# lmjakt/kmer_hasheR

Hardware: NVIDIA B200
Metric: kmers_indexed_per_s (higher is better)
Workload: dtype u64

## Files before the change

include/kmergpu.h:

```cpp
#ifndef KMERGPU_H
#define KMERGPU_H

#include <stddef.h>
#include <stdint.h>

#ifdef __cplusplus
extern "C" {
#endif

#define KMG_MAX_K 32

typedef enum {
  KMG_OK = 0,
  KMG_ERR_ARG = -1,
  KMG_ERR_K = -2,
  KMG_ERR_RANGE = -3,
  KMG_ERR_CUDA = -4,
  KMG_ERR_NOMEM = -5,
  KMG_ERR_NODEV = -6,
  KMG_ERR_UNSTABLE = -7
} kmg_status;

typedef struct kmg_index kmg_index;
typedef struct kmg_query kmg_query;
typedef struct kmg_join kmg_join;

const char *kmg_last_error(void);
int kmg_version(void);
int kmg_device_count(int *n);
int kmg_set_device(int device);
int kmg_set_stream(void *cuda_stream);
void *kmg_host_alloc(size_t bytes);
void kmg_host_free(void *p);

int kmg_build(const char *seq, int64_t len, int k, kmg_index **out);

#define KMG_ORDER_GROUPED 0
#define KMG_ORDER_SORTED 1
int kmg_build_ordered(const char *seq, int64_t len, int k, int order, kmg_index **out);
int kmg_index_order(const kmg_index *idx);

int kmg_free(kmg_index *idx);

int kmg_sizes(const kmg_index *idx, uint64_t *U, uint64_t *N, uint64_t *P);
int kmg_index_k(const kmg_index *idx);

int kmg_kmers_u64(const kmg_index *idx, uint64_t *keys );
int kmg_kmers_ascii(const kmg_index *idx, char *buf );
int kmg_counts(const kmg_index *idx, int32_t *counts );
int kmg_positions(const kmg_index *idx, int32_t *out );
int kmg_pairs(const kmg_index *idx, int32_t *out );
int kmg_pairs_chunk(const kmg_index *idx, uint64_t first, uint64_t n, int32_t *out );
int kmg_positions_base(const kmg_index *idx, uint64_t i_base, int32_t *out);
int kmg_pairs_chunk_base(const kmg_index *idx, uint64_t i_base, uint64_t first, uint64_t n, int32_t *out);

int kmg_query_begin(const kmg_index *idx, const char *q, int64_t qlen, int k, kmg_query **st,
                    uint64_t *M);
int kmg_query_begin_rc(const kmg_index *idx, const char *q, int64_t qlen, int k, kmg_query **st,
                       uint64_t *M);
int kmg_query_emit(kmg_query *st, int32_t *out );
int kmg_query_emit_chunk(kmg_query *st, uint64_t first, uint64_t n, int32_t *out );
int kmg_query_free(kmg_query *st);

int kmg_join_begin(const kmg_index *a, const kmg_index *b, kmg_join **st, uint64_t *M);
int kmg_join_emit(kmg_join *st, int32_t *out );
int kmg_join_emit_chunk(kmg_join *st, uint64_t first, uint64_t n, int32_t *out );
int kmg_join_free(kmg_join *st);

int kmg_shard_sample(const void *d_seq, int64_t g0, int64_t g1, int64_t L, int64_t s0, int64_t s1,
                     int k, int n, uint64_t *d_samples);
int kmg_shard_partition(const void *d_seq, int64_t g0, int64_t g1, int64_t L, int64_t s0,
                        int64_t s1, int k, const uint64_t *splitters ,
                        int nparts, uint64_t *d_keys, uint32_t *d_pos, uint64_t *counts);
int kmg_build_records(uint64_t *d_keys, uint32_t *d_pos, int64_t n, int k, kmg_index **out);
int kmg_query_records(const kmg_index *idx, const uint64_t *d_keys, const int32_t *d_i, int64_t n,
                      kmg_query **st, uint64_t *M);

typedef struct kmg_shard kmg_shard;
int kmg_shard_open(const void *d_seq, int64_t g0, int64_t g1, int64_t L, int64_t s0, int64_t s1,
                   int k, kmg_shard **out);
int kmg_shard_pack_bytes(int n_samples);
int kmg_shard_pack(const void *d_own, int64_t n_own, int k, int n_samples, int order, void *d_pack);
int kmg_shard_open_packed(const void *d_own, int64_t n_own, int64_t L, int world, int rank, int k,
                          int n_samples, int order, const void *d_allpack, kmg_shard **out,
                          uint64_t *d_splitters);
int kmg_shard_close(kmg_shard *sh);
int kmg_shard_set_mixed(kmg_shard *sh, int mixed);
int kmg_shard_windows(const kmg_shard *sh, int64_t *nstarts);
int kmg_shard_sample_keys(const kmg_shard *sh, int n, uint64_t *d_samples);
int kmg_shard_count(const kmg_shard *sh, const uint64_t *d_splitters, int nparts, uint64_t *d_counts);
int kmg_shard_scatter(const kmg_shard *sh, const uint64_t *d_splitters, int nparts, int rank,
                      void *const *peer_keys, void *const *peer_pos, uint64_t capacity,
                      const uint64_t *d_matrix, int32_t pos_add, uint64_t *d_info);
int kmg_build_received(uint64_t *d_keys, uint32_t *d_pos, uint64_t capacity, const uint64_t *d_info,
                       int k, int order, kmg_index **out);
int kmg_query_received(const kmg_index *idx, const uint64_t *d_keys, const int32_t *d_i,
                       uint64_t capacity, const uint64_t *d_info, int mixed, kmg_query **st,
                       uint64_t *M);
int kmg_shard_scatter_ranges(const kmg_shard *sh, int nparts, int rank, void *const *peer_keys, void *const *peer_pos,
                             void *const *peer_counts, uint64_t region_cap, int32_t pos_add);
int kmg_build_regions(uint64_t *d_keys, uint32_t *d_pos, uint64_t region_cap, int nparts, const uint64_t *d_counts, int k,
                      kmg_index **out);
int kmg_query_regions(const kmg_index *idx, const uint64_t *d_keys, const int32_t *d_i, uint64_t region_cap, int nparts,
                      const uint64_t *d_counts, kmg_query **st, uint64_t *M);
int kmg_ipc_alloc(size_t bytes, void **dptr, void *handle);
int kmg_ipc_free(void *dptr);
int kmg_ipc_open(const void *handle, void **dptr);
int kmg_ipc_close(void *dptr);

typedef struct kmg_counter kmg_counter;
int kmg_count_new(int k, int source_n, kmg_counter **out);
int kmg_count_add(kmg_counter *c, const char *seq, int64_t len, int source);
int kmg_count_sizes(const kmg_counter *c, uint64_t *U, int *source_n, int *k, uint64_t *new_total);
int kmg_count_kmers_u64(const kmg_counter *c, uint64_t *keys );
int kmg_count_kmers_ascii(const kmg_counter *c, char *buf );
int kmg_count_matrix(const kmg_counter *c, int32_t *out );
int kmg_count_positions(const kmg_counter *c, int32_t *out );
int kmg_count_spectrum(const kmg_counter *c, int source , uint32_t max_count, double *spec );
int kmg_index_spectrum(const kmg_index *idx, uint32_t max_count, double *spec );
int kmg_count_free(kmg_counter *c);

typedef struct kmg_reads kmg_reads;
int kmg_reads_open(const char *path, kmg_reads **out);
int kmg_reads_from_memory(const void *text, int64_t len, kmg_reads **out);
int kmg_reads_count(const kmg_reads *r, uint64_t *n_records, uint64_t *total_bases);
int kmg_reads_record(const kmg_reads *r, uint64_t i, int64_t *seq_len, char *name_buf, int name_cap);
int kmg_reads_sequence(const kmg_reads *r, uint64_t i, char *out );
int kmg_build_record(const kmg_reads *r, uint64_t i, int k, int order, kmg_index **out);
int kmg_count_add_reads(kmg_counter *c, const kmg_reads *r, int source);
int kmg_reads_free(kmg_reads *r);

int kmg_profile_enable(int on);
int kmg_profile_reset(void);
int kmg_profile_count(void);
int kmg_profile_get(int i, const char **name, double *total_ms, uint64_t *launches,
                    double *algo_bytes);
// ... 12 lines not shown
```

kmer_hasher_b200/__init__.py:

```python
from __future__ import annotations

import ctypes as C

import numpy as np

from . import _lib
from ._lib import KmgError, check

__all__ = ["KmerHash", "KmerCounts", "SequenceFile", "make_kmer_hash_file", "count_kmers_file", "make_kmer_hash", "kmer_pos", "seq_kmer_pos", "kmer_pairs", "count_kmers", "kmer_spectrum",
           "pinned_empty", "KmgError",
           "OPT_KMER", "OPT_POS", "OPT_PAIRS", "OPT_COUNT"]

OPT_KMER, OPT_POS, OPT_PAIRS, OPT_COUNT = 1, 2, 4, 8
ORDER_GROUPED, ORDER_SORTED = 0, 1
KMER_HASH_TAG = "kmer_hash_250930"
MAX_K = 32
INT_MAX = 2**31 - 1

_L = _lib.load()


def _seq_buffer(seq):
    if isinstance(seq, str):
        seq = seq.encode("latin-1")
# ... 99 lines not shown
        return nt.value

    def free(self):
        if self._h:
            _L.kmg_count_free(self._h)
            self._h = None


def _extract(ex_ptr) -> KmerHash:
    if not isinstance(ex_ptr, KmerHash):
        raise TypeError("ptr_r should be an external pointer")
    if ex_ptr.tag != KMER_HASH_TAG:
        raise ValueError("External pointer has incorrect tag")
    return ex_ptr


def _extract_index(ex_ptr) -> KmerHash:
    ix = _extract(ex_ptr)
    if isinstance(ix, KmerCounts):
        raise ValueError("this external pointer holds k-mer counts (count.kmers), not a position index")
    return ix


def make_kmer_hash(seq, k, do_sort=False) -> KmerHash:
    if isinstance(seq, (list, tuple)):
        if len(seq) < 1:
            raise ValueError("seq_r should be a character vector of length at least one")
        seq = seq[0]
    k = int(k)
    order = ORDER_SORTED if int(do_sort) else ORDER_GROUPED
    if k < 1 or k > MAX_K:
        raise ValueError("k must be a positive integer less than 1+MAX_K")
    ptr, n, keep = _seq_buffer(seq)
    if n <= k:
        raise ValueError("the length of the sequence must be at least k")
    h = C.c_void_p()
    check(_L.kmg_build_ordered(ptr, n, k, order, C.byref(h)))
    del keep
    return KmerHash(h.value, k)


def _by_key(ix: "KmerHash"):
    U = ix.sizes_un[0]
    keys = np.empty(U, np.uint64)
    check(_L.kmg_kmers_u64(ix._handle(), _out_ptr(keys)))
    order = np.argsort(keys, kind="stable")
    rank = np.empty(U, np.int64)
    rank[order] = np.arange(U)
    return keys, order, rank


def _renumber(rows: np.ndarray, rank: np.ndarray) -> np.ndarray:
    if len(rows) == 0:
        return rows
    new_i = rank[rows[:, 0].astype(np.int64) - 1] + 1
    o = np.argsort(new_i, kind="stable")
    out = rows[o].copy()
    out[:, 0] = new_i[o].astype(np.int32)
    return out


def kmer_pos(ex_ptr, opt_flag, out: dict | None = None, canonical: bool = False) -> dict:
    ix = _extract(ex_ptr)
    opt_flag = int(opt_flag)
    if isinstance(ix, KmerCounts):
        return _count_table_pos(ix, opt_flag)
    out = out or {}
    U, N = ix.sizes_un
    P = ix.sizes[2] if opt_flag & OPT_PAIRS else 0
    h = ix._handle()
    res = {"kmer": None, "pos": None, "pair.pos": None, "count": None}
    if opt_flag & OPT_KMER:
        buf = out.get("kmer_buf")
        if buf is None:
            buf = np.empty(U * (ix.k + 1), np.uint8)
        check(_L.kmg_kmers_ascii(h, _out_ptr(buf)))
        res["kmer"] = np.ascontiguousarray(buf[:U * (ix.k + 1)].reshape(U, ix.k + 1)[:, :ix.k]).view(f"S{ix.k}").ravel()
    if opt_flag & OPT_POS:
        if N > INT_MAX:
            raise OverflowError("pos matrix extent exceeds int")
        a = out.get("pos")
        if a is None:
            a = np.empty((N, 2), np.int32)
        check(_L.kmg_positions(h, _out_ptr(a)))
        res["pos"] = a[:N]
    if opt_flag & OPT_PAIRS:
        if P > INT_MAX:
            raise OverflowError(f"pair.pos would need {P} rows; an R matrix extent is int "
                                "(use kmg_pairs_chunk to stream)")
        a = out.get("pair.pos")
        if a is None:
            a = np.empty((P, 3), np.int32)
        check(_L.kmg_pairs(h, _out_ptr(a)))
        res["pair.pos"] = a[:P]
    if opt_flag & OPT_COUNT:
        a = out.get("count")
        if a is None:
            a = np.empty(U, np.int32)
        check(_L.kmg_counts(h, _out_ptr(a)))
        res["count"] = a[:U]
    if canonical and _L.kmg_index_order(h) != ORDER_SORTED:
        _, order, rank = _by_key(ix)
        if res["kmer"] is not None:
            res["kmer"] = res["kmer"][order]
        if res["count"] is not None:
            res["count"] = np.asarray(res["count"])[order]
        if res["pos"] is not None:
            res["pos"] = _renumber(np.asarray(res["pos"]), rank)
        if res["pair.pos"] is not None:
            res["pair.pos"] = _renumber(np.asarray(res["pair.pos"]), rank)
    return res


def count_kmers(seq, params, hash_ptr: "KmerCounts | None" = None) -> KmerCounts:
    params = [int(p) for p in params]
    if len(params) != 3:
        raise ValueError("k_r must be an integer vector of length 3")
    k, source, source_n = params
    if k < 1 or k > MAX_K:
        raise ValueError("k must be a positive integer less than 1+MAX_K")
    if source_n < 1 or source >= source_n or source < 0:
        raise ValueError("source_n must be larger than 1 and larger than source")
    if isinstance(seq, (str, bytes, bytearray, np.ndarray)) or hasattr(seq, "data_ptr"):
        seq = [seq]
    if len(seq) < 1:
        raise ValueError("seq_r should be a character vector of length at least one")
    if hash_ptr is None:
        h = C.c_void_p()
        check(_L.kmg_count_new(k, source_n, C.byref(h)))
        hash_ptr = KmerCounts(h.value, k, source_n)
    else:
        if not isinstance(hash_ptr, KmerCounts):
            raise ValueError("failed to extract kmer_hash from external pointer")
        if hash_ptr.k != k:
            raise ValueError("mismatch between specified k and that given in the external pointer")
        if hash_ptr.source_n != source_n:
            raise ValueError("mismatch between specified source_n and that of the external pointer")
    for s in seq:
        ptr, n, keep = _seq_buffer(s)
        if n <= k:
            continue
        check(_L.kmg_count_add(hash_ptr._handle(), ptr, n, source))
        del keep
    return hash_ptr


def _count_table_pos(ct: KmerCounts, opt_flag: int) -> dict:
    U = ct.sizes[0]
    sn, h = ct.source_n, ct._handle()
    res = {"kmer": None, "pos": None, "pair.pos": None, "count": None}
    if opt_flag & OPT_KMER:
        buf = np.empty(U * (ct.k + 1), np.uint8)
        check(_L.kmg_count_kmers_ascii(h, _out_ptr(buf)))
        res["kmer"] = np.ascontiguousarray(buf.reshape(U, ct.k + 1)[:, :ct.k]).view(f"S{ct.k}").ravel()
    if opt_flag & OPT_POS:
        if U * sn > INT_MAX:
            raise OverflowError("pos matrix extent exceeds int")
        a = np.empty((U * sn, 2), np.int32)
        check(_L.kmg_count_positions(h, _out_ptr(a)))
        res["pos"] = a
    if opt_flag & OPT_PAIRS:
        m = np.empty((U, sn), np.int32)
        check(_L.kmg_count_matrix(h, _out_ptr(m)))
        ia, ib = np.triu_indices(sn, 1)
        rows = np.empty((U, len(ia), 3), np.int32)
        rows[:, :, 0] = np.arange(1, U + 1, dtype=np.int32)[:, None]
        rows[:, :, 1] = m[:, ia]
        rows[:, :, 2] = m[:, ib]
        res["pair.pos"] = rows.reshape(-1, 3)
    if opt_flag & OPT_COUNT:
        res["count"] = np.full(U, sn, np.int32)
    return res


class SequenceFile:

    def __init__(self, path_or_text):
        h = C.c_void_p()
# ... 163 lines not shown
```

kmer_hasher_b200/_lib.py:

```python
from __future__ import annotations

import ctypes as C
import os

_HERE = os.path.dirname(os.path.abspath(__file__))
LIB_PATH = os.path.join(_HERE, "csrc", "libkmergpu.so")

u64p = C.POINTER(C.c_uint64)
i32p = C.POINTER(C.c_int32)
vp = C.c_void_p

SIGNATURES = {
    "kmg_last_error": (C.c_char_p, []),
    "kmg_version": (C.c_int, []),
    "kmg_device_count": (C.c_int, [C.POINTER(C.c_int)]),
    "kmg_set_device": (C.c_int, [C.c_int]),
    "kmg_set_stream": (C.c_int, [vp]),
    "kmg_host_alloc": (vp, [C.c_size_t]),
    "kmg_host_free": (None, [vp]),
    "kmg_build": (C.c_int, [vp, C.c_int64, C.c_int, C.POINTER(vp)]),
    "kmg_build_ordered": (C.c_int, [vp, C.c_int64, C.c_int, C.c_int, C.POINTER(vp)]),
    "kmg_index_order": (C.c_int, [vp]),
    "kmg_free": (C.c_int, [vp]),
    "kmg_sizes": (C.c_int, [vp, u64p, u64p, u64p]),
    "kmg_index_k": (C.c_int, [vp]),
    "kmg_kmers_u64": (C.c_int, [vp, vp]),
    "kmg_kmers_ascii": (C.c_int, [vp, vp]),
    "kmg_counts": (C.c_int, [vp, vp]),
    "kmg_positions": (C.c_int, [vp, vp]),
    "kmg_pairs": (C.c_int, [vp, vp]),
    "kmg_pairs_chunk": (C.c_int, [vp, C.c_uint64, C.c_uint64, vp]),
    "kmg_query_begin": (C.c_int, [vp, vp, C.c_int64, C.c_int, C.POINTER(vp), u64p]),
    "kmg_query_begin_rc": (C.c_int, [vp, vp, C.c_int64, C.c_int, C.POINTER(vp), u64p]),
    "kmg_query_emit": (C.c_int, [vp, vp]),
    "kmg_query_emit_chunk": (C.c_int, [vp, C.c_uint64, C.c_uint64, vp]),
    "kmg_query_free": (C.c_int, [vp]),
    "kmg_join_begin": (C.c_int, [vp, vp, C.POINTER(vp), u64p]),
    "kmg_join_emit": (C.c_int, [vp, vp]),
    "kmg_join_emit_chunk": (C.c_int, [vp, C.c_uint64, C.c_uint64, vp]),
    "kmg_join_free": (C.c_int, [vp]),
    "kmg_shard_sample": (C.c_int, [vp, C.c_int64, C.c_int64, C.c_int64, C.c_int64, C.c_int64, C.c_int, C.c_int, vp]),
    "kmg_shard_partition": (C.c_int, [vp, C.c_int64, C.c_int64, C.c_int64, C.c_int64, C.c_int64, C.c_int,
                                      u64p, C.c_int, vp, vp, u64p]),
    "kmg_build_records": (C.c_int, [vp, vp, C.c_int64, C.c_int, C.POINTER(vp)]),
    "kmg_query_records": (C.c_int, [vp, vp, vp, C.c_int64, C.POINTER(vp), u64p]),
    "kmg_shard_open": (C.c_int, [vp, C.c_int64, C.c_int64, C.c_int64, C.c_int64, C.c_int64, C.c_int, C.POINTER(vp)]),
    "kmg_shard_close": (C.c_int, [vp]),
    "kmg_shard_pack_bytes": (C.c_int, [C.c_int]),
    "kmg_shard_pack": (C.c_int, [vp, C.c_int64, C.c_int, C.c_int, C.c_int, vp]),
    "kmg_shard_open_packed": (C.c_int, [vp, C.c_int64, C.c_int64, C.c_int, C.c_int, C.c_int, C.c_int, C.c_int, vp, C.POINTER(vp), vp]),
    "kmg_shard_set_mixed": (C.c_int, [vp, C.c_int]),
    "kmg_shard_windows": (C.c_int, [vp, C.POINTER(C.c_int64)]),
    "kmg_shard_sample_keys": (C.c_int, [vp, C.c_int, vp]),
    "kmg_shard_count": (C.c_int, [vp, vp, C.c_int, vp]),
    "kmg_shard_scatter": (C.c_int, [vp, vp, C.c_int, C.c_int, C.POINTER(vp), C.POINTER(vp), C.c_uint64, vp, C.c_int32, vp]),
    "kmg_build_received": (C.c_int, [vp, vp, C.c_uint64, vp, C.c_int, C.c_int, C.POINTER(vp)]),
    "kmg_query_received": (C.c_int, [vp, vp, vp, C.c_uint64, vp, C.c_int, C.POINTER(vp), u64p]),
    "kmg_shard_scatter_ranges": (C.c_int, [vp, C.c_int, C.c_int, C.POINTER(vp), C.POINTER(vp), C.POINTER(vp), C.c_uint64, C.c_int32]),
    "kmg_build_regions": (C.c_int, [vp, vp, C.c_uint64, C.c_int, vp, C.c_int, C.POINTER(vp)]),
    "kmg_query_regions": (C.c_int, [vp, vp, vp, C.c_uint64, C.c_int, vp, C.POINTER(vp), u64p]),
    "kmg_ipc_alloc": (C.c_int, [C.c_size_t, C.POINTER(vp), vp]),
    "kmg_ipc_free": (C.c_int, [vp]),
    "kmg_ipc_open": (C.c_int, [vp, C.POINTER(vp)]),
    "kmg_ipc_close": (C.c_int, [vp]),
    "kmg_profile_enable": (C.c_int, [C.c_int]),
    "kmg_profile_reset": (C.c_int, []),
    "kmg_profile_count": (C.c_int, []),
    "kmg_profile_get": (C.c_int, [C.c_int, C.POINTER(C.c_char_p), C.POINTER(C.c_double), u64p, C.POINTER(C.c_double)]),
    "kmg_launch_count": (C.c_uint64, []),
    "kmg_selftest_lane_order": (C.c_int, [C.POINTER(C.c_uint32)]),
    "kmg_tune": (C.c_int, [C.c_char_p, C.c_int]),
    "kmg_count_new": (C.c_int, [C.c_int, C.c_int, C.POINTER(vp)]),
    "kmg_count_add": (C.c_int, [vp, vp, C.c_int64, C.c_int]),
    "kmg_count_sizes": (C.c_int, [vp, u64p, C.POINTER(C.c_int), C.POINTER(C.c_int), u64p]),
    "kmg_count_kmers_u64": (C.c_int, [vp, vp]),
    "kmg_count_kmers_ascii": (C.c_int, [vp, vp]),
    "kmg_count_matrix": (C.c_int, [vp, vp]),
    "kmg_count_positions": (C.c_int, [vp, vp]),
    "kmg_count_spectrum": (C.c_int, [vp, C.c_int, C.c_uint32, C.POINTER(C.c_double)]),
    "kmg_index_spectrum": (C.c_int, [vp, C.c_uint32, C.POINTER(C.c_double)]),
    "kmg_count_free": (C.c_int, [vp]),
    "kmg_reads_open": (C.c_int, [C.c_char_p, C.POINTER(vp)]),
    "kmg_reads_from_memory": (C.c_int, [vp, C.c_int64, C.POINTER(vp)]),
    "kmg_reads_count": (C.c_int, [vp, u64p, u64p]),
    "kmg_reads_record": (C.c_int, [vp, C.c_uint64, C.POINTER(C.c_int64), C.c_char_p, C.c_int]),
    "kmg_reads_sequence": (C.c_int, [vp, C.c_uint64, vp]),
    "kmg_build_record": (C.c_int, [vp, C.c_uint64, C.c_int, C.c_int, C.POINTER(vp)]),
    "kmg_count_add_reads": (C.c_int, [vp, vp, C.c_int]),
    "kmg_reads_free": (C.c_int, [vp]),
    "kmg_tune_get": (C.c_int64, [C.c_char_p, C.c_int64]),
    "kmg_trim": (C.c_int, []),
    "kmg_cached_bytes": (C.c_uint64, []),
    "kmg_positions_base": (C.c_int, [vp, C.c_uint64, vp]),
    "kmg_pairs_chunk_base": (C.c_int, [vp, C.c_uint64, C.c_uint64, C.c_uint64, vp]),
}

_lib = None


class KmgError(RuntimeError):
    def __init__(self, code: int, msg: str):
        super().__init__(f"libkmergpu error {code}: {msg}")
        self.code = code


def load() -> C.CDLL:
    global _lib
    if _lib is not None:
        return _lib
    if not os.path.exists(LIB_PATH):
        raise ImportError(f"{LIB_PATH} is missing: run `python -c 'import __graft_entry__ as g; g.build()'` "
                          "(libkmergpu is CUDA-only; there is no CPU fallback)")
    lib = C.CDLL(LIB_PATH)
    for name, (res, args) in SIGNATURES.items():
        fn = getattr(lib, name)
        fn.restype = res
        fn.argtypes = args
    _lib = lib
    return lib


def check(rc: int) -> None:
    if rc != 0:
        raise KmgError(rc, load().kmg_last_error().decode("utf-8", "replace"))
```

kmer_hasher_b200/csrc/api.cu:

```cuda
#include <cstdarg>
#include <cstdio>
#include <cstring>
#include <ctime>
#include <algorithm>
#include <atomic>
#include <condition_variable>
#include <deque>
#include <thread>
#include <map>
#include <mutex>
#include <string>
#include <type_traits>
#include <vector>

#include "../../include/kmergpu.h"
#include "common.cuh"
#include "csr.cuh"
#include "lookback.cuh"
#include "probe.cuh"
#include "sort.cuh"
#include "windows.cuh"

using namespace kmg;

// ... 321 lines not shown
  }
  ~CopyPool() {
    { std::lock_guard<std::mutex> l(mu); stop = true; }
    cv_work.notify_all();
    for (auto &t : th) t.join();
  }
};
static CopyPool g_pool;
constexpr size_t STAGE_BYTES = size_t(64) << 20;
constexpr int STAGE_SLOTS = 3;
struct Staging {
  std::mutex mu;
  char *slot[STAGE_SLOTS] = {nullptr, nullptr, nullptr};
  int ensure() {
    for (auto &p : slot)
      if (!p && cudaMallocHost((void **)&p, STAGE_BYTES) != cudaSuccess) { cudaGetLastError(); return fail(KMG_ERR_NOMEM, "pinned staging allocation failed"); }
    return KMG_OK;
  }
  void release() { for (auto &p : slot) { if (p) cudaFreeHost(p); p = nullptr; } }
};
static Staging g_stage;
static void stage_release() { std::lock_guard<std::mutex> gs(g_stage.mu); g_stage.release(); }
static bool staged_transfers() {
  static int on = -1;
  if (on < 0) { const char *e = getenv("KMERGPU_STAGING"); on = !(e && e[0] == '0'); }
  return on == 1;
}

static int staged_upload(void *d_dst, const void *h_src, size_t bytes, cudaStream_t s) {
  std::lock_guard<std::mutex> g(g_stage.mu);
  TRY(g_stage.ensure());
  cudaEvent_t *ev = g_ctx.ev + 4;
  int c = 0;
  for (size_t off = 0; off < bytes; off += STAGE_BYTES, ++c) {
    const int sl = c % STAGE_SLOTS;
    const size_t n = std::min(STAGE_BYTES, bytes - off);
    if (c >= STAGE_SLOTS) CU(cudaEventSynchronize(ev[sl]));
    g_pool.submit(c, g_stage.slot[sl], (const char *)h_src + off, n);
    g_pool.wait(c);
    CU(cudaMemcpyAsync((char *)d_dst + off, g_stage.slot[sl], n, cudaMemcpyHostToDevice, s));
    CU(cudaEventRecord(ev[sl], s));
  }
  CU(cudaStreamSynchronize(s));
  return KMG_OK;
}

enum PtrKind { PK_HOST_PAGEABLE, PK_HOST_PINNED, PK_DEVICE };
static PtrKind ptr_kind(const void *p) {
  cudaPointerAttributes a;
  if (cudaPointerGetAttributes(&a, p) != cudaSuccess) { cudaGetLastError(); return PK_HOST_PAGEABLE; }
  if (a.type == cudaMemoryTypeDevice || a.type == cudaMemoryTypeManaged) return PK_DEVICE;
  if (a.type == cudaMemoryTypeHost) return PK_HOST_PINNED;
  return PK_HOST_PAGEABLE;
}

struct DevSeq {
  uint8_t *buf = nullptr;
  uint8_t *base = nullptr;
  int64_t len = 0;
};
static int upload_seq(const void *src, int64_t len, cudaStream_t s, DevSeq *out) {
  size_t cap = 16 + (size_t)((len + 15) / 16) * 16 + 16;
  TRY(dalloc(&out->buf, cap, s));
  out->base = out->buf + 16;
  out->len = len;
  CU(cudaMemsetAsync(out->buf, 0, 16, s));
  CU(cudaMemsetAsync(out->buf + cap - 32, 0, 32, s));
  if (len > (int64_t)(8 << 20) && staged_transfers() && ptr_kind(src) == PK_HOST_PAGEABLE) return staged_upload(out->base, src, (size_t)len, s);
  if (len > 0) CU(cudaMemcpyAsync(out->base, src, (size_t)len, cudaMemcpyDefault, s));
  return KMG_OK;
}

struct kmg_index {
  int device = 0;
  int k = 0;
  uint64_t U = 0, N = 0;
  uint64_t P = 0, multi = 0;
  uint32_t maxc = 0;
  bool have_stats = false;
  bool grouped = false;
  int hbits = 0;
  bool unstable = false;
  uint64_t *ukeys = nullptr;
  uint32_t *ustart = nullptr;
  uint32_t *pos = nullptr;
  std::mutex mu;
  uint4 *hash = nullptr;
  uint64_t hash_nb = 0;
  int hash_hbits = 0;
  uint32_t *multi_u = nullptr;
  uint64_t *pair_off = nullptr;
};
struct kmg_query {
  const kmg_index *idx = nullptr;
  uint64_t H = 0, M = 0;
  int32_t *hit_i = nullptr;
  uint32_t *hit_start = nullptr;
  uint64_t *row_off = nullptr;
};

constexpr int HIST_THREADS = 512, HIST_ITEMS = 16, HIST_TILE = HIST_THREADS * HIST_ITEMS;
constexpr int RLE_THREADS = 256, RLE_ITEMS = 16, RLE_TILE = RLE_THREADS * RLE_ITEMS;
constexpr int PROBE_THREADS = 256, PROBE_ITEMS = 8, PROBE_TILE = PROBE_THREADS * PROBE_ITEMS;
constexpr int COMPACT_ITEMS = 8, COMPACT_TILE = PROBE_THREADS * COMPACT_ITEMS;
constexpr int EMIT_THREADS = 256, EMIT_TILE = EMIT_THREADS * 8;
constexpr int PIDX_THREADS = 256, PIDX_ITEMS = 8, PIDX_TILE = PIDX_THREADS * PIDX_ITEMS;

static int g_sort_shape = -1;
static int g_rank_override = -1;
static std::atomic<int> g_rank_dev[64];
static std::atomic<uint64_t> g_unstable_rebuilds{0};
static std::atomic<uint64_t> g_region_rebuilds{0};
static uint32_t g_sort_dbg = 0;
static int lane_order_failures(uint32_t *failures);
static bool log_on();

static int rank_variant() {
  if (g_rank_override >= 0) return g_rank_override;
  const int dev = g_ctx.device & 63;
  int v = g_rank_dev[dev].load(std::memory_order_acquire);
  if (v == 0) {
    const char *e = getenv("KMG_SORT_RANK");
    if (e) v = atoi(e) == 3 ? 2 : 1;
    else {
      uint32_t f = 1;
      v = (lane_order_failures(&f) == KMG_OK && f == 0) ? 2 : 1;
      if (log_on()) fprintf(stderr, "[kmergpu] device %d lane-order self-test: %u failures -> rank variant %d\n", dev, f, v == 2 ? 3 : 0);
    }
    int expect = 0;
    g_rank_dev[dev].compare_exchange_strong(expect, v, std::memory_order_acq_rel);
    v = g_rank_dev[dev].load(std::memory_order_acquire);
  }
  return v == 2 ? 3 : 0;
}
static void demote_rank_variant() {
  g_rank_dev[g_ctx.device & 63].store(1, std::memory_order_release);
  g_unstable_rebuilds.fetch_add(1);
  if (g_rank_override >= 3) g_rank_override = -1;
  if (log_on()) fprintf(stderr, "[kmergpu] device %d: position lists not ascending after a one-atomic sort pass; switching to the bitmap variant\n", g_ctx.device);
}

struct SortPlan { int rb, passes; int bits() const { return rb * passes; } };
static int g_hash_bits = 0;
static int g_hash_rb = 0;
static int g_no_regions = 0;
static int g_scatter_shape = 0;
static int g_scatter_bitmap = 0;
static int g_hash_cas = 0;
static int g_fix_cap = 0;
static SortPlan grouped_plan(int64_t n_upper) {
  if (g_hash_bits > 0) {
    const int rb = g_hash_rb > 0 && g_hash_bits % g_hash_rb == 0 ? g_hash_rb : (g_hash_bits % 8 == 0 ? 8 : 9);
    return SortPlan{rb, g_hash_bits / rb};
  }
  if (g_hash_rb > 0) return SortPlan{g_hash_rb, (36 + g_hash_rb - 1) / g_hash_rb};
  return n_upper <= (int64_t)400000000 ? SortPlan{8, 4} : SortPlan{8, 5};
}
static bool grouped_for(int k, int order, int64_t ) {
  return order == KMG_ORDER_GROUPED && 2 * k > 40;
}

static unsigned long long *g_trace = nullptr;
static int g_trace_tiles = 0;
extern "C" int kmg_trace_read(unsigned long long *host, int tiles) {
  if (!g_trace || tiles > g_trace_tiles) return -1;
  return cudaMemcpy(host, g_trace, (size_t)tiles * 64, cudaMemcpyDeviceToHost) == cudaSuccess ? 0 : -4;
}
extern "C" int kmg_tune(const char *key, int value) {
  if (key && !strcmp(key, "sort_cfg")) {
    if (value != -1 && value != 0 && value != 3 && value != 4) return fail(KMG_ERR_ARG, "sort_cfg must be -1 (auto), 0 (bitmap), 3 (one atomic) or 4 (tests: unstable on purpose)");
    g_rank_override = value;
    return KMG_OK;
  }
  if (key && !strcmp(key, "sort_shape")) {
    if (value < -1 || value > 2) return fail(KMG_ERR_ARG, "sort_shape out of range");
    g_sort_shape = value;
    return KMG_OK;
  }
  if (key && !strcmp(key, "sort_dbg")) { g_sort_dbg = (uint32_t)value; return KMG_OK; }
  if (key && !strcmp(key, "fix_cap")) { g_fix_cap = value > 0 ? value : 0; return KMG_OK; }
  if (key && !strcmp(key, "hash_cas")) { g_hash_cas = value != 0; return KMG_OK; }
  if (key && !strcmp(key, "scatter_bitmap")) { g_scatter_bitmap = value != 0; return KMG_OK; }
  if (key && !strcmp(key, "scatter_shape")) { g_scatter_shape = value; return KMG_OK; }
  if (key && !strcmp(key, "no_regions")) { g_no_regions = value; return KMG_OK; }
  if (key && !strcmp(key, "hash_bits")) {
    if (value != 0 && (value < 8 || value > 56 || (value % 8 && value % 9 && value % 10))) return fail(KMG_ERR_ARG, "hash_bits must be 0 (auto) or a multiple of 8, 9 or 10 in [8,56]");
    g_hash_bits = value;
    return KMG_OK;
  }
  if (key && !strcmp(key, "hash_rb")) {
    if (value != 0 && (value < 8 || value > 10)) return fail(KMG_ERR_ARG, "hash_rb must be 0, 8, 9 or 10");
    g_hash_rb = value;
    return KMG_OK;
  }
  if (key && !strcmp(key, "reset_rank")) {
    for (auto &v : g_rank_dev) v.store(0);
    return KMG_OK;
  }
  if (key && !strcmp(key, "sort_trace")) {
    if (g_trace) { cudaFree(g_trace); g_trace = nullptr; }
    g_trace_tiles = value;
    if (value > 0) { if (cudaMalloc(&g_trace, (size_t)value * 64) != cudaSuccess) return fail(KMG_ERR_NOMEM, "trace alloc"); cudaMemset(g_trace, 0, (size_t)value * 64); }
    return KMG_OK;
  }
  return fail(KMG_ERR_ARG, "unknown tuning key");
}
extern "C" int64_t kmg_tune_get(const char *key, int64_t arg) {
  if (key && !strcmp(key, "rank_variant")) return ctx_init() == KMG_OK ? rank_variant() : -1;
  if (key && !strcmp(key, "unstable_rebuilds")) return (int64_t)g_unstable_rebuilds.load();
  if (key && !strcmp(key, "region_rebuilds")) return (int64_t)g_region_rebuilds.load();
  if (key && !strcmp(key, "hash_bits")) return grouped_plan(arg).bits();
  if (key && !strcmp(key, "hash_rb")) return grouped_plan(arg).rb;
  return -1;
}
static int lane_order_failures(uint32_t *failures) {
  TRY(ctx_init());
  cudaStream_t s = g_ctx.stream();
  uint32_t *bad = nullptr;
  TRY(dalloc(&bad, 1, s));
  CU(cudaMemsetAsync(bad, 0, 4, s));
  LAUNCH("lane_order_selftest", s, lane_order_selftest_kernel<<<g_ctx.sms * 4, 256, 0, s>>>(bad));
  CU(cudaMemcpyAsync(failures, bad, 4, cudaMemcpyDeviceToHost, s));
  CU(cudaStreamSynchronize(s));
  dfree(bad, s);
  return KMG_OK;
}
extern "C" int kmg_selftest_lane_order(uint32_t *failures) {
  if (!failures) return fail(KMG_ERR_ARG, "failures is NULL");
  return lane_order_failures(failures);
}
static_assert(2 * (sizeof(PassSmem<PassCfg<256, 28, 2, 3, 4, 8>, false>) + 1024) <= 196 * 1024, "the record pass's tile outgrew the 196 KB carve-out");
constexpr int REGION_SAMPLE_STRIDE = 251;
constexpr int SORT_TILE_MIN = 4096;

template <class Cfg, bool FROM_SEQ, class BinFn, class NextFn, bool HAS_NEXT, bool PEER = false, bool SEGS = false>
static int launch_pass_cfg(const char *name, const PassParams<BinFn, NextFn> &P, int64_t n_upper, cudaStream_t s, int extra_tiles = 0) {
  using S = PassSmem<Cfg, FROM_SEQ>;
  if constexpr (!FROM_SEQ && !PEER && !SEGS) {
    if (P.segs) return launch_pass_cfg<Cfg, FROM_SEQ, BinFn, NextFn, HAS_NEXT, PEER, true>(name, P, n_upper, s, extra_tiles);
  }
  auto kern = scatter_pass_kernel<Cfg, FROM_SEQ, BinFn, NextFn, HAS_NEXT, PEER, SEGS>;
  CU(cudaFuncSetAttribute(kern, cudaFuncAttributeMaxDynamicSharedMemorySize, (int)sizeof(S)));
  const int64_t tiles = ceil_div<int64_t>(n_upper, Cfg::TILE) + extra_tiles;
  if (tiles == 0) return KMG_OK;
  LAUNCH(name, s, kern<<<(unsigned)tiles, Cfg::THREADS, sizeof(S), s>>>(P));
  return KMG_OK;
}
template <bool FROM_SEQ, class BinFn, class NextFn, bool HAS_NEXT>
static int launch_pass(const char *name, const PassParams<BinFn, NextFn> &P, int64_t n_upper, cudaStream_t s, int rb = RADIX_BITS, int extra_tiles = 0) {
  const int rank = rank_variant();
  const int shape = g_sort_shape < 0 ? (rb == 8 ? 1 : 0)
                                     : (rb == 8) ? ((FROM_SEQ && g_sort_shape == 0) ? 1 : g_sort_shape) : (g_sort_shape == 2 ? 0 : g_sort_shape);
#define KMG_GO(T, I, M, RK, RB) return launch_pass_cfg<PassCfg<T, I, M, RK, (RK >= 3 ? 4 : 8), RB>, FROM_SEQ, BinFn, NextFn, HAS_NEXT>(name, P, n_upper, s, extra_tiles)
#define KMG_SHAPES(RK, RB)                         \
  do {                                             \
    if (shape == 1) KMG_GO(256, 28, 2, RK, RB);    \
    KMG_GO(256, 24, 2, RK, RB);                    \
  } while (0)
  if (rb == 8) {
    if (rank == 4) KMG_GO(256, 24, 2, 4, 8);
    if (shape == 2) { if (rank == 3) KMG_GO(256, 20, 3, 3, 8); else KMG_GO(256, 20, 3, 0, 8); }
    if (rank == 3) KMG_SHAPES(3, 8); else KMG_SHAPES(0, 8);
  } else if (rb == 9) {
    if (rank == 4) KMG_GO(256, 24, 2, 4, 9);
    if (rank == 3) KMG_SHAPES(3, 9); else KMG_SHAPES(0, 9);
  } else if (rb == 10) {
    if (rank == 3) KMG_GO(256, 24, 2, 3, 10); else KMG_GO(256, 24, 2, 0, 10);
  }
#undef KMG_SHAPES
#undef KMG_GO
  return fail(KMG_ERR_ARG, "bad sort configuration");
}

static uint32_t record_tile(int rb) {
  const int shape = g_sort_shape < 0 ? (rb == 8 ? 1 : 0) : (rb == 8) ? g_sort_shape : (g_sort_shape == 2 ? 0 : g_sort_shape);
  if (rank_variant() == 4 || rb == 10) return 256 * 24;
  return shape == 1 ? 256 * 28 : shape == 2 ? 256 * 20 : 256 * 24;
}

struct SortScratch {
  uint32_t *small = nullptr;
  uint64_t *status = nullptr;
  size_t small_words = 0, status_words = 0;
  static constexpr size_t H = (size_t)(MAX_PASSES + 1) * MAX_NB;
  uint32_t *hist(int r) const { return small + (size_t)r * MAX_NB; }
  uint32_t *gbase(int r) const { return small + H + (size_t)r * MAX_NB; }
  uint32_t *common() const { return small + 2 * H; }
  uint32_t *ticket(int i) const { return small + 2 * H + RADIX + i; }
  IndexStats *stats() const { return reinterpret_cast<IndexStats *>(small + 2 * H + RADIX + 16); }
};
static int scratch_clear(SortScratch &sc, cudaStream_t s) {
  CU(cudaMemsetAsync(sc.small, 0, sc.small_words * 4, s));
  CU(cudaMemsetAsync(sc.status, 0, sc.status_words * sizeof(uint64_t), s));
  return KMG_OK;
}
static int scratch_alloc(SortScratch &sc, int64_t n_upper, cudaStream_t s, int rb = RADIX_BITS) {
  sc.small_words = 2 * SortScratch::H + RADIX + 16 + sizeof(IndexStats) / 4;
  TRY(dalloc(&sc.small, sc.small_words, s));
  const size_t tiles = (size_t)ceil_div<int64_t>(n_upper > 0 ? n_upper : 1, SORT_TILE_MIN) + MAX_SEGS + 1;
  sc.status_words = tiles << rb;
  TRY(dalloc(&sc.status, sc.status_words, s));
  return scratch_clear(sc, s);
}
static void scratch_free(SortScratch &sc, cudaStream_t s) { dfree(sc.small, s); dfree(sc.status, s); }

template <class... A>
static int launch_scan_hist(int rb, cudaStream_t s, A... args) {
  if (rb == 8) LAUNCH("scan_hist", s, scan_hist_kernel<256><<<1, 256, 0, s>>>(args...));
  else if (rb == 9) LAUNCH("scan_hist", s, scan_hist_kernel<512><<<1, 512, 0, s>>>(args...));
  else if (rb == 10) LAUNCH("scan_hist", s, scan_hist_kernel<1024><<<1, 1024, 0, s>>>(args...));
  else return fail(KMG_ERR_ARG, "bad digit width");
  return KMG_OK;
}

static int finish_index(kmg_index *ix, SortScratch &sc, uint64_t *keys_sorted, uint32_t *pos_sorted,
                        int64_t n_upper, cudaStream_t s, bool hashed = false) {
  IndexStats *st = sc.stats();
  uint64_t *ukeys = nullptr;
  uint32_t *ustart = nullptr;
  Pair64 *status2 = nullptr;
  const int64_t tiles = ceil_div<int64_t>(n_upper > 0 ? n_upper : 1, RLE_TILE);
  TRY(dalloc(&ukeys, (size_t)n_upper, s));
  TRY(dalloc(&ustart, (size_t)n_upper + 1, s));
  TRY(dalloc(&status2, (size_t)tiles, s));
  CU(cudaMemsetAsync(status2, 0, (size_t)tiles * sizeof(Pair64), s));
  LAUNCH("rle", s, rle_kernel<RLE_THREADS, RLE_ITEMS><<<(unsigned)tiles, RLE_THREADS, 0, s>>>(
                       keys_sorted, pos_sorted, st, ukeys, ustart, status2, sc.ticket(MAX_PASSES + 1), hashed));
  IndexStats h;
  CU(cudaMemcpyAsync(&h, st, sizeof h, cudaMemcpyDeviceToHost, s));
  CU(cudaStreamSynchronize(s));
  ix->N = h.n; ix->U = h.U; ix->unstable = h.unstable != 0;
  ix->have_stats = false;
  dfree(status2, s);
  if (h.U * 2 < (uint64_t)n_upper) {
    uint64_t *uk2; uint32_t *us2;
    TRY(dalloc(&uk2, (size_t)h.U, s));
    TRY(dalloc(&us2, (size_t)h.U + 1, s));
    CU(cudaMemcpyAsync(uk2, ukeys, h.U * sizeof(uint64_t), cudaMemcpyDeviceToDevice, s));
    CU(cudaMemcpyAsync(us2, ustart, (h.U + 1) * sizeof(uint32_t), cudaMemcpyDeviceToDevice, s));
    dfree(ukeys, s); dfree(ustart, s);
    ukeys = uk2; ustart = us2;
  }
  ix->ukeys = ukeys; ix->ustart = ustart; ix->pos = pos_sorted;
  const double N = (double)h.n, U = (double)h.U;
  prof_bytes("rle", 12 * N + 12 * U);
  return KMG_OK;
}

static int sort_tail(SortScratch &sc, SortPlan plan, int first_pass, bool has_next, uint64_t *&ka, uint32_t *&pa, uint64_t *&kb,
                     uint32_t *&pb, int64_t n_upper, cudaStream_t s, uint32_t *final_pos = nullptr, const TileSegs *seg0 = nullptr, int nsegs0 = 0,
                     int end_pass = -1) {
  const int R = plan.passes, rb = plan.rb;
  const uint32_t mask = (1u << rb) - 1;
  for (int r = first_pass; r < (end_pass > 0 ? end_pass : R); ++r) {
    PassParams<DigitBin, DigitBin> P{};
    P.keys_in = ka; P.pos_in = pa; P.keys_out = kb; P.pos_out = (final_pos && r == R - 1) ? final_pos : pb;
    P.gbase = sc.gbase(r); P.hist_next = sc.hist(r + 1);
    P.status = sc.status; P.ticket = sc.ticket(r); P.epoch = (uint32_t)(r + 1);
    P.n_records = &sc.stats()->n;
    P.segs = r == first_pass ? seg0 : nullptr;
    const int extra = r == first_pass && seg0 ? nsegs0 : 0;
    P.bin = DigitBin{r * rb, mask}; P.next = DigitBin{(r + 1) * rb, mask};
    P.dbg = g_sort_dbg;
    P.trace = (r == 2 && g_trace && ceil_div<int64_t>(n_upper, SORT_TILE_MIN) <= g_trace_tiles) ? g_trace : nullptr;
    if (has_next && r + 1 < R) {
      TRY((launch_pass<false, DigitBin, DigitBin, true>("sort_pass_hist", P, n_upper, s, rb, extra)));
      TRY(launch_scan_hist(rb, s, sc.hist(r + 1), sc.gbase(r + 1), (uint64_t *)nullptr));
    } else {
      TRY((launch_pass<false, DigitBin, DigitBin, false>("sort_pass", P, n_upper, s, rb, extra)));
    }
    std::swap(ka, kb);
    std::swap(pa, pb);
  }
  return KMG_OK;
}

static int fix_groups(SortScratch &sc, int bits, uint64_t *keys, uint32_t *pos, uint64_t *sk, uint32_t *sp, int64_t n_upper, cudaStream_t s,
                      uint32_t *h_cnt , uint32_t **fixmem_out) {
  FixLists fl{};
  uint32_t *fixmem = nullptr;
  fl.small_cap = g_fix_cap > 0 ? (uint32_t)g_fix_cap : (uint32_t)std::max<int64_t>(1 << 20, n_upper / 8);
  fl.big_cap = 1 << 16;
  const size_t words = 4 + CLAIM_SLOTS + 2 * (size_t)fl.small_cap + 2 * (size_t)fl.big_cap;
  TRY(dalloc(&fixmem, words, s));
  *fixmem_out = fixmem;
  CU(cudaMemsetAsync(fixmem, 0, (4 + CLAIM_SLOTS) * sizeof(uint32_t), s));
  fl.counters = fixmem; fl.claim = fixmem + 4;
  fl.small_tasks = reinterpret_cast<uint2 *>(fixmem + 4 + CLAIM_SLOTS);
  fl.big_tasks = fl.small_tasks + fl.small_cap;
  const unsigned dgrid = (unsigned)std::min<int64_t>(ceil_div<int64_t>(n_upper, 256 * 8), (int64_t)g_ctx.sms * 16);
  if (bits == 32) LAUNCH("group_detect", s, group_detect_kernel<true><<<dgrid, 256, 0, s>>>(keys, sc.stats(), bits, fl));
  else LAUNCH("group_detect", s, group_detect_kernel<false><<<dgrid, 256, 0, s>>>(keys, sc.stats(), bits, fl));
  LAUNCH("small_fix", s, small_fix_kernel<<<g_ctx.sms * 4, 128, 0, s>>>(keys, pos, fl));
  LAUNCH("big_fix", s, big_fix_kernel<1024><<<g_ctx.sms, 1024, 0, s>>>(keys, pos, sk, sp, fl));
  CU(cudaMemcpyAsync(h_cnt, fl.counters, 4 * sizeof(uint32_t), cudaMemcpyDeviceToHost, s));
  return KMG_OK;
}

static int build_grouped(const SeqView &sv, SortPlan plan, kmg_index *ix, SortScratch &sc, uint64_t *&ka, uint32_t *&pa, uint64_t *&kb,
                         uint32_t *&pb, int64_t n_upper, cudaStream_t s, bool *overflow, bool regions, bool *region_overflow) {
  const int R = plan.passes, rb = plan.rb, NB = 1 << rb;
  const uint32_t mask = (1u << rb) - 1;
  uint64_t *kr = nullptr, *d_counts = nullptr;
  uint32_t *pr = nullptr, *d_over = nullptr;
  TileSegs *segs = nullptr;
  uint32_t h_over = 0;
  regions = regions && R > 1 && NB <= MAX_SEGS && n_upper <= (int64_t)1600000000;
  const uint32_t cap = (uint32_t)(((uint64_t)(n_upper / NB) * 5 / 4 + 4096 + 15) & ~uint64_t(15));
  if (regions && g_no_regions == 2) {
  } else if (regions && n_upper >= (int64_t)REGION_SAMPLE_STRIDE * 4096) {
    uint32_t *d_s = nullptr, h_est = 0;
    TRY(dalloc(&d_s, (size_t)MAX_NB + 1, s));
    int rc0 = KMG_OK;
    if (cudaMemsetAsync(d_s, 0, (MAX_NB + 1) * sizeof(uint32_t), s) != cudaSuccess) rc0 = fail(KMG_ERR_CUDA, "memset failed");
    if (rc0 == KMG_OK) {
      const unsigned g = (unsigned)std::min<int64_t>(ceil_div<int64_t>(n_upper / REGION_SAMPLE_STRIDE, 256), (int64_t)g_ctx.sms * 8);
      region_sample_kernel<<<g, 256, 0, s>>>(sv, REGION_SAMPLE_STRIDE, mask, d_s);
      region_estimate_kernel<<<1, 256, 0, s>>>(d_s, NB, REGION_SAMPLE_STRIDE, d_s + MAX_NB);
      if (cudaMemcpyAsync(&h_est, d_s + MAX_NB, 4, cudaMemcpyDeviceToHost, s) != cudaSuccess || cudaStreamSynchronize(s) != cudaSuccess)
        rc0 = fail(KMG_ERR_CUDA, "region estimate failed: %s", cudaGetErrorString(cudaGetLastError()));
    }
    dfree(d_s, s);
    TRY(rc0);
    if ((uint64_t)h_est * 10 > (uint64_t)cap * 9) regions = false;
  } else if (regions) {
    regions = false;
  }
  auto body = [&]() -> int {
    PassParams<DigitBin, DigitBin> P{};
    P.sv = sv; P.keys_out = ka; P.pos_out = pa;
    P.gbase = sc.gbase(0); P.hist_next = sc.hist(1);
    P.status = sc.status; P.ticket = sc.ticket(0); P.epoch = 1;
    P.hashed = 1;
    P.dbg = g_sort_dbg;
    P.bin = DigitBin{0, mask}; P.next = DigitBin{rb, mask};
    if (regions) {
      TRY(dalloc(&kr, (size_t)NB * cap, s));
      TRY(dalloc(&pr, (size_t)NB * cap, s));
      TRY(dalloc(&d_counts, (size_t)MAX_SEGS, s));
      TRY(dalloc(&d_over, 4, s));
      TRY(dalloc(&segs, 1, s));
      CU(cudaMemsetAsync(d_counts, 0, MAX_SEGS * sizeof(uint64_t), s));
      LAUNCH("region_gbase", s, region_gbase_kernel<<<1, 256, 0, s>>>(sc.gbase(0), NB, cap, d_over));
      P.keys_out = kr; P.pos_out = pr;
      P.bin_counts = d_counts; P.bin_cap = cap; P.bin_overflow = d_over;
      TRY((launch_pass<true, DigitBin, DigitBin, true>("sort_pass_seq", P, n_upper, s, rb)));
      TRY(launch_scan_hist(rb, s, sc.hist(1), sc.gbase(1), (uint64_t *)nullptr));
      LAUNCH("tile_segs", s, tile_segs_kernel<<<1, MAX_SEGS, 0, s>>>(d_counts, NB, (uint64_t)cap, record_tile(rb), segs, &sc.stats()->n));
      CU(cudaMemcpyAsync(&h_over, d_over, 4, cudaMemcpyDeviceToHost, s));
      TRY(sort_tail(sc, plan, 1, true, kr, pr, ka, pa, n_upper, s, nullptr, segs, NB, 2));
      std::swap(kr, ka); std::swap(pr, pa);
      TRY(sort_tail(sc, plan, 2, true, ka, pa, kb, pb, n_upper, s));
    } else {
      const int64_t tiles = ceil_div<int64_t>(n_upper, HIST_TILE);
      const unsigned hgrid = (unsigned)std::min<int64_t>(tiles, (int64_t)g_ctx.sms * 2);
      LAUNCH("hist_seq", s, hist_seq_kernel<HIST_THREADS, HIST_ITEMS, HashDigitBin><<<hgrid, HIST_THREADS, 0, s>>>(sv, sc.hist(0), HashDigitBin{0, mask}));
      TRY(launch_scan_hist(rb, s, sc.hist(0), sc.gbase(0), &sc.stats()->n));
      if (R > 1) {
        TRY((launch_pass<true, DigitBin, DigitBin, true>("sort_pass_seq", P, n_upper, s, rb)));
        TRY(launch_scan_hist(rb, s, sc.hist(1), sc.gbase(1), (uint64_t *)nullptr));
      } else {
        TRY((launch_pass<true, DigitBin, DigitBin, false>("sort_pass_seq", P, n_upper, s, rb)));
      }
      TRY(sort_tail(sc, plan, 1, true, ka, pa, kb, pb, n_upper, s));
    }
    return KMG_OK;
  };
  int rc = body();
  uint32_t h_cnt[4] = {0, 0, 0, 0};
  uint32_t *fixmem = nullptr;
  if (rc == KMG_OK) rc = fix_groups(sc, plan.bits(), ka, pa, kb, pb, n_upper, s, h_cnt, &fixmem);
  if (rc == KMG_OK) rc = finish_index(ix, sc, ka, pa, n_upper, s, true);
  dfree(fixmem, s);
  dfree(kr, s); dfree(pr, s); dfree(d_counts, s); dfree(d_over, s); dfree(segs, s);
  *overflow = h_cnt[2] != 0;
  *region_overflow = h_over != 0;
  if (log_on()) fprintf(stderr, "[kmergpu] grouped build on %d bits: %u short and %u long groups fixed\n", plan.bits(), h_cnt[0], h_cnt[1]);
  ix->hbits = plan.bits();
  const double N = (double)ix->N, L = (double)sv.avail;
  if (!regions) prof_bytes("hist_seq", L);
  prof_bytes("sort_pass_seq", L + 12 * N);
  if (R > 2) prof_bytes("sort_pass_hist", 24 * N * (R - 2));
  if (R > 1) prof_bytes("sort_pass", 24 * N);
  prof_bytes("group_detect", 8 * N);
  return rc;
}

static int build_attempt(const SeqView &sv, int k, kmg_index *ix, int order, cudaStream_t s) {
  const int64_t n_upper = sv.nstarts;
  SortScratch sc;
  uint64_t *ka = nullptr, *kb = nullptr;
  uint32_t *pa = nullptr, *pb = nullptr;
  auto body = [&]() -> int {
    const int R = num_passes(k);
    const bool grouped = grouped_for(k, order, n_upper);
    const SortPlan gp = grouped_plan(n_upper);
    TRY(scratch_alloc(sc, n_upper, s, grouped ? gp.rb : RADIX_BITS));
    TRY(dalloc(&ka, (size_t)n_upper, s));
    TRY(dalloc(&pa, (size_t)n_upper, s));
    if (R > 1) { TRY(dalloc(&kb, (size_t)n_upper, s)); TRY(dalloc(&pb, (size_t)n_upper, s)); }
    if (grouped) {
      bool overflow = false, region_overflow = false;
      TRY(build_grouped(sv, gp, ix, sc, ka, pa, kb, pb, n_upper, s, &overflow, g_no_regions != 1, &region_overflow));
      if (region_overflow) {
        g_region_rebuilds.fetch_add(1);
        if (log_on()) fprintf(stderr, "[kmergpu] a first-pass bin outgrew its region: rebuilding with the histogram sweep\n");
        void *old[3] = {ix->ukeys, ix->ustart, nullptr};
        for (void *p : old) g_arena[ix->device & 63].put(p, s, false);
        ix->ukeys = nullptr; ix->ustart = nullptr; ix->pos = nullptr; ix->hbits = 0; ix->unstable = false;
        TRY(scratch_clear(sc, s));
        overflow = false;
        TRY(build_grouped(sv, gp, ix, sc, ka, pa, kb, pb, n_upper, s, &overflow, false, &region_overflow));
      }
      if (!overflow) { pa = nullptr; ix->grouped = true; return KMG_OK; }
      void *old[3] = {ix->ukeys, ix->ustart, nullptr};
      for (void *p : old) g_arena[ix->device & 63].put(p, s, false);
      ix->ukeys = nullptr; ix->ustart = nullptr; ix->pos = nullptr; ix->hbits = 0;
      scratch_free(sc, s);
      TRY(scratch_alloc(sc, n_upper, s, RADIX_BITS));
    }
    const int64_t tiles = ceil_div<int64_t>(n_upper, HIST_TILE);
    const unsigned hgrid = (unsigned)std::min<int64_t>(tiles, (int64_t)g_ctx.sms * 2);
    LAUNCH("hist_all", s, hist_all_kernel<HIST_THREADS, HIST_ITEMS><<<hgrid, HIST_THREADS, 0, s>>>(sv, sc.common(), sc.hist(0), MAX_NB));
    LAUNCH("hist_finish", s, hist_finish_kernel<<<R, RADIX, 0, s>>>(k, sc.common(), sc.hist(0), sc.gbase(0), MAX_NB, &sc.stats()->n));
    {
      PassParams<DigitBin, DigitBin> P{};
      P.sv = sv; P.keys_out = ka; P.pos_out = pa;
      P.gbase = sc.gbase(0);
      P.status = sc.status; P.ticket = sc.ticket(0); P.epoch = 1;
      P.dbg = g_sort_dbg;
      P.bin = DigitBin{0}; P.next = DigitBin{RADIX_BITS};
      TRY((launch_pass<true, DigitBin, DigitBin, false>("sort_pass_seq", P, n_upper, s)));
    }
    TRY(sort_tail(sc, SortPlan{RADIX_BITS, R}, 1, false, ka, pa, kb, pb, n_upper, s));
    TRY(finish_index(ix, sc, ka, pa, n_upper, s));
    pa = nullptr;
    const double N = (double)ix->N, L = (double)sv.avail;
    prof_bytes("hist_all", L);
    prof_bytes("sort_pass_seq", L + 12 * N);
    if (R > 1) prof_bytes("sort_pass", 24 * N * (R - 1));
    return KMG_OK;
  };
  const int rc = body();
  dfree(ka, s); dfree(kb, s); dfree(pa, s); dfree(pb, s);
  scratch_free(sc, s);
  return rc;
}

static void release_index_arrays(kmg_index *ix, cudaStream_t s) {
  void *ptrs[3] = {ix->ukeys, ix->ustart, ix->pos};
  for (void *p : ptrs) g_arena[ix->device & 63].put(p, s, false);
  ix->ukeys = nullptr; ix->ustart = nullptr; ix->pos = nullptr;
  ix->grouped = false; ix->hbits = 0; ix->unstable = false;
}

static int build_from_view(const SeqView &sv, int k, kmg_index **out, int order = KMG_ORDER_SORTED) {
  cudaStream_t s = g_ctx.stream();
  kmg_index *ix = new (std::nothrow) kmg_index();
  if (!ix) return fail(KMG_ERR_NOMEM, "host allocation failed");
  ix->device = g_ctx.device;
  ix->k = k;
  const int64_t n_upper = sv.nstarts;
  if (n_upper <= 0) {
    int rc = dalloc(&ix->ustart, 1, s);
    if (rc == KMG_OK && cudaMemsetAsync(ix->ustart, 0, 4, s) != cudaSuccess) rc = fail(KMG_ERR_CUDA, "memset failed");
    if (rc != KMG_OK) { delete ix; return rc; }
    cudaStreamSynchronize(s);
    *out = ix;
    return KMG_OK;
  }
  if (n_upper > (int64_t)INT32_MAX) { delete ix; return fail(KMG_ERR_RANGE, "%lld windows exceed the 32-bit coordinates of the reference", (long long)n_upper); }
  int rc = build_attempt(sv, k, ix, order, s);
  if (rc == KMG_OK && ix->unstable) {
    const bool was_atomic = rank_variant() >= 3;
    release_index_arrays(ix, s);
    if (!was_atomic) rc = fail(KMG_ERR_CUDA, "internal error: position lists not ascending after a stable sort");
    else {
      demote_rank_variant();
      rc = build_attempt(sv, k, ix, order, s);
      if (rc == KMG_OK && ix->unstable) rc = fail(KMG_ERR_CUDA, "internal error: position lists not ascending after a stable sort");
    }
  }
  if (rc != KMG_OK) { cudaStreamSynchronize(s); kmg_free(ix); return rc; }
  *out = ix;
  return KMG_OK;
}

static double wall_ms() {
  timespec ts;
  clock_gettime(CLOCK_MONOTONIC, &ts);
  return ts.tv_sec * 1e3 + ts.tv_nsec * 1e-6;
}
static bool log_on() {
  static int on = -1;
  if (on < 0) { const char *e = getenv("KMERGPU_LOG"); on = e && e[0] == '1'; }
  return on == 1;
}

extern "C" int kmg_build(const char *seq, int64_t len, int k, kmg_index **out) {
  return kmg_build_ordered(seq, len, k, KMG_ORDER_GROUPED, out);
}
extern "C" int kmg_index_order(const kmg_index *ix) { return !ix ? fail(KMG_ERR_ARG, "index is NULL") : (ix->grouped ? KMG_ORDER_GROUPED : KMG_ORDER_SORTED); }

extern "C" int kmg_build_ordered(const char *seq, int64_t len, int k, int order, kmg_index **out) {
  if (!out) return fail(KMG_ERR_ARG, "out is NULL");
  if (order != KMG_ORDER_SORTED && order != KMG_ORDER_GROUPED) return fail(KMG_ERR_ARG, "order must be KMG_ORDER_SORTED or KMG_ORDER_GROUPED");
  *out = nullptr;
  if (k < 1 || k > KMG_MAX_K) return fail(KMG_ERR_K, "k must be a positive integer less than 1+MAX_K");
  if (len < 0 || (len > 0 && !seq)) return fail(KMG_ERR_ARG, "bad sequence pointer/length");
  const double t0 = wall_ms();
  TRY(ctx_init());
  cudaStream_t s = g_ctx.stream();
  DevSeq ds;
  TRY(upload_seq(seq, len, s, &ds));
  const double t1 = wall_ms();
  SeqView sv;
  sv.base = ds.base; sv.nstarts = len - k + 1 > 0 ? len - k + 1 : 0; sv.avail = len; sv.s0 = 0; sv.L = len; sv.k = k;
  int rc = build_from_view(sv, k, out, order);
  dfree(ds.buf, s);
  if (log_on())
    fprintf(stderr, "[kmergpu] build len=%lld k=%d: upload(enqueue) %.3f ms, build %.3f ms (host wall clock)\n", (long long)len, k, t1 - t0, wall_ms() - t1);
  return rc;
}

extern "C" int kmg_free(kmg_index *ix) {
  if (!ix) return KMG_OK;
  int prev = -1;
  cudaGetDevice(&prev);
  cudaSetDevice(ix->device);
  const bool mine = g_ctx.ready && g_ctx.device == ix->device;
  if (mine) cudaStreamSynchronize(g_ctx.stream()); else cudaDeviceSynchronize();
  void *ptrs[6] = {ix->ukeys, ix->ustart, ix->pos, ix->hash, ix->multi_u, ix->pair_off};
  for (void *p : ptrs) g_arena[ix->device & 63].put(p, nullptr, true);
  cudaGetLastError();
  if (prev >= 0) cudaSetDevice(prev);
  delete ix;
  return KMG_OK;
}

static int use_index(const kmg_index *ix);
static int ensure_stats(const kmg_index *cix) {
  kmg_index *ix = const_cast<kmg_index *>(cix);
  std::lock_guard<std::mutex> g(ix->mu);
  if (ix->have_stats) return KMG_OK;
  if (ix->U == 0) { ix->P = 0; ix->multi = 0; ix->maxc = 0; ix->have_stats = true; return KMG_OK; }
  TRY(use_index(ix));
  cudaStream_t s = g_ctx.stream();
  IndexStats *st = nullptr, h;
  TRY(dalloc(&st, 1, s));
  auto body = [&]() -> int {
    CU(cudaMemsetAsync(st, 0, sizeof(IndexStats), s));
    const unsigned sgrid = (unsigned)std::min<uint64_t>(ceil_div<uint64_t>(ix->U, 256 * 16), (uint64_t)g_ctx.sms * 8);
    LAUNCH("stats", s, stats_kernel<256><<<sgrid, 256, 0, s>>>(ix->ustart, ix->U, st));
    CU(cudaMemcpyAsync(&h, st, sizeof h, cudaMemcpyDeviceToHost, s));
    CU(cudaStreamSynchronize(s));
    return KMG_OK;
  };
  const int rc = body();
  dfree(st, s);
  TRY(rc);
  ix->P = h.P; ix->multi = h.multi; ix->maxc = h.maxc;
  ix->have_stats = true;
  prof_bytes("stats", 4.0 * (double)ix->U);
  return KMG_OK;
}

extern "C" int kmg_sizes(const kmg_index *ix, uint64_t *U, uint64_t *N, uint64_t *P) {
  if (!ix) return fail(KMG_ERR_ARG, "index is NULL");
  if (P) { TRY(ensure_stats(ix)); *P = ix->P; }
  if (U) *U = ix->U;
  if (N) *N = ix->N;
  return KMG_OK;
}
extern "C" int kmg_index_k(const kmg_index *ix) { return ix ? ix->k : fail(KMG_ERR_ARG, "index is NULL"); }
extern "C" int kmg_index_stats(const kmg_index *ix, uint64_t *multi, uint32_t *max_count) {
  if (!ix) return fail(KMG_ERR_ARG, "index is NULL");
  TRY(ensure_stats(ix));
  if (multi) *multi = ix->multi;
  if (max_count) *max_count = ix->maxc;
  return KMG_OK;
}

static int use_index(const kmg_index *ix) {
  if (!ix) return fail(KMG_ERR_ARG, "index is NULL");
  TRY(ctx_init());
  if (ix->device != g_ctx.device)
    return fail(KMG_ERR_ARG, "the index lives on device %d but this thread works on device %d: call kmg_set_device(%d) first", ix->device, g_ctx.device, ix->device);
  return KMG_OK;
}

template <class Emit>
static int stream_rows_staged(uint64_t total, size_t row_bytes, void *out, Emit emit) {
  std::lock_guard<std::mutex> g(g_stage.mu);
  TRY(g_stage.ensure());
  cudaStream_t s = g_ctx.stream(), cs = g_ctx.copy;
  const uint64_t chunk_rows = std::max<uint64_t>(1, STAGE_BYTES / row_bytes);
  const int64_t nchunks = (int64_t)ceil_div<uint64_t>(total, chunk_rows);
  uint64_t *blk = nullptr;
  char *buf[2] = {nullptr, nullptr};
  TRY(dalloc(&blk, (size_t)ceil_div<uint64_t>(chunk_rows, EMIT_TILE), s));
  int rc = dalloc(&buf[0], chunk_rows * row_bytes, s);
  if (rc == KMG_OK && nchunks > 1) rc = dalloc(&buf[1], chunk_rows * row_bytes, s);
  cudaEvent_t *ev = g_ctx.ev;
  int64_t issued = 0, retired = 0;
  while (rc == KMG_OK && retired < nchunks) {
    while (rc == KMG_OK && issued < nchunks && issued - retired < 2) {
      const int64_t c = issued;
      const int b = (int)(c & 1), sl = (int)(c % STAGE_SLOTS);
      const uint64_t first = (uint64_t)c * chunk_rows, rows = std::min<uint64_t>(chunk_rows, total - first);
      if (c >= STAGE_SLOTS) g_pool.wait((int)(c - STAGE_SLOTS));
      if (c >= 2) cudaStreamWaitEvent(s, ev[4 + (int)((c - 2) % STAGE_SLOTS)], 0);
      rc = emit(first, rows, (void *)buf[b], blk, s);
      if (rc != KMG_OK) break;
      cudaEventRecord(ev[b], s);
      cudaStreamWaitEvent(cs, ev[b], 0);
      if (cudaMemcpyAsync(g_stage.slot[sl], buf[b], rows * row_bytes, cudaMemcpyDeviceToHost, cs) != cudaSuccess)
        rc = fail(KMG_ERR_CUDA, "device->host copy failed: %s", cudaGetErrorString(cudaGetLastError()));
      cudaEventRecord(ev[4 + sl], cs);
      ++issued;
    }
    if (rc != KMG_OK) break;
    const int64_t c = retired;
    const int sl = (int)(c % STAGE_SLOTS);
    const uint64_t first = (uint64_t)c * chunk_rows, rows = std::min<uint64_t>(chunk_rows, total - first);
    if (cudaEventSynchronize(ev[4 + sl]) != cudaSuccess) { rc = fail(KMG_ERR_CUDA, "device->host copy failed: %s", cudaGetErrorString(cudaGetLastError())); break; }
    g_pool.submit((int)c, (char *)out + first * row_bytes, g_stage.slot[sl], rows * row_bytes);
    ++retired;
  }
  for (int64_t c = std::max<int64_t>(0, retired - STAGE_SLOTS); c < retired; ++c) g_pool.wait((int)c);
  cudaStreamSynchronize(cs);
  cudaStreamSynchronize(s);
  dfree(buf[0], s); dfree(buf[1], s); dfree(blk, s);
  if (rc == KMG_OK) {
    cudaError_t e = cudaGetLastError();
    if (e != cudaSuccess) rc = fail(KMG_ERR_CUDA, "extraction failed: %s", cudaGetErrorString(e));
  }
  return rc;
}

template <class Emit>
static int stream_rows(uint64_t total, size_t row_bytes, void *out, uint64_t chunk_rows, Emit emit) {
  if (total == 0) return KMG_OK;
  cudaStream_t s = g_ctx.stream();
  const bool to_device = ptr_kind(out) == PK_DEVICE;
  if (!to_device) chunk_rows = std::min<uint64_t>(chunk_rows, total);
  uint64_t *blk = nullptr;
  TRY(dalloc(&blk, (size_t)ceil_div<uint64_t>(to_device ? total : chunk_rows, EMIT_TILE), s));
  if (to_device) {
    int rc = emit((uint64_t)0, total, out, blk, s);
    if (rc == KMG_OK && cudaStreamSynchronize(s) != cudaSuccess) rc = fail(KMG_ERR_CUDA, "extraction failed: %s", cudaGetErrorString(cudaGetLastError()));
    dfree(blk, s);
    return rc;
  }
  if (staged_transfers() && total * row_bytes > (uint64_t)(8 << 20) && ptr_kind(out) == PK_HOST_PAGEABLE) {
    dfree(blk, s);
    return stream_rows_staged(total, row_bytes, out, emit);
  }
  char *buf[2] = {nullptr, nullptr};
  int rc = dalloc(&buf[0], chunk_rows * row_bytes, s);
  if (rc == KMG_OK && total > chunk_rows) rc = dalloc(&buf[1], chunk_rows * row_bytes, s);
  if (rc != KMG_OK) { dfree(buf[0], s); dfree(blk, s); return rc; }
  cudaStream_t cs = g_ctx.copy;
  cudaEvent_t *ev = g_ctx.ev;
  uint64_t done = 0;
  for (int c = 0; done < total && rc == KMG_OK; ++c, done += chunk_rows) {
    const int b = c & 1;
    const uint64_t rows = std::min<uint64_t>(chunk_rows, total - done);
    if (c >= 2) cudaStreamWaitEvent(s, ev[2 + b], 0);
    rc = emit(done, rows, (void *)buf[b], blk, s);
    if (rc != KMG_OK) break;
    cudaEventRecord(ev[b], s);
    cudaStreamWaitEvent(cs, ev[b], 0);
    if (cudaMemcpyAsync((char *)out + done * row_bytes, buf[b], rows * row_bytes, cudaMemcpyDeviceToHost, cs) != cudaSuccess)
      rc = fail(KMG_ERR_CUDA, "device->host copy failed: %s", cudaGetErrorString(cudaGetLastError()));
    cudaEventRecord(ev[2 + b], cs);
  }
  cudaStreamSynchronize(cs);
  cudaStreamSynchronize(s);
  dfree(buf[0], s); dfree(buf[1], s); dfree(blk, s);
  if (rc == KMG_OK) {
    cudaError_t e = cudaGetLastError();
    if (e != cudaSuccess) rc = fail(KMG_ERR_CUDA, "extraction failed: %s", cudaGetErrorString(e));
  }
  return rc;
}
constexpr uint64_t CHUNK_BYTES = uint64_t(256) << 20;

template <typename OffT>
static int block_starts(const OffT *off, uint64_t cnt, uint64_t first, uint64_t rows, cudaStream_t s, uint64_t *blk) {
  const uint64_t nb = ceil_div<uint64_t>(rows, EMIT_TILE);
  LAUNCH("segment_starts", s, segment_starts_kernel<OffT><<<(unsigned)ceil_div<uint64_t>(nb, 128), 128, 0, s>>>(off, cnt, first, EMIT_TILE, nb, blk));
  return KMG_OK;
}

extern "C" int kmg_kmers_u64(const kmg_index *ix, uint64_t *keys) {
  TRY(use_index(ix));
  if (!keys && ix->U) return fail(KMG_ERR_ARG, "keys is NULL");
  if (ix->U == 0) return KMG_OK;
  cudaStream_t s = g_ctx.stream();
  CU(cudaMemcpyAsync(keys, ix->ukeys, ix->U * sizeof(uint64_t), cudaMemcpyDefault, s));
  CU(cudaStreamSynchronize(s));
  return KMG_OK;
}

extern "C" int kmg_kmers_ascii(const kmg_index *ix, char *out) {
  TRY(use_index(ix));
  if (!out && ix->U) return fail(KMG_ERR_ARG, "buf is NULL");
  const size_t stride = (size_t)ix->k + 1;
  const int k = ix->k;
  const uint64_t *ukeys = ix->ukeys;
  const int sms = g_ctx.sms;
  int rc = stream_rows(ix->U, stride, out, CHUNK_BYTES / stride, [=](uint64_t first, uint64_t rows, void *dst, uint64_t *, cudaStream_t s) -> int {
    const unsigned grid = (unsigned)std::min<uint64_t>(ceil_div<uint64_t>(rows * stride, 256), (uint64_t)sms * 16);
    LAUNCH("kmers_ascii", s, kmers_ascii_kernel<<<grid, 256, 0, s>>>(ukeys + first, rows, k, (char *)dst));
    return KMG_OK;
  });
  prof_bytes("kmers_ascii", (double)ix->U * (8 + stride));
  return rc;
}

extern "C" int kmg_counts(const kmg_index *ix, int32_t *out) {
  TRY(use_index(ix));
  if (!out && ix->U) return fail(KMG_ERR_ARG, "counts is NULL");
  const uint32_t *ustart = ix->ustart;
  const int sms = g_ctx.sms;
  int rc = stream_rows(ix->U, 4, out, CHUNK_BYTES / 4, [=](uint64_t first, uint64_t rows, void *dst, uint64_t *, cudaStream_t s) -> int {
    const unsigned grid = (unsigned)std::min<uint64_t>(ceil_div<uint64_t>(rows, 256), (uint64_t)sms * 16);
    LAUNCH("counts", s, counts_kernel<<<grid, 256, 0, s>>>(ustart + first, rows, (int32_t *)dst));
    return KMG_OK;
  });
  prof_bytes("counts", 8.0 * ix->U);
  return rc;
}

extern "C" int kmg_positions(const kmg_index *ix, int32_t *out) { return kmg_positions_base(ix, 0, out); }

extern "C" int kmg_positions_base(const kmg_index *ix, uint64_t i_base, int32_t *out) {
  TRY(use_index(ix));
  if (!out && ix->N) return fail(KMG_ERR_ARG, "out is NULL");
  if (i_base + ix->U > (uint64_t)INT32_MAX) return fail(KMG_ERR_RANGE, "k-mer numbers exceed int");
  const uint32_t *ustart = ix->ustart, *pos = ix->pos;
  const uint64_t U = ix->U, N = ix->N;
  int rc = stream_rows(N, 8, out, CHUNK_BYTES / 8, [=](uint64_t first, uint64_t rows, void *dst, uint64_t *blk, cudaStream_t s) -> int {
    const unsigned grid = (unsigned)ceil_div<uint64_t>(rows, EMIT_TILE);
    TRY(block_starts(ustart, U, first, rows, s, blk));
    LAUNCH("positions", s, positions_kernel<EMIT_THREADS><<<grid, EMIT_THREADS, 0, s>>>(ustart, U, pos, first, rows, blk, (int2 *)dst, (uint32_t)i_base));
    return KMG_OK;
  });
  prof_bytes("positions", 4.0 * U + 12.0 * N);
  return rc;
}

static int ensure_pair_index(kmg_index *ix) {
  TRY(ensure_stats(ix));
  std::lock_guard<std::mutex> g(ix->mu);
  if (ix->pair_off || ix->multi == 0) return KMG_OK;
  cudaStream_t s = g_ctx.stream();
  uint32_t *multi_u = nullptr, *ticket = nullptr;
  uint64_t *pair_off = nullptr;
  Pair64 *status = nullptr;
  const uint64_t tiles = ceil_div<uint64_t>(ix->U, PIDX_TILE);
  TRY(dalloc(&multi_u, ix->multi, s));
  TRY(dalloc(&pair_off, ix->multi, s));
  TRY(dalloc(&status, tiles, s));
  TRY(dalloc(&ticket, 1, s));
  CU(cudaMemsetAsync(status, 0, tiles * sizeof(Pair64), s));
  CU(cudaMemsetAsync(ticket, 0, 4, s));
  LAUNCH("pair_index", s, pair_index_kernel<PIDX_THREADS, PIDX_ITEMS><<<(unsigned)tiles, PIDX_THREADS, 0, s>>>(
                              ix->ustart, ix->U, multi_u, pair_off, status, ticket));
  CU(cudaStreamSynchronize(s));
  dfree(status, s); dfree(ticket, s);
  ix->multi_u = multi_u; ix->pair_off = pair_off;
  prof_bytes("pair_index", 4.0 * ix->U + 12.0 * ix->multi);
  return KMG_OK;
}

extern "C" int kmg_pairs_chunk(const kmg_index *cix, uint64_t first, uint64_t n, int32_t *out) { return kmg_pairs_chunk_base(cix, 0, first, n, out); }

extern "C" int kmg_pairs_chunk_base(const kmg_index *cix, uint64_t i_base, uint64_t first, uint64_t n, int32_t *out) {
  TRY(use_index(cix));
  if (i_base + cix->U > (uint64_t)INT32_MAX) return fail(KMG_ERR_RANGE, "k-mer numbers exceed int");
  kmg_index *ix = const_cast<kmg_index *>(cix);
  TRY(ensure_stats(ix));
  if (first > ix->P || n > ix->P - first) return fail(KMG_ERR_ARG, "pair rows [%llu,+%llu) outside [0,%llu)", (unsigned long long)first, (unsigned long long)n, (unsigned long long)ix->P);
  if (n == 0) return KMG_OK;
  if (!out) return fail(KMG_ERR_ARG, "out is NULL");
  TRY(ensure_pair_index(ix));
  const uint32_t *ustart = ix->ustart, *pos = ix->pos, *multi_u = ix->multi_u;
  const uint64_t *pair_off = ix->pair_off;
  const uint64_t n_multi = ix->multi;
  int rc = stream_rows(n, 12, out, CHUNK_BYTES / 12, [=](uint64_t f, uint64_t rows, void *dst, uint64_t *blk, cudaStream_t s) -> int {
    const unsigned grid = (unsigned)ceil_div<uint64_t>(rows, EMIT_TILE);
    TRY(block_starts(pair_off, n_multi, first + f, rows, s, blk));
    LAUNCH("pairs", s, pairs_kernel<EMIT_THREADS><<<grid, EMIT_THREADS, 0, s>>>(ustart, pos, multi_u, pair_off, n_multi, first + f, rows, blk, (int32_t *)dst, (uint32_t)i_base));
    return KMG_OK;
  });
  prof_bytes("pairs", 12.0 * n);
  return rc;
}
extern "C" int kmg_pairs(const kmg_index *ix, int32_t *out) {
  if (!ix) return fail(KMG_ERR_ARG, "index is NULL");
  TRY(ensure_stats(ix));
  return kmg_pairs_chunk(ix, 0, ix->P, out);
}

static int ensure_hash(kmg_index *ix) {
  std::lock_guard<std::mutex> g(ix->mu);
  if (ix->hash || ix->U == 0) return KMG_OK;
  cudaStream_t s = g_ctx.stream();
  const unsigned grid = (unsigned)std::min<uint64_t>(ceil_div<uint64_t>(ix->U, 256), (uint64_t)g_ctx.sms * 32);
  uint4 *slots = nullptr;
  const bool stream = ix->grouped && ix->hbits >= 8 && ix->hbits <= 56 && !g_hash_cas && (ix->hbits >= 40 || ix->U + ix->U / 4 <= (uint64_t(1) << ix->hbits));
  if (stream) {
    const uint64_t nb = std::max<uint64_t>(ix->U + ix->U / 4, 4);
    uint64_t *d_last = nullptr;
    TRY(dalloc(&slots, nb * BUCKET_SLOTS, s));
    int rc = dalloc(&d_last, 1, s);
    if (rc != KMG_OK) { dfree(slots, s); return rc; }
    auto body = [&]() -> int {
      KeyHash kt{slots, nb, ix->hbits};
      uint64_t h_last = 0;
      LAUNCH("hash_stream", s, hash_stream_kernel<<<grid, 256, 0, s>>>(ix->ukeys, ix->ustart, ix->U, kt, d_last));
      CU(cudaMemcpyAsync(&h_last, d_last, 8, cudaMemcpyDeviceToHost, s));
      CU(cudaStreamSynchronize(s));
      if (h_last + 1 < nb) CU(cudaMemsetAsync(slots + (h_last + 1) * BUCKET_SLOTS, 0, (nb - h_last - 1) * BUCKET_SLOTS * sizeof(uint4), s));
      constexpr int OV_ITEMS = 8;
      const unsigned ogrid = (unsigned)ceil_div<uint64_t>(ix->U, 256 * OV_ITEMS);
      LAUNCH("hash_insert", s, hash_overflow_kernel<OV_ITEMS><<<ogrid, 256, 0, s>>>(ix->ukeys, ix->ustart, ix->U, kt));
      CU(cudaStreamSynchronize(s));
      return KMG_OK;
    };
    rc = body();
    dfree(d_last, s);
    if (rc != KMG_OK) { dfree(slots, s); return rc; }
    ix->hash = slots; ix->hash_nb = nb; ix->hash_hbits = ix->hbits;
    prof_bytes("hash_stream", 12.0 * ix->U + 16.0 * BUCKET_SLOTS * nb);
    prof_bytes("hash_insert", 8.0 * ix->U);
    return KMG_OK;
  }
  uint64_t cap = 4 * BUCKET_SLOTS;
  while (cap < 2 * ix->U) cap <<= 1;
  TRY(dalloc(&slots, cap, s));
  CU(cudaMemsetAsync(slots, 0, cap * sizeof(uint4), s));
  LAUNCH("hash_insert", s, hash_insert_kernel<<<grid, 256, 0, s>>>(ix->ukeys, ix->ustart, ix->U, KeyHash{slots, cap / BUCKET_SLOTS, 0}, false));
  CU(cudaStreamSynchronize(s));
  ix->hash = slots; ix->hash_nb = cap / BUCKET_SLOTS; ix->hash_hbits = 0;
  prof_bytes("hash_insert", 12.0 * ix->U + 16.0 * ix->U);
  return KMG_OK;
}

static int query_common(const kmg_index *cix, bool from_seq, const SeqView &sv, const uint64_t *d_keys,
                        const int32_t *d_i, int64_t n, kmg_query **out, uint64_t *M, const uint64_t *d_n = nullptr, bool mixed = false) {
  kmg_index *ix = const_cast<kmg_index *>(cix);
  cudaStream_t s = g_ctx.stream();
  kmg_query *q = new (std::nothrow) kmg_query();
  if (!q) return fail(KMG_ERR_NOMEM, "host allocation failed");
  q->idx = ix;
  const int64_t total = from_seq ? sv.nstarts : n;
  if (total <= 0 || ix->U == 0) { *out = q; if (M) *M = 0; return KMG_OK; }
  int rc = ensure_hash(ix);
  if (rc != KMG_OK) { delete q; return rc; }
  QueryStats *qs = nullptr;
  Pair64 *status = nullptr;
  uint32_t *ticket = nullptr;
  uint2 *found = nullptr;
  auto body = [&]() -> int {
    const uint64_t tiles = ceil_div<uint64_t>((uint64_t)total, COMPACT_TILE);
    TRY(dalloc(&q->hit_i, (size_t)total, s));
    TRY(dalloc(&q->hit_start, (size_t)total, s));
    TRY(dalloc(&q->row_off, (size_t)total, s));
    TRY(dalloc(&qs, 1, s));
    TRY(dalloc(&status, tiles, s));
    TRY(dalloc(&ticket, 1, s));
    CU(cudaMemsetAsync(qs, 0, sizeof(QueryStats), s));
    CU(cudaMemsetAsync(status, 0, tiles * sizeof(Pair64), s));
    CU(cudaMemsetAsync(ticket, 0, 4, s));
    KeyHash kt{ix->hash, ix->hash_nb, ix->hash_hbits};
    TRY(dalloc(&found, (size_t)total, s));
    const unsigned ltiles = (unsigned)ceil_div<uint64_t>((uint64_t)total, PROBE_TILE);
    if (from_seq) {
      LAUNCH("probe_lookup", s, probe_lookup_kernel<PROBE_THREADS, PROBE_ITEMS, true><<<ltiles, PROBE_THREADS, 0, s>>>(sv, nullptr, 0, nullptr, kt, found));
      LAUNCH("probe_compact", s, probe_compact_kernel<PROBE_THREADS, COMPACT_ITEMS, true><<<(unsigned)tiles, PROBE_THREADS, 0, s>>>(
                                     found, sv.s0 + sv.k, nullptr, total, nullptr, q->hit_i, q->hit_start, q->row_off, qs, status, ticket));
    } else {
      LAUNCH("probe_lookup_rec", s, probe_lookup_kernel<PROBE_THREADS, PROBE_ITEMS, false><<<ltiles, PROBE_THREADS, 0, s>>>(sv, d_keys, n, d_n, kt, found, mixed));
      LAUNCH("probe_compact", s, probe_compact_kernel<PROBE_THREADS, COMPACT_ITEMS, false><<<(unsigned)tiles, PROBE_THREADS, 0, s>>>(
                                     found, 0, d_i, n, d_n, q->hit_i, q->hit_start, q->row_off, qs, status, ticket));
    }
    QueryStats h;
    CU(cudaMemcpyAsync(&h, qs, sizeof h, cudaMemcpyDeviceToHost, s));
    CU(cudaStreamSynchronize(s));
    q->H = h.H; q->M = h.M;
    return KMG_OK;
  };
  rc = body();
  dfree(qs, s); dfree(status, s); dfree(ticket, s); dfree(found, s);
  if (rc != KMG_OK) { cudaStreamSynchronize(s); kmg_query_free(q); return rc; }
  prof_bytes(from_seq ? "probe_lookup" : "probe_lookup_rec", (from_seq ? (double)sv.avail : 8.0 * total) + 128.0 * total + 8.0 * total);
  prof_bytes("probe_compact", 8.0 * total + 16.0 * q->H);
  *out = q;
  if (M) *M = q->M;
  return KMG_OK;
}

extern "C" int kmg_query_begin(const kmg_index *ix, const char *qseq, int64_t qlen, int k, kmg_query **st, uint64_t *M) {
  if (!st) return fail(KMG_ERR_ARG, "st is NULL");
  *st = nullptr;
  if (k < 1 || k > KMG_MAX_K) return fail(KMG_ERR_K, "k must be in [1,32]");
  if (qlen < 0 || (qlen > 0 && !qseq)) return fail(KMG_ERR_ARG, "bad query pointer/length");
  if (qlen + 1 > (int64_t)INT32_MAX) return fail(KMG_ERR_RANGE, "query longer than int coordinates");
  TRY(use_index(ix));
  cudaStream_t s = g_ctx.stream();
  DevSeq ds;
  TRY(upload_seq(qseq, qlen, s, &ds));
  SeqView sv;
  sv.base = ds.base; sv.nstarts = qlen - k + 1 > 0 ? qlen - k + 1 : 0; sv.avail = qlen; sv.s0 = 0; sv.L = qlen; sv.k = k;
  int rc = query_common(ix, true, sv, nullptr, nullptr, 0, st, M);
  dfree(ds.buf, s);
  return rc;
}

extern "C" int kmg_query_begin_rc(const kmg_index *ix, const char *qseq, int64_t qlen, int k, kmg_query **st, uint64_t *M) {
  if (!st) return fail(KMG_ERR_ARG, "st is NULL");
  *st = nullptr;
  if (k < 1 || k > KMG_MAX_K) return fail(KMG_ERR_K, "k must be in [1,32]");
  if (qlen < 0 || (qlen > 0 && !qseq)) return fail(KMG_ERR_ARG, "bad query pointer/length");
  if (qlen + 1 > (int64_t)INT32_MAX) return fail(KMG_ERR_RANGE, "query longer than int coordinates");
// ... 26 lines not shown
  *st = nullptr;
  if (n < 0 || (n > 0 && (!d_keys || !d_i))) return fail(KMG_ERR_ARG, "bad record arrays");
  TRY(use_index(ix));
  SeqView sv{};
  return query_common(ix, false, sv, d_keys, d_i, n, st, M);
}

extern "C" int kmg_query_emit_chunk(kmg_query *q, uint64_t first, uint64_t n, int32_t *out) {
  if (!q) return fail(KMG_ERR_ARG, "query is NULL");
  TRY(use_index(q->idx));
  if (first > q->M || n > q->M - first) return fail(KMG_ERR_ARG, "rows outside the result");
  if (n == 0) return KMG_OK;
  if (!out) return fail(KMG_ERR_ARG, "out is NULL");
  const kmg_index *ix = q->idx;
  const int32_t *hit_i = q->hit_i;
  const uint32_t *hit_start = q->hit_start, *pos = ix->pos;
  const uint64_t *row_off = q->row_off;
  const uint64_t H = q->H;
  int rc = stream_rows(n, 8, out, CHUNK_BYTES / 8, [=](uint64_t f, uint64_t rows, void *dst, uint64_t *blk, cudaStream_t s) -> int {
    const unsigned grid = (unsigned)ceil_div<uint64_t>(rows, EMIT_TILE);
    TRY(block_starts(row_off, H, first + f, rows, s, blk));
    LAUNCH("probe_emit", s, probe_emit_kernel<EMIT_THREADS><<<grid, EMIT_THREADS, 0, s>>>(hit_i, hit_start, row_off, H, pos, first + f, rows, blk, (int2 *)dst));
    return KMG_OK;
  });
  prof_bytes("probe_emit", 12.0 * n);
  return rc;
}
extern "C" int kmg_query_emit(kmg_query *q, int32_t *out) {
  if (!q) return fail(KMG_ERR_ARG, "query is NULL");
  return kmg_query_emit_chunk(q, 0, q->M, out);
}
extern "C" int kmg_query_free(kmg_query *q) {
  if (!q) return KMG_OK;
  const int dev = q->idx ? q->idx->device : g_ctx.device;
  int prev = -1;
  cudaGetDevice(&prev);
  cudaSetDevice(dev);
  const bool mine = g_ctx.ready && g_ctx.device == dev;
  if (mine) cudaStreamSynchronize(g_ctx.stream()); else cudaDeviceSynchronize();
  void *ptrs[3] = {q->hit_i, q->hit_start, q->row_off};
  for (void *p : ptrs) g_arena[dev & 63].put(p, nullptr, true);
  cudaGetLastError();
  if (prev >= 0) cudaSetDevice(prev);
  delete q;
  return KMG_OK;
}

struct kmg_join {
  const kmg_index *a = nullptr, *b = nullptr;
  uint64_t H = 0, M = 0;
  uint32_t *hit_astart = nullptr, *hit_bstart = nullptr, *hit_cb = nullptr;
  uint64_t *row_off = nullptr;
};

extern "C" int kmg_join_free(kmg_join *j) {
  if (!j) return KMG_OK;
  const int dev = j->a ? j->a->device : g_ctx.device;
  int prev = -1;
  cudaGetDevice(&prev);
  cudaSetDevice(dev);
  const bool mine = g_ctx.ready && g_ctx.device == dev;
  if (mine) cudaStreamSynchronize(g_ctx.stream()); else cudaDeviceSynchronize();
  void *ptrs[4] = {j->hit_astart, j->hit_bstart, j->hit_cb, j->row_off};
  for (void *p : ptrs) g_arena[dev & 63].put(p, nullptr, true);
  cudaGetLastError();
  if (prev >= 0) cudaSetDevice(prev);
  delete j;
  return KMG_OK;
}

extern "C" int kmg_join_begin(const kmg_index *a, const kmg_index *cb, kmg_join **out, uint64_t *M) {
  if (!out) return fail(KMG_ERR_ARG, "st is NULL");
  *out = nullptr;
  if (!a || !cb) return fail(KMG_ERR_ARG, "index is NULL");
  if (a->device != cb->device) return fail(KMG_ERR_ARG, "the two indexes live on different devices (%d, %d)", a->device, cb->device);
  TRY(use_index(a));
  kmg_index *b = const_cast<kmg_index *>(cb);
  cudaStream_t s = g_ctx.stream();
  kmg_join *j = new (std::nothrow) kmg_join();
  if (!j) return fail(KMG_ERR_NOMEM, "host allocation failed");
  j->a = a; j->b = b;
  if (a->U == 0 || b->U == 0) { *out = j; if (M) *M = 0; return KMG_OK; }
  int rc = ensure_hash(b);
  if (rc != KMG_OK) { delete j; return rc; }
  QueryStats *qs = nullptr;
  Pair64 *status = nullptr;
  uint32_t *ticket = nullptr;
  uint2 *found = nullptr;
  const uint64_t U = a->U;
  auto body = [&]() -> int {
    const uint64_t tiles = ceil_div<uint64_t>(U, PROBE_TILE);
    TRY(dalloc(&j->hit_astart, (size_t)U, s));
    TRY(dalloc(&j->hit_bstart, (size_t)U, s));
    TRY(dalloc(&j->hit_cb, (size_t)U, s));
    TRY(dalloc(&j->row_off, (size_t)U, s));
    TRY(dalloc(&found, (size_t)U, s));
    TRY(dalloc(&qs, 1, s));
    TRY(dalloc(&status, tiles, s));
    TRY(dalloc(&ticket, 1, s));
    CU(cudaMemsetAsync(qs, 0, sizeof(QueryStats), s));
    CU(cudaMemsetAsync(status, 0, tiles * sizeof(Pair64), s));
    CU(cudaMemsetAsync(ticket, 0, 4, s));
    KeyHash kt{b->hash, b->hash_nb, b->hash_hbits};
    SeqView sv{};
    LAUNCH("probe_lookup_rec", s, probe_lookup_kernel<PROBE_THREADS, PROBE_ITEMS, false><<<(unsigned)tiles, PROBE_THREADS, 0, s>>>(
                                      sv, a->ukeys, (int64_t)U, nullptr, kt, found));
    LAUNCH("join_compact", s, join_compact_kernel<PROBE_THREADS, PROBE_ITEMS><<<(unsigned)tiles, PROBE_THREADS, 0, s>>>(
                                  found, a->ustart, U, j->hit_astart, j->hit_bstart, j->hit_cb, j->row_off, qs, status, ticket));
    QueryStats h;
    CU(cudaMemcpyAsync(&h, qs, sizeof h, cudaMemcpyDeviceToHost, s));
    CU(cudaStreamSynchronize(s));
    j->H = h.H; j->M = h.M;
    return KMG_OK;
  };
  rc = body();
  dfree(qs, s); dfree(status, s); dfree(ticket, s); dfree(found, s);
  if (rc != KMG_OK) { cudaStreamSynchronize(s); kmg_join_free(j); return rc; }
  prof_bytes("probe_lookup_rec", 8.0 * U + 128.0 * U + 8.0 * U);
  prof_bytes("join_compact", 12.0 * U + 20.0 * j->H);
  *out = j;
  if (M) *M = j->M;
  return KMG_OK;
}

extern "C" int kmg_join_emit_chunk(kmg_join *j, uint64_t first, uint64_t n, int32_t *out) {
  if (!j) return fail(KMG_ERR_ARG, "join is NULL");
  TRY(use_index(j->a));
  if (first > j->M || n > j->M - first) return fail(KMG_ERR_ARG, "rows outside the result");
  if (n == 0) return KMG_OK;
  if (!out) return fail(KMG_ERR_ARG, "out is NULL");
  const uint32_t *ha = j->hit_astart, *hb = j->hit_bstart, *hc = j->hit_cb, *pa = j->a->pos, *pb = j->b->pos;
  const uint64_t *row_off = j->row_off;
  const uint64_t H = j->H;
  int rc = stream_rows(n, 8, out, CHUNK_BYTES / 8, [=](uint64_t f, uint64_t rows, void *dst, uint64_t *blk, cudaStream_t s) -> int {
    const unsigned grid = (unsigned)ceil_div<uint64_t>(rows, EMIT_TILE);
    TRY(block_starts(row_off, H, first + f, rows, s, blk));
    LAUNCH("join_emit", s, join_emit_kernel<EMIT_THREADS><<<grid, EMIT_THREADS, 0, s>>>(ha, hb, hc, row_off, H, pa, pb, first + f, rows, blk, (int2 *)dst));
    return KMG_OK;
  });
  prof_bytes("join_emit", 16.0 * n);
  return rc;
}
extern "C" int kmg_join_emit(kmg_join *j, int32_t *out) {
  if (!j) return fail(KMG_ERR_ARG, "join is NULL");
  return kmg_join_emit_chunk(j, 0, j->M, out);
}

static int shard_view(const void *d_seq, int64_t g0, int64_t g1, int64_t L, int64_t s0, int64_t s1, int k,
                      cudaStream_t s, DevSeq *ds, SeqView *sv) {
  if (k < 1 || k > KMG_MAX_K) return fail(KMG_ERR_K, "k must be in [1,32]");
  if (!(0 <= g0 && g0 <= g1 && g1 <= L && 0 <= s0 && s0 <= s1)) return fail(KMG_ERR_ARG, "inconsistent shard bounds");
  const int64_t need_lo = s0 > 0 ? s0 - 1 : 0, need_hi = std::min<int64_t>(L, s1 + k - 1);
  if (s1 > s0 && (g0 > need_lo || g1 < need_hi)) return fail(KMG_ERR_ARG, "shard bytes [%lld,%lld) do not cover [%lld,%lld)", (long long)g0, (long long)g1, (long long)need_lo, (long long)need_hi);
  const int64_t avail = std::max<int64_t>(0, need_hi - s0);
  size_t cap = 16 + (size_t)((avail + 15) / 16) * 16 + 16;
  TRY(dalloc(&ds->buf, cap, s));
  ds->base = ds->buf + 16;
  CU(cudaMemsetAsync(ds->buf, 0, 16, s));
  CU(cudaMemsetAsync(ds->buf + cap - 32, 0, 32, s));
  if (avail > 0) {
    const int64_t lead = s0 > 0 ? 1 : 0;
    CU(cudaMemcpyAsync(ds->base - lead, (const uint8_t *)d_seq + (s0 - lead - g0), (size_t)(avail + lead), cudaMemcpyDefault, s));
  }
  int64_t nstarts = std::min<int64_t>(s1, L - k + 1) - s0;
  sv->base = ds->base; sv->nstarts = nstarts > 0 ? nstarts : 0; sv->avail = avail; sv->s0 = s0; sv->L = L; sv->k = k;
  return KMG_OK;
// ... 21 lines not shown
  LAUNCH("sample", s, sample_kernel<<<ceil_div(n, 256), 256, 0, s>>>(sv, n, d_samples));
  CU(cudaStreamSynchronize(s));
  dfree(ds.buf, s);
  return KMG_OK;
}

extern "C" int kmg_shard_partition(const void *d_seq, int64_t g0, int64_t g1, int64_t L, int64_t s0, int64_t s1, int k,
                                   const uint64_t *splitters, int nparts, uint64_t *d_keys, uint32_t *d_pos, uint64_t *counts) {
  if (nparts < 1 || nparts > RADIX || !counts) return fail(KMG_ERR_ARG, "nparts must be in [1,%d]", RADIX);
  if (nparts > 1 && !splitters) return fail(KMG_ERR_ARG, "splitters is NULL");
  TRY(ctx_init());
  cudaStream_t s = g_ctx.stream();
  DevSeq ds; SeqView sv;
  TRY(shard_view(d_seq, g0, g1, L, s0, s1, k, s, &ds, &sv));
  for (int i = 0; i < nparts; ++i) counts[i] = 0;
  if (sv.nstarts == 0) { dfree(ds.buf, s); return KMG_OK; }
  if (!d_keys || !d_pos) { dfree(ds.buf, s); return fail(KMG_ERR_ARG, "record arrays are NULL"); }
  if (s0 + sv.nstarts > (int64_t)INT32_MAX) { dfree(ds.buf, s); return fail(KMG_ERR_RANGE, "positions exceed int"); }
  SortScratch sc;
  uint64_t *d_spl = nullptr;
  auto body = [&]() -> int {
    TRY(scratch_alloc(sc, sv.nstarts, s));
    TRY(dalloc(&d_spl, (size_t)RADIX, s));
    if (nparts > 1) CU(cudaMemcpyAsync(d_spl, splitters, (size_t)(nparts - 1) * sizeof(uint64_t), cudaMemcpyHostToDevice, s));
    OwnerBin ob{d_spl, nparts};
    const int64_t tiles = ceil_div<int64_t>(sv.nstarts, HIST_TILE);
    const unsigned hgrid = (unsigned)std::min<int64_t>(tiles, (int64_t)g_ctx.sms * 2);
    LAUNCH("hist_seq_owner", s, hist_seq_kernel<HIST_THREADS, HIST_ITEMS, OwnerBin><<<hgrid, HIST_THREADS, 0, s>>>(sv, sc.hist(0), ob));
    TRY(launch_scan_hist(RADIX_BITS, s, sc.hist(0), sc.gbase(0), (uint64_t *)nullptr));
    PassParams<OwnerBin, NoBin> P{};
    P.sv = sv; P.keys_out = d_keys; P.pos_out = d_pos;
    P.gbase = sc.gbase(0); P.hist_next = nullptr;
    P.status = sc.status; P.ticket = sc.ticket(0); P.epoch = 1;
    P.bin = ob;
    TRY((launch_pass<true, OwnerBin, NoBin, false>("partition", P, sv.nstarts, s)));
    std::vector<uint32_t> h(RADIX);
    CU(cudaMemcpyAsync(h.data(), sc.hist(0), RADIX * 4, cudaMemcpyDeviceToHost, s));
    CU(cudaStreamSynchronize(s));
    double tot = 0;
    for (int i = 0; i < nparts; ++i) { counts[i] = h[i]; tot += h[i]; }
    prof_bytes("hist_seq_owner", (double)sv.avail);
    prof_bytes("partition", (double)sv.avail + 12.0 * tot);
    return KMG_OK;
  };
  int rc = body();
  dfree(d_spl, s); dfree(ds.buf, s);
  scratch_free(sc, s);
  if (rc != KMG_OK) cudaStreamSynchronize(s);
  return rc;
}

extern "C" int kmg_build_records(uint64_t *d_keys, uint32_t *d_pos, int64_t n, int k, kmg_index **out) {
  if (!out) return fail(KMG_ERR_ARG, "out is NULL");
  *out = nullptr;
  if (k < 1 || k > KMG_MAX_K) return fail(KMG_ERR_K, "k must be in [1,32]");
  if (n < 0 || (n > 0 && (!d_keys || !d_pos))) return fail(KMG_ERR_ARG, "bad record arrays");
  if (n > (int64_t)INT32_MAX) return fail(KMG_ERR_RANGE, "too many records");
  TRY(ctx_init());
  cudaStream_t s = g_ctx.stream();
  kmg_index *ix = new (std::nothrow) kmg_index();
  if (!ix) return fail(KMG_ERR_NOMEM, "host allocation failed");
  ix->device = g_ctx.device;
  ix->k = k;
  if (n == 0) {
    int rc = dalloc(&ix->ustart, 1, s);
    if (rc == KMG_OK) cudaMemsetAsync(ix->ustart, 0, 4, s);
    cudaStreamSynchronize(s);
    if (rc != KMG_OK) { delete ix; return rc; }
    *out = ix;
    return KMG_OK;
  }
  SortScratch sc;
  uint64_t *ka = d_keys, *kb = nullptr;
  uint32_t *pa = d_pos, *pb = nullptr, *pfinal = nullptr;
  auto body = [&]() -> int {
    TRY(scratch_alloc(sc, n, s));
    TRY(dalloc(&kb, (size_t)n, s));
    TRY(dalloc(&pb, (size_t)n, s));
    const unsigned hgrid = (unsigned)std::min<int64_t>(ceil_div<int64_t>(n, 256 * 16), (int64_t)g_ctx.sms * 8);
    LAUNCH("hist_rec", s, hist_rec_kernel<256, DigitBin><<<hgrid, 256, 0, s>>>(d_keys, n, nullptr, sc.hist(0), DigitBin{0}));
    TRY(launch_scan_hist(RADIX_BITS, s, sc.hist(0), sc.gbase(0), &sc.stats()->n));
    TRY(dalloc(&pfinal, (size_t)n, s));
    TRY(sort_tail(sc, SortPlan{RADIX_BITS, num_passes(k)}, 0, true, ka, pa, kb, pb, n, s, pfinal));
    TRY(finish_index(ix, sc, ka, pfinal, n, s));
    pfinal = nullptr;
    if (ix->unstable) { demote_rank_variant(); return fail(KMG_ERR_UNSTABLE, "position lists not ascending after the one-atomic sort pass; rebuild (the bitmap variant is now selected)"); }
    const int R = num_passes(k);
    prof_bytes("hist_rec", 8.0 * n);
    if (R > 1) prof_bytes("sort_pass_hist", 24.0 * n * (R - 1));
    prof_bytes("sort_pass", 24.0 * n);
    return KMG_OK;
  };
  int rc = body();
  if (ka != d_keys) dfree(ka, s);
  if (kb != d_keys) dfree(kb, s);
  if (pa != d_pos) dfree(pa, s);
  if (pb != d_pos) dfree(pb, s);
  dfree(pfinal, s);
  scratch_free(sc, s);
  if (rc != KMG_OK) { cudaStreamSynchronize(s); kmg_free(ix); return rc; }
  *out = ix;
  return KMG_OK;
}


struct kmg_shard {
  int device = 0;
  bool hashed = false;
  DevSeq ds;
  SeqView sv;
};

extern "C" int kmg_shard_open(const void *d_seq, int64_t g0, int64_t g1, int64_t L, int64_t s0, int64_t s1, int k, kmg_shard **out) {
  if (!out) return fail(KMG_ERR_ARG, "out is NULL");
  *out = nullptr;
  TRY(ctx_init());
  kmg_shard *sh = new (std::nothrow) kmg_shard();
  if (!sh) return fail(KMG_ERR_NOMEM, "host allocation failed");
  sh->device = g_ctx.device;
  int rc = shard_view(d_seq, g0, g1, L, s0, s1, k, g_ctx.stream(), &sh->ds, &sh->sv);
  if (rc != KMG_OK) { delete sh; return rc; }
  if (s0 + sh->sv.nstarts > (int64_t)INT32_MAX) { kmg_shard_close(sh); return fail(KMG_ERR_RANGE, "positions exceed int"); }
  *out = sh;
  return KMG_OK;
}
extern "C" int kmg_shard_close(kmg_shard *sh) {
  if (!sh) return KMG_OK;
  if (g_ctx.ready && g_ctx.device == sh->device) dfree(sh->ds.buf, g_ctx.stream());
  else { cudaSetDevice(sh->device); g_arena[sh->device & 63].put(sh->ds.buf, nullptr, false); }
  delete sh;
  return KMG_OK;
}
extern "C" int kmg_shard_set_mixed(kmg_shard *sh, int mixed) {
  if (!sh) return fail(KMG_ERR_ARG, "shard is NULL");
  sh->hashed = mixed != 0;
  return KMG_OK;
}
extern "C" int kmg_shard_windows(const kmg_shard *sh, int64_t *nstarts) {
  if (!sh || !nstarts) return fail(KMG_ERR_ARG, "NULL argument");
  *nstarts = sh->sv.nstarts;
  return KMG_OK;
}

extern "C" int kmg_shard_sample_keys(const kmg_shard *sh, int n, uint64_t *d_samples) {
  if (!sh || n <= 0 || !d_samples) return fail(KMG_ERR_ARG, "bad sample request");
  TRY(ctx_init());
  cudaStream_t s = g_ctx.stream();
  LAUNCH("sample", s, sample_kernel<<<ceil_div(n, 256), 256, 0, s>>>(sh->sv, n, d_samples));
  return KMG_OK;
}

__global__ void widen_counts_kernel(const uint32_t *hist, int n, uint64_t *out) {
  if ((int)threadIdx.x < n) out[threadIdx.x] = hist[threadIdx.x];
}

extern "C" int kmg_shard_count(const kmg_shard *sh, const uint64_t *d_splitters, int nparts, uint64_t *d_counts) {
  if (!sh || !d_counts) return fail(KMG_ERR_ARG, "NULL argument");
  if (nparts < 1 || nparts > MAX_PEERS) return fail(KMG_ERR_ARG, "nparts must be in [1,%d]", MAX_PEERS);
  if (nparts > 1 && !d_splitters) return fail(KMG_ERR_ARG, "splitters is NULL");
  TRY(ctx_init());
  cudaStream_t s = g_ctx.stream();
  uint32_t *hist = nullptr;
  TRY(dalloc(&hist, (size_t)RADIX, s));
  CU(cudaMemsetAsync(hist, 0, RADIX * 4, s));
  if (sh->sv.nstarts > 0) {
    OwnerBin ob{d_splitters, nparts};
    const int64_t tiles = ceil_div<int64_t>(sh->sv.nstarts, HIST_TILE);
    const unsigned hgrid = (unsigned)std::min<int64_t>(tiles, (int64_t)g_ctx.sms * 2);
    if (sh->hashed)
      LAUNCH("hist_seq_owner", s, hist_seq_kernel<HIST_THREADS, HIST_ITEMS, HashOwnerBin><<<hgrid, HIST_THREADS, 0, s>>>(sh->sv, hist, HashOwnerBin{ob}));
    else
      LAUNCH("hist_seq_owner", s, hist_seq_kernel<HIST_THREADS, HIST_ITEMS, OwnerBin><<<hgrid, HIST_THREADS, 0, s>>>(sh->sv, hist, ob));
    prof_bytes("hist_seq_owner", (double)sh->sv.avail);
  }
  LAUNCH("widen_counts", s, widen_counts_kernel<<<1, MAX_PEERS, 0, s>>>(hist, nparts, d_counts));
  dfree(hist, s);
// ... 7 lines not shown
  if (nparts < 1 || nparts > MAX_PEERS || rank < 0 || rank >= nparts) return fail(KMG_ERR_ARG, "bad nparts/rank");
  if (nparts > 1 && !d_splitters) return fail(KMG_ERR_ARG, "splitters is NULL");
  if (capacity > (uint64_t)INT32_MAX) return fail(KMG_ERR_RANGE, "capacity exceeds int coordinates");
  TRY(ctx_init());
  cudaStream_t s = g_ctx.stream();
  SortScratch sc;
  PeerTable *tab = nullptr;
  auto body = [&]() -> int {
    TRY(scratch_alloc(sc, sh->sv.nstarts, s));
    TRY(dalloc(&tab, 1, s));
    PeerPtrs pp{};
    for (int i = 0; i < nparts; ++i) { pp.keys[i] = (uint64_t *)peer_keys[i]; pp.pos[i] = (uint32_t *)peer_pos[i]; }
    LAUNCH("owner_offsets", s, owner_offsets_kernel<<<1, RADIX, 0, s>>>(d_matrix, nparts, rank, capacity, pp, sc.gbase(0), tab, d_info));
    if (sh->sv.nstarts == 0) return KMG_OK;
    OwnerBin ob{d_splitters, nparts};
    PassParams<OwnerBin, NoBin> P{};
    P.sv = sh->sv;
    P.gbase = sc.gbase(0); P.hist_next = nullptr;
    P.status = sc.status; P.ticket = sc.ticket(0); P.epoch = 1;
    P.pos_add = (uint32_t)pos_add;
    P.hashed = sh->hashed ? 1u : 0u;
    P.peer = tab;
    P.bin = ob;
    TRY((launch_pass_cfg<PassCfg<256, 24, 2, 0, 8, 8>, true, OwnerBin, NoBin, false, true>("scatter_peer", P, sh->sv.nstarts, s)));
    prof_bytes("scatter_peer", (double)sh->sv.avail + 12.0 * (double)sh->sv.nstarts);
    return KMG_OK;
  };
  int rc = body();
  dfree(tab, s);
  scratch_free(sc, s);
  return rc;
}

__global__ void set_n_kernel(const uint64_t *info, uint64_t cap, uint64_t *n) { *n = info[0] < cap ? info[0] : cap; }

static int owner_build(uint64_t *d_keys, uint32_t *d_pos, uint64_t capacity, const uint64_t *d_info, int nsegs, uint64_t region_cap,
                       const uint64_t *d_counts, int k, int order, kmg_index **out) {
  TRY(ctx_init());
  cudaStream_t s = g_ctx.stream();
  kmg_index *ix = new (std::nothrow) kmg_index();
  if (!ix) return fail(KMG_ERR_NOMEM, "host allocation failed");
  ix->device = g_ctx.device;
  ix->k = k;
  const int64_t n = (int64_t)capacity;
  SortScratch sc;
  uint64_t *ka = d_keys, *kb = nullptr;
  uint32_t *pa = d_pos, *pb = nullptr, *pfinal = nullptr;
  TileSegs *seg = nullptr;
  uint64_t h_info[2] = {0, 0};
  uint32_t h_seg_overflow = 0;
  const bool grouped = grouped_for(k, order, n);
  const SortPlan gp = grouped_plan(d_counts ? n * 10 / 13 : n * 4 / 5);
  auto body = [&]() -> int {
    TRY(scratch_alloc(sc, n, s, grouped ? gp.rb : RADIX_BITS));
    TRY(dalloc(&kb, (size_t)n, s));
    TRY(dalloc(&pb, (size_t)n, s));
    const unsigned hgrid = (unsigned)std::min<int64_t>(ceil_div<int64_t>(n, 256 * 16), (int64_t)g_ctx.sms * 8);
    const int rb0 = grouped ? gp.rb : RADIX_BITS;
    if (d_counts) {
      TRY(dalloc(&seg, 1, s));
      LAUNCH("tile_segs", s, tile_segs_kernel<<<1, MAX_SEGS, 0, s>>>(d_counts, nsegs, region_cap, record_tile(rb0), seg, &sc.stats()->n));
      LAUNCH("hist_rec", s, hist_seg_kernel<256, DigitBin><<<hgrid, 256, 0, s>>>(d_keys, seg, sc.hist(0), DigitBin{0, (1u << rb0) - 1}));
      CU(cudaMemcpyAsync(&h_seg_overflow, &seg->overflow, 4, cudaMemcpyDeviceToHost, s));
    } else {
      LAUNCH("set_n", s, set_n_kernel<<<1, 1, 0, s>>>(d_info, capacity, &sc.stats()->n));
      LAUNCH("hist_rec", s, hist_rec_kernel<256, DigitBin><<<hgrid, 256, 0, s>>>(d_keys, n, &sc.stats()->n, sc.hist(0), DigitBin{0, (1u << rb0) - 1}));
      CU(cudaMemcpyAsync(h_info, d_info, sizeof h_info, cudaMemcpyDeviceToHost, s));
    }
    TRY(launch_scan_hist(rb0, s, sc.hist(0), sc.gbase(0), (uint64_t *)nullptr));
    TRY(dalloc(&pfinal, (size_t)n, s));
    if (grouped) {
      TRY(sort_tail(sc, gp, 0, true, ka, pa, kb, pb, n, s, nullptr, seg, nsegs));
      uint32_t h_cnt[4] = {0, 0, 0, 0};
      uint32_t *fixmem = nullptr;
      int rc = fix_groups(sc, gp.bits(), ka, pa, kb, pb, n, s, h_cnt, &fixmem);
      if (rc == KMG_OK && pa != d_pos) {
        dfree(pfinal, s);
        pfinal = pa;
        pa = nullptr;
      } else if (rc == KMG_OK && cudaMemcpyAsync(pfinal, pa, (size_t)n * 4, cudaMemcpyDeviceToDevice, s) != cudaSuccess) {
        rc = fail(KMG_ERR_CUDA, "copy failed");
      }
      if (rc == KMG_OK) {
        rc = finish_index(ix, sc, ka, pfinal, n, s, true);
        if (rc == KMG_OK) pfinal = nullptr;
      }
      dfree(fixmem, s);
      TRY(rc);
      if (h_cnt[2]) return fail(KMG_ERR_RANGE, "more colliding groups than the task lists hold");
      ix->grouped = true;
      ix->hbits = gp.bits();
    } else {
      TRY(sort_tail(sc, SortPlan{RADIX_BITS, num_passes(k)}, 0, true, ka, pa, kb, pb, n, s, pfinal, seg, nsegs));
      TRY(finish_index(ix, sc, ka, pfinal, n, s));
    }
    pfinal = nullptr;
    if (ix->unstable) { demote_rank_variant(); return fail(KMG_ERR_UNSTABLE, "position lists not ascending after the one-atomic sort pass; rebuild (the bitmap variant is now selected)"); }
    const int R = grouped ? gp.passes : num_passes(k);
    prof_bytes("hist_rec", 8.0 * (double)ix->N);
    if (R > 1) prof_bytes("sort_pass_hist", 24.0 * (double)ix->N * (R - 1));
    prof_bytes("sort_pass", 24.0 * (double)ix->N);
    if (grouped) prof_bytes("group_detect", 8.0 * (double)ix->N);
    return KMG_OK;
  };
  int rc = body();
  if (ka != d_keys) dfree(ka, s);
  if (kb != d_keys) dfree(kb, s);
  if (pa && pa != d_pos) dfree(pa, s);
  if (pb != d_pos) dfree(pb, s);
  dfree(pfinal, s);
  dfree(seg, s);
  scratch_free(sc, s);
  if (rc == KMG_OK && (h_info[1] || h_seg_overflow))
    rc = fail(KMG_ERR_RANGE, "an owner received more than the exchange capacity of %llu records", (unsigned long long)(d_counts ? region_cap : capacity));
  if (rc != KMG_OK) { cudaStreamSynchronize(s); kmg_free(ix); return rc; }
  *out = ix;
  return KMG_OK;
}

extern "C" int kmg_build_received(uint64_t *d_keys, uint32_t *d_pos, uint64_t capacity, const uint64_t *d_info, int k, int order,
                                  kmg_index **out) {
  if (!out) return fail(KMG_ERR_ARG, "out is NULL");
  *out = nullptr;
  if (k < 1 || k > KMG_MAX_K) return fail(KMG_ERR_K, "k must be in [1,32]");
  if (capacity == 0 || capacity > (uint64_t)INT32_MAX || !d_keys || !d_pos || !d_info) return fail(KMG_ERR_ARG, "bad record arrays");
  return owner_build(d_keys, d_pos, capacity, d_info, 0, 0, nullptr, k, order, out);
}
extern "C" int kmg_build_regions(uint64_t *d_keys, uint32_t *d_pos, uint64_t region_cap, int nparts, const uint64_t *d_counts, int k,
                                 kmg_index **out) {
  if (!out) return fail(KMG_ERR_ARG, "out is NULL");
  *out = nullptr;
  if (k < 1 || k > KMG_MAX_K) return fail(KMG_ERR_K, "k must be in [1,32]");
  if (nparts < 1 || nparts > MAX_PEERS || region_cap == 0 || region_cap * (uint64_t)nparts > (uint64_t)INT32_MAX || !d_keys || !d_pos || !d_counts)
    return fail(KMG_ERR_ARG, "bad record arrays");
  if (!grouped_for(k, KMG_ORDER_GROUPED, (int64_t)(region_cap * nparts))) return fail(KMG_ERR_ARG, "region exchange carries mixed keys: k must be large enough for the grouped build");
  return owner_build(d_keys, d_pos, region_cap * (uint64_t)nparts, nullptr, nparts, region_cap, d_counts, k, KMG_ORDER_GROUPED, out);
}

__global__ void region_table_kernel(PeerPtrs pp, PeerPtrs counts , int nparts, int rank, uint64_t region_cap,
                                    PeerTable *tab, uint32_t *gbase, bool announce_zero) {
  const int b = threadIdx.x;
  for (int o = b; o < MAX_NB; o += blockDim.x) gbase[o] = 0;
  if (b < MAX_PEERS) {
    tab->keys[b] = b < nparts ? pp.keys[b] : nullptr;
    tab->pos[b] = b < nparts ? pp.pos[b] : nullptr;
    tab->delta[b] = (int64_t)rank * (int64_t)region_cap;
    tab->counts[b] = b < nparts ? counts.keys[b] : nullptr;
    if (announce_zero && b < nparts) counts.keys[b][rank] = 0;
  }
  if (b == 0) { tab->cap = region_cap; tab->rank = (uint32_t)rank; tab->region = 1; }
}

extern "C" int kmg_shard_scatter_ranges(const kmg_shard *sh, int nparts, int rank, void *const *peer_keys, void *const *peer_pos,
                                        void *const *peer_counts, uint64_t region_cap, int32_t pos_add) {
  if (!sh || !peer_keys || !peer_pos || !peer_counts) return fail(KMG_ERR_ARG, "NULL argument");
  if (nparts < 1 || nparts > MAX_PEERS || rank < 0 || rank >= nparts) return fail(KMG_ERR_ARG, "bad nparts/rank");
  if (region_cap == 0 || region_cap * (uint64_t)nparts > (uint64_t)INT32_MAX) return fail(KMG_ERR_RANGE, "capacity exceeds int coordinates");
  if (!sh->hashed) return fail(KMG_ERR_ARG, "region exchange needs a shard of mixed keys (grouped order, k large enough)");
  TRY(ctx_init());
  cudaStream_t s = g_ctx.stream();
  SortScratch sc;
  PeerTable *tab = nullptr;
  auto body = [&]() -> int {
    TRY(scratch_alloc(sc, sh->sv.nstarts, s, 4));
    TRY(dalloc(&tab, 1, s));
    PeerPtrs pp{}, pc{};
    for (int i = 0; i < nparts; ++i) { pp.keys[i] = (uint64_t *)peer_keys[i]; pp.pos[i] = (uint32_t *)peer_pos[i]; pc.keys[i] = (uint64_t *)peer_counts[i]; }
    LAUNCH("region_table", s, region_table_kernel<<<1, 256, 0, s>>>(pp, pc, nparts, rank, region_cap, tab, sc.gbase(0), sh->sv.nstarts == 0));
    if (sh->sv.nstarts == 0) return KMG_OK;
    PassParams<RangeBin, NoBin> P{};
    P.sv = sh->sv;
    P.gbase = sc.gbase(0); P.hist_next = nullptr;
    P.status = sc.status; P.ticket = sc.ticket(0); P.epoch = 1;
    P.pos_add = (uint32_t)pos_add;
    P.hashed = 1;
    P.peer = tab;
    P.dbg = g_sort_dbg;
    P.bin = RangeBin{(uint32_t)nparts};
    if (rank_variant() >= 3 && !g_scatter_bitmap) {
      if (g_scatter_shape == 1) TRY((launch_pass_cfg<PassCfg<256, 24, 3, 3, 4, 4>, true, RangeBin, NoBin, false, true>("scatter_peer", P, sh->sv.nstarts, s)));
      else if (g_scatter_shape == 2) TRY((launch_pass_cfg<PassCfg<256, 16, 4, 3, 4, 4>, true, RangeBin, NoBin, false, true>("scatter_peer", P, sh->sv.nstarts, s)));
      else TRY((launch_pass_cfg<PassCfg<256, 24, 2, 3, 4, 4>, true, RangeBin, NoBin, false, true>("scatter_peer", P, sh->sv.nstarts, s)));
    } else
      TRY((launch_pass_cfg<PassCfg<256, 24, 2, 0, 8, 4>, true, RangeBin, NoBin, false, true>("scatter_peer", P, sh->sv.nstarts, s)));
    prof_bytes("scatter_peer", (double)sh->sv.avail + 12.0 * (double)sh->sv.nstarts);
    return KMG_OK;
  };
  int rc = body();
// ... 229 lines not shown
};

__global__ void count_first_kernel(const uint32_t *__restrict__ ustart, uint64_t U, int source_n, int source, int32_t *__restrict__ counts) {
  for (uint64_t u = (uint64_t)blockIdx.x * blockDim.x + threadIdx.x; u < U; u += (uint64_t)gridDim.x * blockDim.x)
    counts[u * source_n + source] = (int32_t)(ustart[u + 1] - ustart[u]);
}
__global__ void iota_kernel(uint32_t *p, uint64_t n) {
  for (uint64_t i = (uint64_t)blockIdx.x * blockDim.x + threadIdx.x; i < n; i += (uint64_t)gridDim.x * blockDim.x) p[i] = (uint32_t)i;
}
__global__ void count_merge_kernel(const uint32_t *__restrict__ mstart, const uint32_t *__restrict__ mpay, uint64_t Um, uint64_t Ut,
                                   const int32_t *__restrict__ old_counts, const uint32_t *__restrict__ bstart, int source_n, int source,
                                   int32_t *__restrict__ counts) {
  for (uint64_t u = (uint64_t)blockIdx.x * blockDim.x + threadIdx.x; u < Um; u += (uint64_t)gridDim.x * blockDim.x) {
    int32_t add = 0;
    const int32_t *row = nullptr;
    for (uint32_t j = mstart[u]; j < mstart[u + 1]; ++j) {
      const uint32_t p = mpay[j];
      if (p < Ut) row = old_counts + (uint64_t)p * source_n;
      else add += (int32_t)(bstart[p - Ut + 1] - bstart[p - Ut]);
    }
    for (int s = 0; s < source_n; ++s) counts[u * source_n + s] = (row ? row[s] : 0) + (s == source ? add : 0);
  }
}
__global__ void count_rows_kernel(const int32_t *__restrict__ counts, uint64_t cells, int source_n, int2 *__restrict__ out) {
  for (uint64_t c = (uint64_t)blockIdx.x * blockDim.x + threadIdx.x; c < cells; c += (uint64_t)gridDim.x * blockDim.x)
    out[c] = make_int2((int)(c / source_n + 1), counts[c]);
}
__global__ void spectrum_counts_kernel(const int32_t *__restrict__ counts, uint64_t U, int source_n, int source, uint32_t max_count,
                                       unsigned long long *__restrict__ spec) {
  for (uint64_t u = (uint64_t)blockIdx.x * blockDim.x + threadIdx.x; u < U; u += (uint64_t)gridDim.x * blockDim.x) {
    uint64_t c = 0;
    if (source >= 0) c = (uint64_t)counts[u * source_n + source];
    else for (int s = 0; s < source_n; ++s) c += (uint64_t)counts[u * source_n + s];
    atomicAdd(spec + (c >= max_count ? max_count : c), 1ull);
  }
}
__global__ void spectrum_index_kernel(const uint32_t *__restrict__ ustart, uint64_t U, uint32_t max_count, unsigned long long *__restrict__ spec) {
  for (uint64_t u = (uint64_t)blockIdx.x * blockDim.x + threadIdx.x; u < U; u += (uint64_t)gridDim.x * blockDim.x) {
    const uint32_t c = ustart[u + 1] - ustart[u];
    atomicAdd(spec + (c >= max_count ? max_count : c), 1ull);
  }
}

extern "C" int kmg_count_new(int k, int source_n, kmg_counter **out) {
  if (!out) return fail(KMG_ERR_ARG, "out is NULL");
  *out = nullptr;
  if (k < 1 || k > KMG_MAX_K) return fail(KMG_ERR_K, "k must be a positive integer less than 1+MAX_K");
  if (source_n < 1) return fail(KMG_ERR_ARG, "source_n must be larger than 1 and larger than source");
  TRY(ctx_init());
  kmg_counter *c = new (std::nothrow) kmg_counter();
  if (!c) return fail(KMG_ERR_NOMEM, "host allocation failed");
  c->device = g_ctx.device; c->k = k; c->source_n = source_n;
  *out = c;
  return KMG_OK;
}
extern "C" int kmg_count_free(kmg_counter *c) {
  if (!c) return KMG_OK;
  int prev = -1;
  cudaGetDevice(&prev);
  cudaSetDevice(c->device);
  const bool mine = g_ctx.ready && g_ctx.device == c->device;
  if (mine) cudaStreamSynchronize(g_ctx.stream()); else cudaDeviceSynchronize();
  g_arena[c->device & 63].put(c->keys, nullptr, true);
  g_arena[c->device & 63].put(c->counts, nullptr, true);
  cudaGetLastError();
  if (prev >= 0) cudaSetDevice(prev);
  delete c;
  return KMG_OK;
}
static int use_counter(const kmg_counter *c) {
  if (!c) return fail(KMG_ERR_ARG, "counter is NULL");
  TRY(ctx_init());
  if (c->device != g_ctx.device) return fail(KMG_ERR_ARG, "the count table lives on device %d but this thread works on device %d", c->device, g_ctx.device);
  return KMG_OK;
}

extern "C" int kmg_count_add(kmg_counter *c, const char *seq, int64_t len, int source) {
  TRY(use_counter(c));
  if (source < 0 || source >= c->source_n) return fail(KMG_ERR_ARG, "source_n must be larger than 1 and larger than source");
  if (len < 0 || (len > 0 && !seq)) return fail(KMG_ERR_ARG, "bad sequence pointer/length");
  kmg_index *b = nullptr;
  TRY(kmg_build_ordered(seq, len, c->k, KMG_ORDER_SORTED, &b));
  if (b->U == 0) { kmg_free(b); return KMG_OK; }
  cudaStream_t s = g_ctx.stream();
  const int sn = c->source_n;
  const unsigned grid_of_b = (unsigned)std::min<uint64_t>(ceil_div<uint64_t>(b->U, 256), (uint64_t)g_ctx.sms * 16);
  uint64_t *cat_keys = nullptr;
  uint32_t *cat_pay = nullptr;
  int32_t *ncounts = nullptr;
  kmg_index *m = nullptr;
  auto body = [&]() -> int {
    if (c->U == 0) {
      TRY(dalloc(&ncounts, (size_t)b->U * sn, s));
      CU(cudaMemsetAsync(ncounts, 0, (size_t)b->U * sn * sizeof(int32_t), s));
      LAUNCH("count_first", s, count_first_kernel<<<grid_of_b, 256, 0, s>>>(b->ustart, b->U, sn, source, ncounts));
      CU(cudaStreamSynchronize(s));
      c->keys = b->ukeys; b->ukeys = nullptr;
      c->counts = ncounts; ncounts = nullptr;
      c->U = b->U; c->new_total += b->U;
      return KMG_OK;
    }
    const uint64_t Ut = c->U, n = Ut + b->U;
    if (n > (uint64_t)INT32_MAX) return fail(KMG_ERR_RANGE, "count table would exceed 2^31-1 k-mers");
    TRY(dalloc(&cat_keys, (size_t)n, s));
    TRY(dalloc(&cat_pay, (size_t)n, s));
    CU(cudaMemcpyAsync(cat_keys, c->keys, Ut * 8, cudaMemcpyDeviceToDevice, s));
    CU(cudaMemcpyAsync(cat_keys + Ut, b->ukeys, b->U * 8, cudaMemcpyDeviceToDevice, s));
    LAUNCH("iota", s, iota_kernel<<<(unsigned)std::min<uint64_t>(ceil_div<uint64_t>(n, 256), (uint64_t)g_ctx.sms * 16), 256, 0, s>>>(cat_pay, n));
    TRY(kmg_build_records(cat_keys, cat_pay, (int64_t)n, c->k, &m));
    TRY(dalloc(&ncounts, (size_t)m->U * sn, s));
    LAUNCH("count_merge", s, count_merge_kernel<<<(unsigned)std::min<uint64_t>(ceil_div<uint64_t>(m->U, 256), (uint64_t)g_ctx.sms * 16), 256, 0, s>>>(
                                 m->ustart, m->pos, m->U, Ut, c->counts, b->ustart, sn, source, ncounts));
    CU(cudaStreamSynchronize(s));
    dfree(c->keys, s); dfree(c->counts, s);
    c->keys = m->ukeys; m->ukeys = nullptr;
    c->counts = ncounts; ncounts = nullptr;
    c->new_total += m->U - Ut;
    c->U = m->U;
    return KMG_OK;
  };
  const int rc = body();
  dfree(cat_keys, s); dfree(cat_pay, s); dfree(ncounts, s);
  if (m) kmg_free(m);
  kmg_free(b);
  return rc;
}

extern "C" int kmg_count_sizes(const kmg_counter *c, uint64_t *U, int *source_n, int *k, uint64_t *new_total) {
  if (!c) return fail(KMG_ERR_ARG, "counter is NULL");
  if (U) *U = c->U;
  if (source_n) *source_n = c->source_n;
  if (k) *k = c->k;
  if (new_total) *new_total = c->new_total;
  return KMG_OK;
}
extern "C" int kmg_count_kmers_u64(const kmg_counter *c, uint64_t *keys) {
  TRY(use_counter(c));
  if (c->U == 0) return KMG_OK;
  if (!keys) return fail(KMG_ERR_ARG, "keys is NULL");
  CU(cudaMemcpyAsync(keys, c->keys, c->U * 8, cudaMemcpyDefault, g_ctx.stream()));
  CU(cudaStreamSynchronize(g_ctx.stream()));
  return KMG_OK;
}
extern "C" int kmg_count_kmers_ascii(const kmg_counter *c, char *out) {
  TRY(use_counter(c));
  if (!out && c->U) return fail(KMG_ERR_ARG, "buf is NULL");
  const size_t stride = (size_t)c->k + 1;
  const int k = c->k;
  const uint64_t *keys = c->keys;
  const int sms = g_ctx.sms;
  return stream_rows(c->U, stride, out, CHUNK_BYTES / stride, [=](uint64_t first, uint64_t rows, void *dst, uint64_t *, cudaStream_t s) -> int {
    const unsigned grid = (unsigned)std::min<uint64_t>(ceil_div<uint64_t>(rows * stride, 256), (uint64_t)sms * 16);
    LAUNCH("kmers_ascii", s, kmers_ascii_kernel<<<grid, 256, 0, s>>>(keys + first, rows, k, (char *)dst));
    return KMG_OK;
  });
}
extern "C" int kmg_count_matrix(const kmg_counter *c, int32_t *out) {
  TRY(use_counter(c));
  if (c->U == 0) return KMG_OK;
  if (!out) return fail(KMG_ERR_ARG, "out is NULL");
  CU(cudaMemcpyAsync(out, c->counts, c->U * c->source_n * sizeof(int32_t), cudaMemcpyDefault, g_ctx.stream()));
  CU(cudaStreamSynchronize(g_ctx.stream()));
  return KMG_OK;
}
extern "C" int kmg_count_positions(const kmg_counter *c, int32_t *out) {
  TRY(use_counter(c));
  const uint64_t cells = c->U * (uint64_t)c->source_n;
  if (cells == 0) return KMG_OK;
  if (!out) return fail(KMG_ERR_ARG, "out is NULL");
  const int32_t *counts = c->counts;
  const int sn = c->source_n, sms = g_ctx.sms;
  return stream_rows(cells, 8, out, CHUNK_BYTES / 8, [=](uint64_t first, uint64_t rows, void *dst, uint64_t *, cudaStream_t s) -> int {
    const unsigned grid = (unsigned)std::min<uint64_t>(ceil_div<uint64_t>(rows, 256), (uint64_t)sms * 16);
    LAUNCH("count_rows", s, count_rows_kernel<<<grid, 256, 0, s>>>(counts, first + rows, sn, (int2 *)dst - first));
    return KMG_OK;
  });
}

static int spectrum_out(unsigned long long *d_spec, uint32_t max_count, double *spec, cudaStream_t s) {
  std::vector<unsigned long long> h((size_t)max_count + 1);
  CU(cudaMemcpyAsync(h.data(), d_spec, h.size() * 8, cudaMemcpyDeviceToHost, s));
  CU(cudaStreamSynchronize(s));
  for (size_t i = 0; i < h.size(); ++i) spec[i] = (double)h[i];
  return KMG_OK;
}
extern "C" int kmg_count_spectrum(const kmg_counter *c, int source, uint32_t max_count, double *spec) {
  TRY(use_counter(c));
  if (!spec) return fail(KMG_ERR_ARG, "spec is NULL");
  if (max_count < 1 || max_count > (1u << 30)) return fail(KMG_ERR_ARG, "Unsuitable value of max_count");
  if (source >= c->source_n) return fail(KMG_ERR_ARG, "source out of range");
  cudaStream_t s = g_ctx.stream();
  unsigned long long *d = nullptr;
// ... 242 lines not shown
```

kmer_hasher_b200/csrc/csr.cuh:

```cuda
#pragma once
#include "common.cuh"
#include "lookback.cuh"

namespace kmg {

struct IndexStats {
  uint64_t n;
  uint64_t U;
  uint64_t P;
  uint64_t multi;
  uint32_t maxc;
  uint32_t unstable;
};

template <int THREADS, int ITEMS>
__global__ void __launch_bounds__(THREADS)
rle_kernel(const uint64_t *__restrict__ keys, const uint32_t *__restrict__ pos, IndexStats *st, uint64_t *__restrict__ ukeys,
           uint32_t *__restrict__ ustart, Pair64 *status, uint32_t *ticket, const bool hashed) {
  constexpr int TILE = THREADS * ITEMS, WARPS = THREADS / 32;
  __shared__ uint32_t s_tile, s_wsum[WARPS];
  __shared__ uint64_t s_base;
  const unsigned tid = threadIdx.x, lane = tid & 31u, warp = tid >> 5;
  if (tid == 0) s_tile = atomicAdd(ticket, 1u);
  __syncthreads();
  const uint32_t tile = s_tile;
  const uint64_t n = st->n;
  const uint64_t q0 = (uint64_t)tile * TILE;
  if (q0 >= n) {
    if (n == 0 && tile == 0 && tid == 0) { ustart[0] = 0; st->U = 0; }
    return;
  }
  const uint64_t w0 = q0 + (uint64_t)warp * (32 * ITEMS);
  uint64_t key[ITEMS];
  uint32_t p[ITEMS];
  uint32_t heads = 0, running = 0;
  uint64_t carry = 0;
  uint32_t pcarry = 0;
  bool bad = false;
  if (lane == 0 && w0 > 0 && w0 < n) { carry = ld_stream_u64(keys + w0 - 1); pcarry = ld_stream_u32(pos + w0 - 1); }
  if (q0 + TILE <= n) {
#pragma unroll
    for (int i = 0; i < ITEMS; ++i) key[i] = ld_stream_u64(keys + w0 + i * 32 + lane);
#pragma unroll
    for (int i = 0; i < ITEMS; ++i) p[i] = ld_stream_u32(pos + w0 + i * 32 + lane);
  } else {
#pragma unroll
    for (int i = 0; i < ITEMS; ++i) {
      const uint64_t idx = w0 + i * 32 + lane;
      key[i] = idx < n ? ld_stream_u64(keys + idx) : 0;
      p[i] = idx < n ? ld_stream_u32(pos + idx) : 0;
    }
  }
#pragma unroll
  for (int i = 0; i < ITEMS; ++i) {
    const uint64_t idx = w0 + i * 32 + lane;
    const bool ok = idx < n;
    uint64_t prev = __shfl_up_sync(FULL, key[i], 1);
    uint32_t pprev = __shfl_up_sync(FULL, p[i], 1);
    if (lane == 0) { prev = carry; pprev = pcarry; }
    const bool head = ok && (idx == 0 || key[i] != prev);
    bad |= ok && !head && p[i] <= pprev;
    running += __popc(__ballot_sync(FULL, head));
    if (head) heads |= 1u << i;
    carry = __shfl_sync(FULL, key[i], 31);
    pcarry = __shfl_sync(FULL, p[i], 31);
  }
  if (__any_sync(FULL, bad) && lane == 0) st->unstable = 1;
  if (lane == 0) s_wsum[warp] = running;
  __syncthreads();
  uint32_t wbase = 0, total = 0;
#pragma unroll
  for (int w = 0; w < WARPS; ++w) {
    uint32_t c = s_wsum[w];
    if (w < (int)warp) wbase += c;
    total += c;
  }
  if (warp == 0) {
    uint64_t ea, eb;
    pair_lookback(status, tile, total, 0, ea, eb);
    if (lane == 0) s_base = ea;
  }
  __syncthreads();
  uint64_t base = s_base + wbase;
#pragma unroll
  for (int i = 0; i < ITEMS; ++i) {
    const bool head = (heads >> i) & 1u;
    const unsigned bal = __ballot_sync(FULL, head);
    if (head) {
      const uint64_t u = base + __popc(bal & lanemask_lt());
      ukeys[u] = hashed ? unmix64(key[i]) : key[i];
      ustart[u] = (uint32_t)(w0 + i * 32 + lane);
    }
    base += __popc(bal);
  }
  if (q0 + TILE >= n && tid == 0) {
    const uint64_t U = s_base + total;
    ustart[U] = (uint32_t)n;
    st->U = U;
  }
}

constexpr int SMALL_GROUP = 64;
constexpr uint32_t CLAIM_SLOTS = 1u << 16;

struct FixLists {
  uint2 *small_tasks;
  uint2 *big_tasks;
  uint32_t *counters;
  uint32_t *claim;
  uint32_t small_cap, big_cap;
};

__device__ __forceinline__ uint64_t first_at_least(const uint64_t *h, uint64_t n, uint64_t lowmask, uint64_t v) {
  uint64_t lo = 0, hi = n;
  while (lo < hi) {
    const uint64_t mid = (lo + hi) >> 1;
    if ((h[mid] & lowmask) < v) lo = mid + 1; else hi = mid;
  }
  return lo;
}

__device__ __forceinline__ void file_group(const uint64_t *__restrict__ h, uint64_t n, uint64_t lowmask, uint64_t i, const FixLists &fl) {
  const uint64_t low = h[i] & lowmask;
  constexpr int WALK = 24;
  uint64_t s = i, e = i + 1;
  int w = 0;
  while (s > 0 && w < WALK && (h[s - 1] & lowmask) == low) { --s; ++w; }
  if (s > 0 && (h[s - 1] & lowmask) == low) s = first_at_least(h, n, lowmask, low);
  w = 0;
  while (e < n && w < WALK && (h[e] & lowmask) == low) { ++e; ++w; }
  if (e < n && (h[e] & lowmask) == low) e = low == lowmask ? n : first_at_least(h, n, lowmask, low + 1);
  if (e - s <= SMALL_GROUP) {
    bool first = true;
    const uint64_t h0 = h[s];
    for (uint64_t j = s + 1; j < i; ++j) first &= h[j] == h0;
    if (first) {
      bool dirty = false;
      for (uint64_t j = s + 1; j < e && !dirty; ++j) {
        const uint64_t x = h[j];
        if (x != h[j - 1])
          for (uint64_t m = s; m + 1 < j; ++m)
            if (h[m] == x) { dirty = true; break; }
      }
      if (dirty) {
        const uint32_t t = atomicAdd(fl.counters + 0, 1u);
        if (t < fl.small_cap) fl.small_tasks[t] = make_uint2((uint32_t)s, (uint32_t)e); else fl.counters[2] = 1;
      }
    }
  } else {
    uint32_t slot = (uint32_t)(mix64(s) & (CLAIM_SLOTS - 1));
    bool mine = false, seen = false;
    for (uint32_t probe = 0; probe < CLAIM_SLOTS && !mine && !seen; ++probe) {
      const uint32_t old = atomicCAS(fl.claim + slot, 0u, (uint32_t)s + 1u);
      mine = old == 0u;
      seen = old == (uint32_t)s + 1u;
      slot = (slot + 1) & (CLAIM_SLOTS - 1);
    }
    if (!mine && !seen) fl.counters[2] = 1;
    if (mine) {
      const uint32_t t = atomicAdd(fl.counters + 1, 1u);
      if (t < fl.big_cap) fl.big_tasks[t] = make_uint2((uint32_t)s, (uint32_t)e); else fl.counters[2] = 1;
    }
  }
}

__device__ __forceinline__ void file_group_warp(const uint64_t *__restrict__ h, uint64_t n, uint64_t lowmask, uint64_t i, const FixLists &fl) {
  const unsigned lane = lane_id();
  const uint64_t w0 = i >= 16 ? i - 16 : 0;
  const unsigned p = (unsigned)(i - w0);
  const bool valid = w0 + lane < n;
  const uint64_t x = valid ? h[w0 + lane] : 0;
  const uint64_t low = __shfl_sync(FULL, x, p) & lowmask;
  const unsigned m = __ballot_sync(FULL, valid && (x & lowmask) == low);
  const unsigned below = ~m & ((1u << p) - 1u);
  const unsigned s = below ? 32u - __clz(below) : 0u;
  const unsigned above = ~m >> p;
  const unsigned e = above ? p + (unsigned)__ffs(above) - 1u : 32u;
  if ((s == 0 && w0 > 0) || (e == 32 && w0 + 32 < n)) {
    if (lane == 0) file_group(h, n, lowmask, i, fl);
    return;
  }
  const unsigned run = (e >= 32 ? ~0u : ((1u << e) - 1u)) & ~((1u << s) - 1u);
// ... 126 lines not shown
        s_cur = mm;
        s_placed = placed;
      }
      __syncthreads();
      const uint64_t cur = s_cur;
      if (have_last && cur <= last) break;
      for (uint32_t base = s; base < e; base += THREADS) {
        const uint32_t j = base + tid;
        const bool hit = j < e && h[j] == cur;
        const unsigned bal = __ballot_sync(FULL, hit);
        if (lane == 0) s_cnt[warp] = __popc(bal);
        __syncthreads();
        uint32_t before = 0, total = 0;
#pragma unroll
        for (int w = 0; w < THREADS / 32; ++w) { if (w < (int)warp) before += s_cnt[w]; total += s_cnt[w]; }
        const uint32_t at = s + s_placed + before + __popc(bal & lanemask_lt());
        if (hit) { sh[at] = cur; sp[at] = pos[j]; }
        __syncthreads();
        if (tid == 0) s_placed += total;
        __syncthreads();
      }
      placed = s_placed;
      last = cur;
      have_last = true;
      __syncthreads();
    }
    for (uint32_t j = s + tid; j < e; j += THREADS) { h[j] = sh[j]; pos[j] = sp[j]; }
    __syncthreads();
  }
}

template <int THREADS>
__global__ void __launch_bounds__(THREADS)
stats_kernel(const uint32_t *__restrict__ ustart, const uint64_t U, IndexStats *st) {
  uint64_t P = 0, multi = 0;
  uint32_t maxc = 0;
  const uint64_t groups = U / 4;
  for (uint64_t g = (uint64_t)blockIdx.x * THREADS + threadIdx.x; g < groups; g += (uint64_t)gridDim.x * THREADS) {
    const uint4 v = ld_stream_u4(reinterpret_cast<const uint4 *>(ustart) + g);
    const uint32_t nx = __ldg(ustart + 4 * g + 4);
    const uint32_t c[4] = {v.y - v.x, v.z - v.y, v.w - v.z, nx - v.w};
#pragma unroll
    for (int j = 0; j < 4; ++j) {
      P += (uint64_t)c[j] * (c[j] - 1) / 2;
      multi += c[j] > 1;
      maxc = max(maxc, c[j]);
    }
  }
  if (blockIdx.x == 0 && threadIdx.x < U - 4 * groups) {
    const uint64_t u = 4 * groups + threadIdx.x;
    const uint64_t c = ustart[u + 1] - ustart[u];
    P += c * (c - 1) / 2;
    multi += c > 1;
    maxc = max(maxc, (uint32_t)c);
  }
  P = warp_sum64(P);
  multi = warp_sum64(multi);
#pragma unroll
  for (int d = 16; d > 0; d >>= 1) maxc = max(maxc, __shfl_xor_sync(FULL, maxc, d));
  if (lane_id() == 0) {
    if (P) atomicAdd((unsigned long long *)&st->P, (unsigned long long)P);
    if (multi) atomicAdd((unsigned long long *)&st->multi, (unsigned long long)multi);
    if (maxc) atomicMax(&st->maxc, maxc);
  }
}

template <typename OffT>
__global__ void segment_starts_kernel(const OffT *__restrict__ off, uint64_t cnt, uint64_t first, uint64_t T, uint64_t nblocks,
                                      uint64_t *__restrict__ out) {
  const uint64_t b = (uint64_t)blockIdx.x * blockDim.x + threadIdx.x;
  if (b >= nblocks) return;
  const uint64_t r0 = first + b * T;
  uint64_t lo = 0, hi = cnt;
  while (hi - lo > 1) {
    const uint64_t mid = (lo + hi) >> 1;
    if ((uint64_t)off[mid] <= r0) lo = mid; else hi = mid;
  }
  out[b] = lo;
}

template <int THREADS, int PER, typename OffT>
__device__ __forceinline__ uint64_t block_segments(const OffT *__restrict__ off, uint64_t cnt, uint64_t r0, uint64_t m_first_in,
                                                   uint8_t *s_flag , uint32_t *s_seg ,
                                                   uint32_t *s_warp , uint64_t *s_first) {
  static_assert(PER == 8, "flags are read as one 64-bit word per thread");
  constexpr int T = THREADS * PER, WARPS = THREADS / 32;
  const unsigned tid = threadIdx.x;
  if (tid == 0) *s_first = m_first_in;
  reinterpret_cast<uint64_t *>(s_flag)[tid] = 0;
  __syncthreads();
  const uint64_t m_first = *s_first;
  for (uint64_t m = m_first + 1 + tid; m < cnt; m += THREADS) {
    const uint64_t o = (uint64_t)off[m];
    if (o >= r0 + T) break;
    s_flag[o - r0] = 1;
  }
  __syncthreads();
  const uint64_t f = reinterpret_cast<const uint64_t *>(s_flag)[tid];
  uint32_t mine = __popcll(f);
  uint32_t incl = warp_incl_scan(mine);
  if (lane_id() == 31) s_warp[tid >> 5] = incl;
  __syncthreads();
  uint32_t run = incl - mine;
#pragma unroll
  for (int w = 0; w < WARPS; ++w) if (w < (int)(tid >> 5)) run += s_warp[w];
  uint32_t out[PER];
#pragma unroll
  for (int j = 0; j < PER; ++j) { run += (uint32_t)((f >> (8 * j)) & 1u); out[j] = run; }
  uint4 *dst = reinterpret_cast<uint4 *>(s_seg + tid * PER);
  dst[0] = make_uint4(out[0], out[1], out[2], out[3]);
  dst[1] = make_uint4(out[4], out[5], out[6], out[7]);
  __syncthreads();
  return m_first;
}

__global__ void counts_kernel(const uint32_t *__restrict__ ustart, uint64_t U, int32_t *__restrict__ out) {
  const bool vec = ((reinterpret_cast<uintptr_t>(ustart) | reinterpret_cast<uintptr_t>(out)) & 15u) == 0;
  const uint64_t groups = vec ? U / 4 : 0;
  for (uint64_t g = (uint64_t)blockIdx.x * blockDim.x + threadIdx.x; g < groups; g += (uint64_t)gridDim.x * blockDim.x) {
    const uint4 v = ld_stream_u4(reinterpret_cast<const uint4 *>(ustart) + g);
    const uint32_t nx = __ldg(ustart + 4 * g + 4);
    reinterpret_cast<int4 *>(out)[g] = make_int4((int)(v.y - v.x), (int)(v.z - v.y), (int)(v.w - v.z), (int)(nx - v.w));
  }
  for (uint64_t u = 4 * groups + (uint64_t)blockIdx.x * blockDim.x + threadIdx.x; u < U; u += (uint64_t)gridDim.x * blockDim.x)
    out[u] = (int32_t)(ustart[u + 1] - ustart[u]);
}

template <int THREADS>
__global__ void __launch_bounds__(THREADS)
positions_kernel(const uint32_t *__restrict__ ustart, uint64_t U, const uint32_t *__restrict__ pos, uint64_t first,
                 uint64_t nrows, const uint64_t *__restrict__ blk_first, int2 *__restrict__ out, const uint32_t i_base) {
  constexpr int PER = 8, T = THREADS * PER;
  __shared__ __align__(16) uint8_t s_flag[T];
  __shared__ __align__(16) uint32_t s_seg[T];
  __shared__ uint32_t s_warp[THREADS / 32];
  __shared__ uint64_t s_first;
  const uint64_t b0 = (uint64_t)blockIdx.x * T;
  if (b0 >= nrows) return;
  const uint64_t r0 = first + b0;
  const uint64_t u0 = block_segments<THREADS, PER, uint32_t>(ustart, U, r0, blk_first[blockIdx.x], s_flag, s_seg, s_warp, &s_first);
#pragma unroll
  for (int j = 0; j < PER; ++j) {
    const uint32_t s = j * THREADS + threadIdx.x;
    if (b0 + s < nrows) out[b0 + s] = make_int2((int)(i_base + u0 + s_seg[s] + 1), (int)ld_stream_u32(pos + r0 + s));
  }
}

template <int THREADS, int ITEMS>
__global__ void __launch_bounds__(THREADS)
pair_index_kernel(const uint32_t *__restrict__ ustart, uint64_t U, uint32_t *__restrict__ multi_u,
                  uint64_t *__restrict__ pair_off, Pair64 *status, uint32_t *ticket) {
  constexpr int TILE = THREADS * ITEMS, WARPS = THREADS / 32;
  __shared__ uint32_t s_tile, s_wcnt[WARPS];
  __shared__ uint64_t s_wsum[WARPS], s_base_cnt, s_base_sum;
  const unsigned tid = threadIdx.x, lane = tid & 31u, warp = tid >> 5;
  if (tid == 0) s_tile = atomicAdd(ticket, 1u);
  __syncthreads();
  const uint32_t tile = s_tile;
  const uint64_t q0 = (uint64_t)tile * TILE;
  if (q0 >= U) return;
  const uint64_t u0 = q0 + (uint64_t)tid * ITEMS;
  uint32_t c[ITEMS], cnt = 0;
  uint64_t sum = 0;
#pragma unroll
  for (int i = 0; i < ITEMS; ++i) {
    const uint64_t u = u0 + i;
    c[i] = u < U ? ustart[u + 1] - ustart[u] : 0;
    if (c[i] > 1) { cnt++; sum += (uint64_t)c[i] * (c[i] - 1) / 2; }
  }
  const uint32_t icnt = warp_incl_scan(cnt);
  const uint64_t isum = warp_incl_scan64(sum);
  if (lane == 31) { s_wcnt[warp] = icnt; s_wsum[warp] = isum; }
  __syncthreads();
  uint64_t bcnt = 0, bsum = 0, tcnt = 0, tsum = 0;
#pragma unroll
  for (int w = 0; w < WARPS; ++w) {
    if (w < (int)warp) { bcnt += s_wcnt[w]; bsum += s_wsum[w]; }
    tcnt += s_wcnt[w]; tsum += s_wsum[w];
  }
  if (warp == 0) {
    uint64_t ea, eb;
    pair_lookback(status, tile, tcnt, tsum, ea, eb);
    if (lane == 0) { s_base_cnt = ea; s_base_sum = eb; }
  }
  __syncthreads();
  uint64_t m = s_base_cnt + bcnt + (icnt - cnt);
  uint64_t o = s_base_sum + bsum + (isum - sum);
#pragma unroll
  for (int i = 0; i < ITEMS; ++i) {
    if (c[i] > 1) {
      multi_u[m] = (uint32_t)(u0 + i);
      pair_off[m] = o;
      ++m;
      o += (uint64_t)c[i] * (c[i] - 1) / 2;
    }
  }
}

__device__ __forceinline__ void unrank_pair(uint64_t t, uint64_t n, uint32_t &a, uint32_t &b) {
  const uint64_t m = 2 * n - 1;
  const uint64_t D = m * m - 8 * t;
  uint64_t r = (uint64_t)sqrt((double)D);
  while (r * r > D) --r;
  while ((r + 1) * (r + 1) <= D) ++r;
  uint64_t j = (m - r) / 2;
  if (j > n - 2) j = n - 2;
  while (j > 0 && j * (2 * n - j - 1) / 2 > t) --j;
  while (j + 1 <= n - 2 && (j + 1) * (2 * n - j - 2) / 2 <= t) ++j;
  a = (uint32_t)j;
  b = (uint32_t)(j + 1 + (t - j * (2 * n - j - 1) / 2));
}

template <int THREADS>
__global__ void __launch_bounds__(THREADS)
pairs_kernel(const uint32_t *__restrict__ ustart, const uint32_t *__restrict__ pos,
             const uint32_t *__restrict__ multi_u, const uint64_t *__restrict__ pair_off, uint64_t n_multi,
             uint64_t first, uint64_t nrows, const uint64_t *__restrict__ blk_first, int32_t *__restrict__ out, const uint32_t i_base) {
  constexpr int PER = 8, T = THREADS * PER;
  __shared__ __align__(16) uint8_t s_flag[T];
  __shared__ __align__(16) uint32_t s_seg[T];
  __shared__ uint32_t s_warp[THREADS / 32];
  __shared__ uint64_t s_first;
  const uint64_t b0 = (uint64_t)blockIdx.x * T;
// ... 32 lines not shown
```

kmer_hasher_b200/csrc/probe.cuh:

```cuda
#pragma once
#include "common.cuh"
#include "lookback.cuh"
#include "windows.cuh"
#include "csr.cuh"

namespace kmg {

struct QueryStats {
  uint64_t H;
  uint64_t M;
};

constexpr int BUCKET_SLOTS = 2;

__device__ __forceinline__ uint64_t hash64(uint64_t x) {
  x ^= x >> 33; x *= 0xff51afd7ed558ccdULL;
  x ^= x >> 33; x *= 0xc4ceb9fe1a85ec53ULL;
  x ^= x >> 33;
  return x;
}

struct KeyHash {
  uint4 *slots;
  uint64_t nb;
  int hbits;
  __device__ __forceinline__ uint64_t bucket(uint64_t key) const {
    const uint64_t h = hash64(key);
    return hbits ? __umul64hi(h << (64 - hbits), nb) : (h & (nb - 1));
  }
  __device__ __forceinline__ uint64_t next(uint64_t b) const { return b + 1 == nb ? 0 : b + 1; }
};

__device__ __forceinline__ bool claim_slot(uint4 *slot, uint4 desired) {
  uint64_t olo, ohi;
  const uint64_t dlo = (uint64_t)desired.x | ((uint64_t)desired.y << 32), dhi = (uint64_t)desired.z | ((uint64_t)desired.w << 32);
  asm volatile(
      "{\n\t.reg .b128 cmp, val, old;\n\t"
      "mov.b128 cmp, {%3, %3};\n\t"
      "mov.b128 val, {%4, %5};\n\t"
      "atom.relaxed.gpu.global.cas.b128 old, [%2], cmp, val;\n\t"
      "mov.b128 {%0, %1}, old;\n\t}"
      : "=l"(olo), "=l"(ohi) : "l"(slot), "l"((uint64_t)0), "l"(dlo), "l"(dhi) : "memory");
  return olo == 0 && ohi == 0;
}

__device__ __forceinline__ void cas_insert(const KeyHash &kh, uint64_t key, uint32_t start, uint32_t count, uint64_t b, bool skip_home) {
  const uint4 rec = make_uint4((uint32_t)key, (uint32_t)(key >> 32), start, count);
  if (skip_home) b = kh.next(b);
  bool placed = false;
  while (!placed) {
#pragma unroll
    for (int j = 0; j < BUCKET_SLOTS; ++j)
      if (!placed) placed = claim_slot(kh.slots + b * BUCKET_SLOTS + j, rec);
    b = kh.next(b);
  }
}

__global__ void hash_insert_kernel(const uint64_t *__restrict__ ukeys, const uint32_t *__restrict__ ustart, uint64_t U, KeyHash kh,
                                   const bool overflow_only) {
  for (uint64_t u = (uint64_t)blockIdx.x * blockDim.x + threadIdx.x; u < U; u += (uint64_t)gridDim.x * blockDim.x) {
    const uint64_t key = ukeys[u];
    const uint64_t b = kh.bucket(key);
    if (overflow_only) {
      if (u < 2) continue;
      if (kh.bucket(ukeys[u - 1]) != b || kh.bucket(ukeys[u - 2]) != b) continue;
    }
    const uint32_t start = ustart[u];
    cas_insert(kh, key, start, ustart[u + 1] - start, b, overflow_only);
  }
}

template <int ITEMS>
__global__ void __launch_bounds__(256)
hash_overflow_kernel(const uint64_t *__restrict__ ukeys, const uint32_t *__restrict__ ustart, uint64_t U, KeyHash kh) {
  const uint64_t u0 = ((uint64_t)blockIdx.x * blockDim.x + threadIdx.x) * ITEMS;
  if (u0 >= U) return;
  uint64_t key[ITEMS], cur[ITEMS];
  uint32_t st[ITEMS], cn[ITEMS], slot = 0;
  uint32_t pend = 0;
  uint64_t bm2 = u0 >= 2 ? kh.bucket(ukeys[u0 - 2]) : ~uint64_t(0), bm1 = u0 >= 1 ? kh.bucket(ukeys[u0 - 1]) : ~uint64_t(0);
#pragma unroll
  for (int i = 0; i < ITEMS; ++i) {
    const uint64_t u = u0 + i;
    key[i] = u < U ? ukeys[u] : 0;
    const uint64_t b = kh.bucket(key[i]);
    if (u < U && u >= 2 && bm1 == b && bm2 == b) {
      pend |= 1u << i;
      cur[i] = kh.next(b);
      st[i] = ustart[u];
      cn[i] = ustart[u + 1] - st[i];
    }
    bm2 = bm1; bm1 = b;
  }
  while (pend) {
    uint64_t olo[ITEMS], ohi[ITEMS];
#pragma unroll
    for (int i = 0; i < ITEMS; ++i) {
      if ((pend >> i) & 1u) {
        uint4 *sl = kh.slots + cur[i] * BUCKET_SLOTS + ((slot >> i) & 1u);
        const uint64_t dlo = key[i], dhi = (uint64_t)st[i] | ((uint64_t)cn[i] << 32);
        asm volatile(
            "{\n\t.reg .b128 cmp, val, old;\n\t"
            "mov.b128 cmp, {%3, %3};\n\t"
            "mov.b128 val, {%4, %5};\n\t"
            "atom.relaxed.gpu.global.cas.b128 old, [%2], cmp, val;\n\t"
            "mov.b128 {%0, %1}, old;\n\t}"
            : "=l"(olo[i]), "=l"(ohi[i]) : "l"(sl), "l"((uint64_t)0), "l"(dlo), "l"(dhi) : "memory");
      }
    }
#pragma unroll
    for (int i = 0; i < ITEMS; ++i) {
      if ((pend >> i) & 1u) {
        if (olo[i] == 0 && ohi[i] == 0) pend &= ~(1u << i);
        else if ((slot >> i) & 1u) { slot &= ~(1u << i); cur[i] = kh.next(cur[i]); }
        else slot |= 1u << i;
      }
    }
  }
}

__global__ void hash_stream_kernel(const uint64_t *__restrict__ ukeys, const uint32_t *__restrict__ ustart, uint64_t U, KeyHash kh,
                                   uint64_t *last_bucket) {
  const uint4 zero = make_uint4(0, 0, 0, 0);
  for (uint64_t u = (uint64_t)blockIdx.x * blockDim.x + threadIdx.x; u < U; u += (uint64_t)gridDim.x * blockDim.x) {
    const uint64_t key = ukeys[u];
    const uint64_t b = kh.bucket(key);
    const int64_t bp1 = u > 0 ? (int64_t)kh.bucket(ukeys[u - 1]) : -1;
    if (bp1 != (int64_t)b) {
      const uint32_t s0 = ustart[u], s1 = ustart[u + 1];
      uint4 second = zero;
      if (u + 1 < U) {
        const uint64_t kn = ukeys[u + 1];
        if (kh.bucket(kn) == b) second = make_uint4((uint32_t)kn, (uint32_t)(kn >> 32), s1, ustart[u + 2] - s1);
      }
      kh.slots[b * BUCKET_SLOTS] = make_uint4((uint32_t)key, (uint32_t)(key >> 32), s0, s1 - s0);
      kh.slots[b * BUCKET_SLOTS + 1] = second;
      for (int64_t g = bp1 + 1; g < (int64_t)b; ++g) { kh.slots[g * BUCKET_SLOTS] = zero; kh.slots[g * BUCKET_SLOTS + 1] = zero; }
    }
    if (u + 1 == U) *last_bucket = b;
  }
}

__device__ __forceinline__ uint2 resolve_key(const KeyHash &kh, uint64_t key, uint64_t b, uint4 s0, uint4 s1) {
  const uint32_t klo = (uint32_t)key, khi = (uint32_t)(key >> 32);
  while (true) {
    if (s0.w != 0 && s0.x == klo && s0.y == khi) return make_uint2(s0.z, s0.w);
    if (s1.w != 0 && s1.x == klo && s1.y == khi) return make_uint2(s1.z, s1.w);
    if (s0.w == 0 || s1.w == 0) return make_uint2(0u, 0u);
    b = kh.next(b);
    ld_stream_sector(kh.slots + b * BUCKET_SLOTS, s0, s1);
  }
}

template <int THREADS, int ITEMS, bool FROM_SEQ>
__global__ void __launch_bounds__(THREADS, 4)
probe_lookup_kernel(const SeqView sv, const uint64_t *__restrict__ keys_in, int64_t n_in, const uint64_t *__restrict__ n_dev,
                    const KeyHash kh, uint2 *__restrict__ found, const bool mixed = false) {
  constexpr int TILE = THREADS * ITEMS;
  __shared__ TileCodes<FROM_SEQ ? TILE : 16> tc;
  const unsigned tid = threadIdx.x;
  const int64_t q0 = (int64_t)blockIdx.x * TILE;
  const int64_t total = FROM_SEQ ? sv.nstarts : (n_dev ? min((int64_t)*n_dev, n_in) : n_in);
  if (q0 >= total) return;
  const int t0 = tid * ITEMS;
  bool special = false;
  if constexpr (FROM_SEQ) special = tile_pack<TILE, THREADS>(sv, q0, tc);
  constexpr int BATCH = 4;
  static_assert(ITEMS % BATCH == 0, "items in batches");
  uint64_t key = 0;
  const uint64_t kmask = key_mask(FROM_SEQ ? sv.k : 32);
#pragma unroll
  for (int i0 = 0; i0 < ITEMS; i0 += BATCH) {
    uint4 s0[BATCH], s1[BATCH];
    uint64_t kk[BATCH], home[BATCH];
    bool ok[BATCH];
#pragma unroll
    for (int j = 0; j < BATCH; ++j) {
      const int i = i0 + j;
      if constexpr (FROM_SEQ) {
        if (i == 0) key = tile_key<TILE>(tc, t0, sv.k);
        else {
          const int p = t0 + i + sv.k - 1;
          const uint32_t code = (tc.codes[p >> 4] >> (30 - 2 * (p & 15))) & 3u;
          key = ((key << 2) | code) & kmask;
        }
        ok[j] = tile_valid<TILE>(sv, tc, q0, t0 + i, special);
      } else {
        ok[j] = q0 + t0 + i < total;
        key = ok[j] ? ld_stream_u64(keys_in + q0 + t0 + i) : 0;
        if (mixed) key = unmix64(key);
      }
      kk[j] = key;
      home[j] = kh.bucket(key);
      if (ok[j]) ld_stream_sector(kh.slots + home[j] * BUCKET_SLOTS, s0[j], s1[j]);
    }
    uint2 r[BATCH];
#pragma unroll
    for (int j = 0; j < BATCH; ++j) r[j] = ok[j] ? resolve_key(kh, kk[j], home[j], s0[j], s1[j]) : make_uint2(0u, 0u);
    if (q0 + t0 + i0 + BATCH <= total) {
      uint4 *dst = reinterpret_cast<uint4 *>(found + q0 + t0 + i0);
      dst[0] = make_uint4(r[0].x, r[0].y, r[1].x, r[1].y);
      dst[1] = make_uint4(r[2].x, r[2].y, r[3].x, r[3].y);
    } else {
#pragma unroll
      for (int j = 0; j < BATCH; ++j)
        if (q0 + t0 + i0 + j < total) found[q0 + t0 + i0 + j] = r[j];
    }
  }
}

template <int THREADS, int ITEMS, bool FROM_SEQ>
__global__ void __launch_bounds__(THREADS)
probe_compact_kernel(const uint2 *__restrict__ found, int64_t coord0, const int32_t *__restrict__ i_in, int64_t n_in,
                     const uint64_t *__restrict__ n_dev, int32_t *__restrict__ hit_i, uint32_t *__restrict__ hit_start,
                     uint64_t *__restrict__ row_off, QueryStats *qs, Pair64 *status, uint32_t *ticket) {
  constexpr int TILE = THREADS * ITEMS, WARPS = THREADS / 32;
// ... 201 lines not shown
```

kmer_hasher_b200/rglue/kmer_hash.c:

```c
#include <R.h>
#include <Rinternals.h>
#include <limits.h>
#include <stdint.h>
#include <stdlib.h>
#include <string.h>

#include "kmergpu.h"

#define KMER_HASH_TAG "kmer_hash_250930"
enum { F_KMER = 1, F_POS = 2, F_PAIRS = 4, F_COUNT = 8 };
static const char *const field_names[4] = {"kmer", "pos", "pair.pos", "count"};

typedef struct {
  kmg_index *index;
  kmg_counter *counter;
  int k;
} kmer_handle;

static kmer_handle *handle_or_null(SEXP ptr) {
  if (TYPEOF(ptr) != EXTPTRSXP) return NULL;
  SEXP tag = R_ExternalPtrTag(ptr);
  if (TYPEOF(tag) != STRSXP || length(tag) != 1 || strcmp(CHAR(STRING_ELT(tag, 0)), KMER_HASH_TAG) != 0) return NULL;
  return (kmer_handle *)R_ExternalPtrAddr(ptr);
}
// ... 106 lines not shown
  }
  UNPROTECT(1);
  if (failed) error("kmer.pos failed while extracting %s: %s", failed, kmg_last_error());
  return ret;
}

SEXP count_kmers(SEXP hash_ptr_r, SEXP params_r, SEXP seq_r) {
  if (TYPEOF(seq_r) != STRSXP || length(seq_r) < 1) error("seq_r should be a character vector of length at least one");
  if (TYPEOF(params_r) != INTSXP || length(params_r) != 3) error("k_r must be an integer vector of length 3");
  const int *params = INTEGER(params_r);
  const int k = params[0], source = params[1], source_n = params[2];
  if (k < 1 || k > KMG_MAX_K) error("k must be a positive integer less than 1+MAX_K");
  if (source_n < 1 || source >= source_n || source < 0) error("source_n must be larger than 1 and larger than source");
  SEXP ptr_r = hash_ptr_r;
  kmer_handle *h = NULL;
  int protect_n = 0;
  if (ptr_r == R_NilValue) {
    h = (kmer_handle *)calloc(1, sizeof *h);
    if (!h) error("out of memory");
    h->k = k;
    if (kmg_count_new(k, source_n, &h->counter) != KMG_OK) {
      free(h);
      error("count.kmers failed: %s", kmg_last_error());
    }
    SEXP tag = PROTECT(allocVector(STRSXP, 1));
    SET_STRING_ELT(tag, 0, mkChar(KMER_HASH_TAG));
    ptr_r = PROTECT(R_MakeExternalPtr(h, tag, R_NilValue));
    R_RegisterCFinalizerEx(ptr_r, finalise_handle, TRUE);
    protect_n = 2;
  } else {
    h = handle_or_null(hash_ptr_r);
  }
  if (!h) error("failed to extract kmer_hash from external pointer");
  if (!h->counter) { UNPROTECT(protect_n); error("the external pointer holds a position index, not k-mer counts"); }
  if (h->k != k) { UNPROTECT(protect_n); error("mismatch between specified k and that given in the external pointer"); }
  int sn = 0;
  kmg_count_sizes(h->counter, NULL, &sn, NULL, NULL);
  if (sn != source_n) { UNPROTECT(protect_n); error("mismatch between specified source_n and that of the external pointer"); }
  for (int i = 0; i < length(seq_r); ++i) {
    SEXP s = STRING_ELT(seq_r, i);
    if (length(s) <= k) continue;
    if (kmg_count_add(h->counter, CHAR(s), (int64_t)length(s), source) != KMG_OK) {
      UNPROTECT(protect_n);
      error("count.kmers failed: %s", kmg_last_error());
    }
  }
  UNPROTECT(protect_n);
  return ptr_r;
}

SEXP kmer_positions(SEXP ptr_r, SEXP opt_flag_r) {
  kmer_handle *h = handle_or_error(ptr_r);
  if (TYPEOF(opt_flag_r) != INTSXP || length(opt_flag_r) != 1) error("opt_flag_r should be an integer vector of length 1");
  const unsigned flag = (unsigned)asInteger(opt_flag_r);
  if (h->counter) return count_table_positions(h, flag);

  uint64_t U = 0, N = 0, P = 0;
  if (kmg_sizes(h->index, &U, &N, (flag & F_PAIRS) ? &P : NULL) != KMG_OK) error("kmer.pos failed: %s", kmg_last_error());
  if ((flag & (F_KMER | F_COUNT)) && U > (uint64_t)INT_MAX) error("%llu distinct k-mers do not fit an R vector", (unsigned long long)U);
  if ((flag & F_POS) && N > (uint64_t)INT_MAX) error("%llu positions do not fit an R matrix", (unsigned long long)N);
  if ((flag & F_PAIRS) && P > (uint64_t)INT_MAX)
    error("pair.pos would have %llu rows, more than an R matrix can hold (2^31-1); index a shorter region", (unsigned long long)P);

  SEXP ret = PROTECT(allocVector(VECSXP, 4));
  SEXP names = PROTECT(allocVector(STRSXP, 4));
  for (int i = 0; i < 4; ++i) SET_STRING_ELT(names, i, mkChar(field_names[i]));
  setAttrib(ret, R_NamesSymbol, names);
  UNPROTECT(1);

  const char *failed = NULL;
  if (flag & F_KMER) {
    const size_t stride = (size_t)h->k + 1;
    char *buf = R_alloc(U ? U : 1, (int)stride);
    if (kmg_kmers_ascii(h->index, buf) != KMG_OK) failed = "kmer";
    else {
      SEXP kmers = allocVector(STRSXP, (R_xlen_t)U);
      SET_VECTOR_ELT(ret, 0, kmers);
      for (uint64_t u = 0; u < U; ++u) SET_STRING_ELT(kmers, (R_xlen_t)u, mkCharLen(buf + u * stride, h->k));
    }
  }
  if (!failed && (flag & F_POS)) {
    SEXP m = allocMatrix(INTSXP, 2, (int)N);
    SET_VECTOR_ELT(ret, 1, m);
    if (kmg_positions(h->index, INTEGER(m)) != KMG_OK) failed = "pos";
  }
  if (!failed && (flag & F_PAIRS)) {
    SEXP m = allocMatrix(INTSXP, 3, (int)P);
    SET_VECTOR_ELT(ret, 2, m);
    if (kmg_pairs(h->index, INTEGER(m)) != KMG_OK) failed = "pair.pos";
  }
  if (!failed && (flag & F_COUNT)) {
    SEXP v = allocVector(INTSXP, (R_xlen_t)U);
    SET_VECTOR_ELT(ret, 3, v);
    if (kmg_counts(h->index, INTEGER(v)) != KMG_OK) failed = "count";
  }
  UNPROTECT(1);
  if (failed) error("kmer.pos failed while extracting %s: %s", failed, kmg_last_error());
  return ret;
}

static void finalise_query_guard(SEXP g) {
  kmg_query *q = (kmg_query *)R_ExternalPtrAddr(g);
  if (q) kmg_query_free(q);
  R_ClearExternalPtr(g);
}
static void finalise_join_guard(SEXP g) {
  kmg_join *j = (kmg_join *)R_ExternalPtrAddr(g);
  if (j) kmg_join_free(j);
  R_ClearExternalPtr(g);
}

SEXP sequence_kmer_positions(SEXP ptr_r, SEXP seq_r, SEXP k_r) {
  kmer_handle *h = index_handle_or_error(ptr_r);
  if (TYPEOF(seq_r) != STRSXP || length(seq_r) != 1) error("seq_r should be a single sequence");
  if (TYPEOF(k_r) != INTSXP || length(k_r) != 1) error("k should be an integer of length 1");
  const int k = INTEGER(k_r)[0];
  SEXP s = STRING_ELT(seq_r, 0);
  const char *allow = getenv("KMERGPU_ALLOW_K32");
  const int kmax = (allow && allow[0] == '1') ? 32 : 31;
  if (length(s) <= k || k > kmax || k < 1) error("the sequence should be longer than k and k should not be longer than 31");

  kmg_query *q = NULL;
  uint64_t M = 0;
  if (kmg_query_begin(h->index, CHAR(s), (int64_t)length(s), k, &q, &M) != KMG_OK) error("seq.kmer.pos failed: %s", kmg_last_error());
  if (M > (uint64_t)INT_MAX) {
    kmg_query_free(q);
    error("seq.kmer.pos would return %llu rows, more than an R matrix can hold (2^31-1)", (unsigned long long)M);
  }
  SEXP guard = PROTECT(R_MakeExternalPtr(q, R_NilValue, R_NilValue));
  R_RegisterCFinalizerEx(guard, finalise_query_guard, TRUE);
  SEXP m = PROTECT(allocMatrix(INTSXP, 2, (int)M));
  const int rc = kmg_query_emit(q, INTEGER(m));
  kmg_query_free(q);
  R_ClearExternalPtr(guard);
  UNPROTECT(2);
  if (rc != KMG_OK) error("seq.kmer.pos failed: %s", kmg_last_error());
  return m;
}

SEXP kmer_pair_pos(SEXP ptr_a, SEXP ptr_b) {
  kmer_handle *a = index_handle_or_error(ptr_a);
  kmer_handle *b = index_handle_or_error(ptr_b);
  kmg_join *j = NULL;
  uint64_t M = 0;
  if (kmg_join_begin(a->index, b->index, &j, &M) != KMG_OK) error("kmer.pairs failed: %s", kmg_last_error());
  if (M > (uint64_t)INT_MAX) {
    kmg_join_free(j);
    error("kmer.pairs would return %llu rows, more than an R matrix can hold (2^31-1)", (unsigned long long)M);
  }
  SEXP guard = PROTECT(R_MakeExternalPtr(j, R_NilValue, R_NilValue));
  R_RegisterCFinalizerEx(guard, finalise_join_guard, TRUE);
  SEXP m = PROTECT(allocMatrix(INTSXP, 2, (int)M));
  const int rc = kmg_join_emit(j, INTEGER(m));
  kmg_join_free(j);
  R_ClearExternalPtr(guard);
  UNPROTECT(2);
  if (rc != KMG_OK) error("kmer.pairs failed: %s", kmg_last_error());
  return m;
}

static SEXP new_tagged_pointer(kmer_handle *h) {
  SEXP tag = PROTECT(allocVector(STRSXP, 1));
  SET_STRING_ELT(tag, 0, mkChar(KMER_HASH_TAG));
  SEXP ptr = PROTECT(R_MakeExternalPtr(h, tag, R_NilValue));
  R_RegisterCFinalizerEx(ptr, finalise_handle, TRUE);
  UNPROTECT(2);
  return ptr;
}

SEXP make_kmer_h_index_file(SEXP file_r, SEXP record_r, SEXP k_r, SEXP sort_pos_r) {
  if (TYPEOF(file_r) != STRSXP || length(file_r) != 1) error("file_r should be a single file name");
  if (TYPEOF(record_r) != INTSXP || length(record_r) != 1) error("record_r should be a single integer");
  if (TYPEOF(k_r) != INTSXP || length(k_r) < 1) error("k_r must be an integer vector of length at least one");
  if (TYPEOF(sort_pos_r) != INTSXP || length(sort_pos_r) < 1) error("sort_pos_r must be an integer vector of length at least one");
// ... 66 lines not shown
```

Before: 25.63 billion.

## Defer unique-key materialisation, compact hash overflow list, fuse positions and counts

```diff
diff --git a/include/kmergpu.h b/include/kmergpu.h
--- a/include/kmergpu.h
+++ b/include/kmergpu.h
@@ -52,6 +52,7 @@
 int kmg_pairs(const kmg_index *idx, int32_t *out );
 int kmg_pairs_chunk(const kmg_index *idx, uint64_t first, uint64_t n, int32_t *out );
 int kmg_positions_base(const kmg_index *idx, uint64_t i_base, int32_t *out);
+int kmg_positions_counts(const kmg_index *idx, uint64_t i_base, int32_t *pos , int32_t *counts );
 int kmg_pairs_chunk_base(const kmg_index *idx, uint64_t i_base, uint64_t first, uint64_t n, int32_t *out);
 
 int kmg_query_begin(const kmg_index *idx, const char *q, int64_t qlen, int k, kmg_query **st,
diff --git a/kmer_hasher_b200/__init__.py b/kmer_hasher_b200/__init__.py
--- a/kmer_hasher_b200/__init__.py
+++ b/kmer_hasher_b200/__init__.py
@@ -205,7 +205,14 @@
         a = out.get("pos")
         if a is None:
             a = np.empty((N, 2), np.int32)
-        check(_L.kmg_positions(h, _out_ptr(a)))
+        if opt_flag & OPT_COUNT:
+            c = out.get("count")
+            if c is None:
+                c = np.empty(U, np.int32)
+            check(_L.kmg_positions_counts(h, 0, _out_ptr(a), _out_ptr(c)))
+            res["count"] = c[:U]
+        else:
+            check(_L.kmg_positions(h, _out_ptr(a)))
         res["pos"] = a[:N]
     if opt_flag & OPT_PAIRS:
         if P > INT_MAX:
@@ -216,7 +223,7 @@
             a = np.empty((P, 3), np.int32)
         check(_L.kmg_pairs(h, _out_ptr(a)))
         res["pair.pos"] = a[:P]
-    if opt_flag & OPT_COUNT:
+    if opt_flag & OPT_COUNT and res["count"] is None:
         a = out.get("count")
         if a is None:
             a = np.empty(U, np.int32)
diff --git a/kmer_hasher_b200/_lib.py b/kmer_hasher_b200/_lib.py
--- a/kmer_hasher_b200/_lib.py
+++ b/kmer_hasher_b200/_lib.py
@@ -92,6 +92,7 @@
     "kmg_trim": (C.c_int, []),
     "kmg_cached_bytes": (C.c_uint64, []),
     "kmg_positions_base": (C.c_int, [vp, C.c_uint64, vp]),
+    "kmg_positions_counts": (C.c_int, [vp, C.c_uint64, vp, vp]),
     "kmg_pairs_chunk_base": (C.c_int, [vp, C.c_uint64, C.c_uint64, C.c_uint64, vp]),
 }
 
diff --git a/kmer_hasher_b200/csrc/api.cu b/kmer_hasher_b200/csrc/api.cu
--- a/kmer_hasher_b200/csrc/api.cu
+++ b/kmer_hasher_b200/csrc/api.cu
@@ -427,6 +427,8 @@
   int hbits = 0;
   bool unstable = false;
   uint64_t *ukeys = nullptr;
+  uint64_t *hkeys = nullptr;
+  bool hmixed = false;
   uint32_t *ustart = nullptr;
   uint32_t *pos = nullptr;
   std::mutex mu;
@@ -493,6 +495,7 @@
 static int g_scatter_bitmap = 0;
 static int g_hash_cas = 0;
 static int g_fix_cap = 0;
+static int g_overflow_cap = 0;
 static SortPlan grouped_plan(int64_t n_upper) {
   if (g_hash_bits > 0) {
     const int rb = g_hash_rb > 0 && g_hash_bits % g_hash_rb == 0 ? g_hash_rb : (g_hash_bits % 8 == 0 ? 8 : 9);
@@ -524,6 +527,7 @@
   }
   if (key && !strcmp(key, "sort_dbg")) { g_sort_dbg = (uint32_t)value; return KMG_OK; }
   if (key && !strcmp(key, "fix_cap")) { g_fix_cap = value > 0 ? value : 0; return KMG_OK; }
+  if (key && !strcmp(key, "overflow_cap")) { g_overflow_cap = value > 0 ? value : 0; return KMG_OK; }
   if (key && !strcmp(key, "hash_cas")) { g_hash_cas = value != 0; return KMG_OK; }
   if (key && !strcmp(key, "scatter_bitmap")) { g_scatter_bitmap = value != 0; return KMG_OK; }
   if (key && !strcmp(key, "scatter_shape")) { g_scatter_shape = value; return KMG_OK; }
@@ -658,37 +662,68 @@
   return KMG_OK;
 }
 
+static int gather_ukeys(const uint64_t *keys, const uint32_t *ustart, uint64_t U, bool mixed, uint64_t **out, cudaStream_t s) {
+  uint64_t *ukeys = nullptr;
+  *out = nullptr;
+  if (U == 0) return KMG_OK;
+  TRY(dalloc(&ukeys, (size_t)U, s));
+  const unsigned grid = (unsigned)std::min<uint64_t>(ceil_div<uint64_t>(U, 256), (uint64_t)g_ctx.sms * 16);
+  LAUNCH("ukeys_gather", s, ukeys_gather_kernel<<<grid, 256, 0, s>>>(keys, ustart, U, mixed, ukeys));
+  prof_bytes("ukeys_gather", 12.0 * (double)U + 8.0 * (double)U);
+  *out = ukeys;
+  return KMG_OK;
+}
+
 static int finish_index(kmg_index *ix, SortScratch &sc, uint64_t *keys_sorted, uint32_t *pos_sorted,
-                        int64_t n_upper, cudaStream_t s, bool hashed = false) {
+                        int64_t n_upper, cudaStream_t s, bool hashed = false, bool may_keep = true) {
   IndexStats *st = sc.stats();
+  uint32_t *ustart = nullptr;
   uint64_t *ukeys = nullptr;
-  uint32_t *ustart = nullptr;
   Pair64 *status2 = nullptr;
   const int64_t tiles = ceil_div<int64_t>(n_upper > 0 ? n_upper : 1, RLE_TILE);
-  TRY(dalloc(&ukeys, (size_t)n_upper, s));
   TRY(dalloc(&ustart, (size_t)n_upper + 1, s));
+  if (!may_keep) TRY(dalloc(&ukeys, (size_t)n_upper, s));
   TRY(dalloc(&status2, (size_t)tiles, s));
   CU(cudaMemsetAsync(status2, 0, (size_t)tiles * sizeof(Pair64), s));
-  LAUNCH("rle", s, rle_kernel<RLE_THREADS, RLE_ITEMS><<<(unsigned)tiles, RLE_THREADS, 0, s>>>(
-                       keys_sorted, pos_sorted, st, ukeys, ustart, status2, sc.ticket(MAX_PASSES + 1), hashed));
+  if (may_keep)
+    LAUNCH("rle", s, rle_kernel<RLE_THREADS, RLE_ITEMS, false><<<(unsigned)tiles, RLE_THREADS, 0, s>>>(
+                         keys_sorted, pos_sorted, st, nullptr, ustart, status2, sc.ticket(MAX_PASSES + 1), false));
+  else
+    LAUNCH("rle", s, rle_kernel<RLE_THREADS, RLE_ITEMS, true><<<(unsigned)tiles, RLE_THREADS, 0, s>>>(
+                         keys_sorted, pos_sorted, st, ukeys, ustart, status2, sc.ticket(MAX_PASSES + 1), hashed));
   IndexStats h;
   CU(cudaMemcpyAsync(&h, st, sizeof h, cudaMemcpyDeviceToHost, s));
   CU(cudaStreamSynchronize(s));
   ix->N = h.n; ix->U = h.U; ix->unstable = h.unstable != 0;
   ix->have_stats = false;
   dfree(status2, s);
-  if (h.U * 2 < (uint64_t)n_upper) {
-    uint64_t *uk2; uint32_t *us2;
-    TRY(dalloc(&uk2, (size_t)h.U, s));
+  ix->hmixed = hashed;
+  const bool shrink = h.U * 2 < (uint64_t)n_upper;
+  if (shrink) {
+    uint32_t *us2;
     TRY(dalloc(&us2, (size_t)h.U + 1, s));
-    CU(cudaMemcpyAsync(uk2, ukeys, h.U * sizeof(uint64_t), cudaMemcpyDeviceToDevice, s));
     CU(cudaMemcpyAsync(us2, ustart, (h.U + 1) * sizeof(uint32_t), cudaMemcpyDeviceToDevice, s));
-    dfree(ukeys, s); dfree(ustart, s);
-    ukeys = uk2; ustart = us2;
-  }
-  ix->ukeys = ukeys; ix->ustart = ustart; ix->pos = pos_sorted;
+    dfree(ustart, s);
+    ustart = us2;
+    if (ukeys) {
+      uint64_t *uk2;
+      TRY(dalloc(&uk2, (size_t)h.U, s));
+      CU(cudaMemcpyAsync(uk2, ukeys, h.U * sizeof(uint64_t), cudaMemcpyDeviceToDevice, s));
+      dfree(ukeys, s);
+      ukeys = uk2;
+    }
+  }
+  ix->ustart = ustart; ix->pos = pos_sorted;
+  if (ukeys) {
+    ix->ukeys = ukeys;
+  } else if (shrink) {
+    TRY(gather_ukeys(keys_sorted, ustart, h.U, hashed, &ix->ukeys, s));
+    CU(cudaStreamSynchronize(s));
+  } else {
+    ix->hkeys = keys_sorted;
+  }
   const double N = (double)h.n, U = (double)h.U;
-  prof_bytes("rle", 12 * N + 12 * U);
+  prof_bytes("rle", 12 * N + (may_keep ? 4 : 12) * U);
   return KMG_OK;
 }
 
@@ -852,7 +887,7 @@
         if (log_on()) fprintf(stderr, "[kmergpu] a first-pass bin outgrew its region: rebuilding with the histogram sweep\n");
         void *old[3] = {ix->ukeys, ix->ustart, nullptr};
         for (void *p : old) g_arena[ix->device & 63].put(p, s, false);
-        ix->ukeys = nullptr; ix->ustart = nullptr; ix->pos = nullptr; ix->hbits = 0; ix->unstable = false;
+        ix->ukeys = nullptr; ix->hkeys = nullptr; ix->ustart = nullptr; ix->pos = nullptr; ix->hbits = 0; ix->unstable = false;
         TRY(scratch_clear(sc, s));
         overflow = false;
         TRY(build_grouped(sv, gp, ix, sc, ka, pa, kb, pb, n_upper, s, &overflow, false, &region_overflow));
@@ -860,7 +895,7 @@
       if (!overflow) { pa = nullptr; ix->grouped = true; return KMG_OK; }
       void *old[3] = {ix->ukeys, ix->ustart, nullptr};
       for (void *p : old) g_arena[ix->device & 63].put(p, s, false);
-      ix->ukeys = nullptr; ix->ustart = nullptr; ix->pos = nullptr; ix->hbits = 0;
+      ix->ukeys = nullptr; ix->hkeys = nullptr; ix->ustart = nullptr; ix->pos = nullptr; ix->hbits = 0;
       scratch_free(sc, s);
       TRY(scratch_alloc(sc, n_upper, s, RADIX_BITS));
     }
@@ -887,15 +922,16 @@
     return KMG_OK;
   };
   const int rc = body();
+  if (ix->hkeys == ka) ka = nullptr;
   dfree(ka, s); dfree(kb, s); dfree(pa, s); dfree(pb, s);
   scratch_free(sc, s);
   return rc;
 }
 
 static void release_index_arrays(kmg_index *ix, cudaStream_t s) {
-  void *ptrs[3] = {ix->ukeys, ix->ustart, ix->pos};
+  void *ptrs[4] = {ix->ukeys, ix->hkeys, ix->ustart, ix->pos};
   for (void *p : ptrs) g_arena[ix->device & 63].put(p, s, false);
-  ix->ukeys = nullptr; ix->ustart = nullptr; ix->pos = nullptr;
+  ix->ukeys = nullptr; ix->hkeys = nullptr; ix->ustart = nullptr; ix->pos = nullptr;
   ix->grouped = false; ix->hbits = 0; ix->unstable = false;
 }
 
@@ -975,7 +1011,7 @@
   cudaSetDevice(ix->device);
   const bool mine = g_ctx.ready && g_ctx.device == ix->device;
   if (mine) cudaStreamSynchronize(g_ctx.stream()); else cudaDeviceSynchronize();
-  void *ptrs[6] = {ix->ukeys, ix->ustart, ix->pos, ix->hash, ix->multi_u, ix->pair_off};
+  void *ptrs[7] = {ix->ukeys, ix->hkeys, ix->ustart, ix->pos, ix->hash, ix->multi_u, ix->pair_off};
   for (void *p : ptrs) g_arena[ix->device & 63].put(p, nullptr, true);
   cudaGetLastError();
   if (prev >= 0) cudaSetDevice(prev);
@@ -1007,6 +1043,24 @@
   ix->P = h.P; ix->multi = h.multi; ix->maxc = h.maxc;
   ix->have_stats = true;
   prof_bytes("stats", 4.0 * (double)ix->U);
+  return KMG_OK;
+}
+
+static int ensure_ukeys(const kmg_index *cix) {
+  kmg_index *ix = const_cast<kmg_index *>(cix);
+  std::lock_guard<std::mutex> g(ix->mu);
+  if (ix->ukeys || ix->U == 0) return KMG_OK;
+  TRY(use_index(ix));
+  if (!ix->hkeys) return fail(KMG_ERR_CUDA, "internal error: the index holds neither its keys nor its sorted records");
+  cudaStream_t s = g_ctx.stream();
+  uint64_t *ukeys = nullptr;
+  TRY(gather_ukeys(ix->hkeys, ix->ustart, ix->U, ix->hmixed, &ukeys, s));
+  if (cudaStreamSynchronize(s) != cudaSuccess) {
+    dfree(ukeys, s);
+    return fail(KMG_ERR_CUDA, "key gather failed: %s", cudaGetErrorString(cudaGetLastError()));
+  }
+  dfree(ix->hkeys, s);
+  ix->ukeys = ukeys;
   return KMG_OK;
 }
 
@@ -1142,6 +1196,7 @@
   TRY(use_index(ix));
   if (!keys && ix->U) return fail(KMG_ERR_ARG, "keys is NULL");
   if (ix->U == 0) return KMG_OK;
+  TRY(ensure_ukeys(ix));
   cudaStream_t s = g_ctx.stream();
   CU(cudaMemcpyAsync(keys, ix->ukeys, ix->U * sizeof(uint64_t), cudaMemcpyDefault, s));
   CU(cudaStreamSynchronize(s));
@@ -1151,6 +1206,7 @@
 extern "C" int kmg_kmers_ascii(const kmg_index *ix, char *out) {
   TRY(use_index(ix));
   if (!out && ix->U) return fail(KMG_ERR_ARG, "buf is NULL");
+  TRY(ensure_ukeys(ix));
   const size_t stride = (size_t)ix->k + 1;
   const int k = ix->k;
   const uint64_t *ukeys = ix->ukeys;
@@ -1193,6 +1249,28 @@
     return KMG_OK;
   });
   prof_bytes("positions", 4.0 * U + 12.0 * N);
+  return rc;
+}
+
+extern "C" int kmg_positions_counts(const kmg_index *ix, uint64_t i_base, int32_t *pos_out, int32_t *counts) {
+  TRY(use_index(ix));
+  if ((!pos_out && ix->N) || (!counts && ix->U)) return fail(KMG_ERR_ARG, "out is NULL");
+  if (ix->N == 0) return KMG_OK;
+  if (ptr_kind(pos_out) != PK_DEVICE || ptr_kind(counts) != PK_DEVICE) {
+    TRY(kmg_positions_base(ix, i_base, pos_out));
+    return kmg_counts(ix, counts);
+  }
+  if (i_base + ix->U > (uint64_t)INT32_MAX) return fail(KMG_ERR_RANGE, "k-mer numbers exceed int");
+  const uint32_t *ustart = ix->ustart, *pos = ix->pos;
+  const uint64_t U = ix->U, N = ix->N;
+  int rc = stream_rows(N, 8, pos_out, N, [=](uint64_t first, uint64_t rows, void *dst, uint64_t *blk, cudaStream_t s) -> int {
+    const unsigned grid = (unsigned)ceil_div<uint64_t>(rows, EMIT_TILE);
+    TRY(block_starts(ustart, U, first, rows, s, blk));
+    LAUNCH("positions_counts", s, positions_kernel<EMIT_THREADS, true><<<grid, EMIT_THREADS, 0, s>>>(
+                                      ustart, U, pos, first, rows, blk, (int2 *)dst, (uint32_t)i_base, counts));
+    return KMG_OK;
+  });
+  prof_bytes("positions_counts", 8.0 * U + 12.0 * N);
   return rc;
 }
 
@@ -1254,40 +1332,53 @@
   if (ix->hash || ix->U == 0) return KMG_OK;
   cudaStream_t s = g_ctx.stream();
   const unsigned grid = (unsigned)std::min<uint64_t>(ceil_div<uint64_t>(ix->U, 256), (uint64_t)g_ctx.sms * 32);
+  const bool lazy = !ix->ukeys;
+  const KeySource keys{lazy ? ix->hkeys : ix->ukeys, lazy, lazy && ix->hmixed};
   uint4 *slots = nullptr;
   const bool stream = ix->grouped && ix->hbits >= 8 && ix->hbits <= 56 && !g_hash_cas && (ix->hbits >= 40 || ix->U + ix->U / 4 <= (uint64_t(1) << ix->hbits));
   if (stream) {
     const uint64_t nb = std::max<uint64_t>(ix->U + ix->U / 4, 4);
+    const uint32_t list_cap = g_overflow_cap > 0 ? (uint32_t)g_overflow_cap : (uint32_t)std::min<uint64_t>(ix->U / 4 + 1024, INT32_MAX);
     uint64_t *d_last = nullptr;
+    uint4 *list = nullptr;
     TRY(dalloc(&slots, nb * BUCKET_SLOTS, s));
-    int rc = dalloc(&d_last, 1, s);
-    if (rc != KMG_OK) { dfree(slots, s); return rc; }
+    int rc = dalloc(&d_last, 2, s);
+    if (rc == KMG_OK) rc = dalloc(&list, list_cap, s);
+    if (rc != KMG_OK) { dfree(slots, s); dfree(d_last, s); return rc; }
+    uint64_t h_last[2] = {0, 0};
     auto body = [&]() -> int {
       KeyHash kt{slots, nb, ix->hbits};
-      uint64_t h_last = 0;
-      LAUNCH("hash_stream", s, hash_stream_kernel<<<grid, 256, 0, s>>>(ix->ukeys, ix->ustart, ix->U, kt, d_last));
-      CU(cudaMemcpyAsync(&h_last, d_last, 8, cudaMemcpyDeviceToHost, s));
+      CU(cudaMemsetAsync(d_last, 0, 2 * sizeof(uint64_t), s));
+      LAUNCH("hash_stream", s, hash_stream_kernel<<<grid, 256, 0, s>>>(keys, ix->ustart, ix->U, kt, d_last, list, list_cap,
+                                                                         reinterpret_cast<uint32_t *>(d_last + 1)));
+      CU(cudaMemcpyAsync(h_last, d_last, sizeof h_last, cudaMemcpyDeviceToHost, s));
       CU(cudaStreamSynchronize(s));
-      if (h_last + 1 < nb) CU(cudaMemsetAsync(slots + (h_last + 1) * BUCKET_SLOTS, 0, (nb - h_last - 1) * BUCKET_SLOTS * sizeof(uint4), s));
+      if (h_last[0] + 1 < nb) CU(cudaMemsetAsync(slots + (h_last[0] + 1) * BUCKET_SLOTS, 0, (nb - h_last[0] - 1) * BUCKET_SLOTS * sizeof(uint4), s));
       constexpr int OV_ITEMS = 8;
-      const unsigned ogrid = (unsigned)ceil_div<uint64_t>(ix->U, 256 * OV_ITEMS);
-      LAUNCH("hash_insert", s, hash_overflow_kernel<OV_ITEMS><<<ogrid, 256, 0, s>>>(ix->ukeys, ix->ustart, ix->U, kt));
+      const uint64_t n_over = (uint32_t)h_last[1];
+      if (n_over <= list_cap) {
+        if (n_over) LAUNCH("hash_insert", s, hash_overflow_list_kernel<OV_ITEMS><<<(unsigned)ceil_div<uint64_t>(n_over, 256 * OV_ITEMS), 256, 0, s>>>(list, n_over, kt));
+      } else {
+        const unsigned ogrid = (unsigned)ceil_div<uint64_t>(ix->U, 256 * OV_ITEMS);
+        LAUNCH("hash_insert", s, hash_overflow_kernel<OV_ITEMS><<<ogrid, 256, 0, s>>>(keys, ix->ustart, ix->U, kt));
+      }
       CU(cudaStreamSynchronize(s));
       return KMG_OK;
     };
     rc = body();
-    dfree(d_last, s);
+    dfree(d_last, s); dfree(list, s);
     if (rc != KMG_OK) { dfree(slots, s); return rc; }
     ix->hash = slots; ix->hash_nb = nb; ix->hash_hbits = ix->hbits;
-    prof_bytes("hash_stream", 12.0 * ix->U + 16.0 * BUCKET_SLOTS * nb);
-    prof_bytes("hash_insert", 8.0 * ix->U);
+    const uint64_t n_over = (uint32_t)h_last[1];
+    prof_bytes("hash_stream", 12.0 * ix->U + 16.0 * BUCKET_SLOTS * nb + 16.0 * (double)std::min<uint64_t>(n_over, list_cap));
+    prof_bytes("hash_insert", n_over <= list_cap ? 16.0 * n_over : 12.0 * ix->U);
     return KMG_OK;
   }
   uint64_t cap = 4 * BUCKET_SLOTS;
   while (cap < 2 * ix->U) cap <<= 1;
   TRY(dalloc(&slots, cap, s));
   CU(cudaMemsetAsync(slots, 0, cap * sizeof(uint4), s));
-  LAUNCH("hash_insert", s, hash_insert_kernel<<<grid, 256, 0, s>>>(ix->ukeys, ix->ustart, ix->U, KeyHash{slots, cap / BUCKET_SLOTS, 0}, false));
+  LAUNCH("hash_insert", s, hash_insert_kernel<<<grid, 256, 0, s>>>(keys, ix->ustart, ix->U, KeyHash{slots, cap / BUCKET_SLOTS, 0}, false));
   CU(cudaStreamSynchronize(s));
   ix->hash = slots; ix->hash_nb = cap / BUCKET_SLOTS; ix->hash_hbits = 0;
   prof_bytes("hash_insert", 12.0 * ix->U + 16.0 * ix->U);
@@ -1480,6 +1571,7 @@
   j->a = a; j->b = b;
   if (a->U == 0 || b->U == 0) { *out = j; if (M) *M = 0; return KMG_OK; }
   int rc = ensure_hash(b);
+  if (rc == KMG_OK) rc = ensure_ukeys(a);
   if (rc != KMG_OK) { delete j; return rc; }
   QueryStats *qs = nullptr;
   Pair64 *status = nullptr;
@@ -1667,7 +1759,7 @@
     TRY(launch_scan_hist(RADIX_BITS, s, sc.hist(0), sc.gbase(0), &sc.stats()->n));
     TRY(dalloc(&pfinal, (size_t)n, s));
     TRY(sort_tail(sc, SortPlan{RADIX_BITS, num_passes(k)}, 0, true, ka, pa, kb, pb, n, s, pfinal));
-    TRY(finish_index(ix, sc, ka, pfinal, n, s));
+    TRY(finish_index(ix, sc, ka, pfinal, n, s, false, ka != d_keys));
     pfinal = nullptr;
     if (ix->unstable) { demote_rank_variant(); return fail(KMG_ERR_UNSTABLE, "position lists not ascending after the one-atomic sort pass; rebuild (the bitmap variant is now selected)"); }
     const int R = num_passes(k);
@@ -1677,6 +1769,7 @@
     return KMG_OK;
   };
   int rc = body();
+  if (ix->hkeys == ka) ka = nullptr;
   if (ka != d_keys) dfree(ka, s);
   if (kb != d_keys) dfree(kb, s);
   if (pa != d_pos) dfree(pa, s);
@@ -1850,7 +1943,7 @@
         rc = fail(KMG_ERR_CUDA, "copy failed");
       }
       if (rc == KMG_OK) {
-        rc = finish_index(ix, sc, ka, pfinal, n, s, true);
+        rc = finish_index(ix, sc, ka, pfinal, n, s, true, ka != d_keys);
         if (rc == KMG_OK) pfinal = nullptr;
       }
       dfree(fixmem, s);
@@ -1860,7 +1953,7 @@
       ix->hbits = gp.bits();
     } else {
       TRY(sort_tail(sc, SortPlan{RADIX_BITS, num_passes(k)}, 0, true, ka, pa, kb, pb, n, s, pfinal, seg, nsegs));
-      TRY(finish_index(ix, sc, ka, pfinal, n, s));
+      TRY(finish_index(ix, sc, ka, pfinal, n, s, false, ka != d_keys));
     }
     pfinal = nullptr;
     if (ix->unstable) { demote_rank_variant(); return fail(KMG_ERR_UNSTABLE, "position lists not ascending after the one-atomic sort pass; rebuild (the bitmap variant is now selected)"); }
@@ -1872,6 +1965,7 @@
     return KMG_OK;
   };
   int rc = body();
+  if (ix->hkeys == ka) ka = nullptr;
   if (ka != d_keys) dfree(ka, s);
   if (kb != d_keys) dfree(kb, s);
   if (pa && pa != d_pos) dfree(pa, s);
@@ -2267,6 +2361,7 @@
   kmg_index *b = nullptr;
   TRY(kmg_build_ordered(seq, len, c->k, KMG_ORDER_SORTED, &b));
   if (b->U == 0) { kmg_free(b); return KMG_OK; }
+  if (const int rc0 = ensure_ukeys(b)) { kmg_free(b); return rc0; }
   cudaStream_t s = g_ctx.stream();
   const int sn = c->source_n;
   const unsigned grid_of_b = (unsigned)std::min<uint64_t>(ceil_div<uint64_t>(b->U, 256), (uint64_t)g_ctx.sms * 16);
@@ -2293,6 +2388,7 @@
     CU(cudaMemcpyAsync(cat_keys + Ut, b->ukeys, b->U * 8, cudaMemcpyDeviceToDevice, s));
     LAUNCH("iota", s, iota_kernel<<<(unsigned)std::min<uint64_t>(ceil_div<uint64_t>(n, 256), (uint64_t)g_ctx.sms * 16), 256, 0, s>>>(cat_pay, n));
     TRY(kmg_build_records(cat_keys, cat_pay, (int64_t)n, c->k, &m));
+    TRY(ensure_ukeys(m));
     TRY(dalloc(&ncounts, (size_t)m->U * sn, s));
     LAUNCH("count_merge", s, count_merge_kernel<<<(unsigned)std::min<uint64_t>(ceil_div<uint64_t>(m->U, 256), (uint64_t)g_ctx.sms * 16), 256, 0, s>>>(
                                  m->ustart, m->pos, m->U, Ut, c->counts, b->ustart, sn, source, ncounts));
diff --git a/kmer_hasher_b200/csrc/csr.cuh b/kmer_hasher_b200/csrc/csr.cuh
--- a/kmer_hasher_b200/csrc/csr.cuh
+++ b/kmer_hasher_b200/csrc/csr.cuh
@@ -13,7 +13,7 @@
   uint32_t unstable;
 };
 
-template <int THREADS, int ITEMS>
+template <int THREADS, int ITEMS, bool KEYS>
 __global__ void __launch_bounds__(THREADS)
 rle_kernel(const uint64_t *__restrict__ keys, const uint32_t *__restrict__ pos, IndexStats *st, uint64_t *__restrict__ ukeys,
            uint32_t *__restrict__ ustart, Pair64 *status, uint32_t *ticket, const bool hashed) {
@@ -88,7 +88,7 @@
     const unsigned bal = __ballot_sync(FULL, head);
     if (head) {
       const uint64_t u = base + __popc(bal & lanemask_lt());
-      ukeys[u] = hashed ? unmix64(key[i]) : key[i];
+      if (KEYS) ukeys[u] = hashed ? unmix64(key[i]) : key[i];
       ustart[u] = (uint32_t)(w0 + i * 32 + lane);
     }
     base += __popc(bal);
@@ -98,6 +98,17 @@
     ustart[U] = (uint32_t)n;
     st->U = U;
   }
+}
+
+__device__ __forceinline__ uint64_t distinct_key(const uint64_t *__restrict__ keys, const uint32_t *__restrict__ ustart, uint64_t u,
+                                                 bool mixed) {
+  const uint64_t h = keys[ustart[u]];
+  return mixed ? unmix64(h) : h;
+}
+__global__ void ukeys_gather_kernel(const uint64_t *__restrict__ keys, const uint32_t *__restrict__ ustart, uint64_t U, bool mixed,
+                                    uint64_t *__restrict__ ukeys) {
+  for (uint64_t u = (uint64_t)blockIdx.x * blockDim.x + threadIdx.x; u < U; u += (uint64_t)gridDim.x * blockDim.x)
+    ukeys[u] = distinct_key(keys, ustart, u, mixed);
 }
 
 constexpr int SMALL_GROUP = 64;
@@ -390,7 +401,8 @@
 template <int THREADS, int PER, typename OffT>
 __device__ __forceinline__ uint64_t block_segments(const OffT *__restrict__ off, uint64_t cnt, uint64_t r0, uint64_t m_first_in,
                                                    uint8_t *s_flag , uint32_t *s_seg ,
-                                                   uint32_t *s_warp , uint64_t *s_first) {
+                                                   uint32_t *s_warp , uint64_t *s_first,
+                                                   int32_t *__restrict__ counts = nullptr) {
   static_assert(PER == 8, "flags are read as one 64-bit word per thread");
   constexpr int T = THREADS * PER, WARPS = THREADS / 32;
   const unsigned tid = threadIdx.x;
@@ -398,10 +410,12 @@
   reinterpret_cast<uint64_t *>(s_flag)[tid] = 0;
   __syncthreads();
   const uint64_t m_first = *s_first;
+  if (counts && tid == 0 && (uint64_t)off[m_first] == r0) counts[m_first] = (int32_t)(off[m_first + 1] - off[m_first]);
   for (uint64_t m = m_first + 1 + tid; m < cnt; m += THREADS) {
     const uint64_t o = (uint64_t)off[m];
     if (o >= r0 + T) break;
     s_flag[o - r0] = 1;
+    if (counts) counts[m] = (int32_t)((uint64_t)off[m + 1] - o);
   }
   __syncthreads();
   const uint64_t f = reinterpret_cast<const uint64_t *>(s_flag)[tid];
@@ -434,10 +448,11 @@
     out[u] = (int32_t)(ustart[u + 1] - ustart[u]);
 }
 
-template <int THREADS>
+template <int THREADS, bool COUNTS = false>
 __global__ void __launch_bounds__(THREADS)
 positions_kernel(const uint32_t *__restrict__ ustart, uint64_t U, const uint32_t *__restrict__ pos, uint64_t first,
-                 uint64_t nrows, const uint64_t *__restrict__ blk_first, int2 *__restrict__ out, const uint32_t i_base) {
+                 uint64_t nrows, const uint64_t *__restrict__ blk_first, int2 *__restrict__ out, const uint32_t i_base,
+                 int32_t *__restrict__ counts = nullptr) {
   constexpr int PER = 8, T = THREADS * PER;
   __shared__ __align__(16) uint8_t s_flag[T];
   __shared__ __align__(16) uint32_t s_seg[T];
@@ -446,7 +461,8 @@
   const uint64_t b0 = (uint64_t)blockIdx.x * T;
   if (b0 >= nrows) return;
   const uint64_t r0 = first + b0;
-  const uint64_t u0 = block_segments<THREADS, PER, uint32_t>(ustart, U, r0, blk_first[blockIdx.x], s_flag, s_seg, s_warp, &s_first);
+  const uint64_t u0 = block_segments<THREADS, PER, uint32_t>(ustart, U, r0, blk_first[blockIdx.x], s_flag, s_seg, s_warp, &s_first,
+                                                             COUNTS ? counts : nullptr);
 #pragma unroll
   for (int j = 0; j < PER; ++j) {
     const uint32_t s = j * THREADS + threadIdx.x;
diff --git a/kmer_hasher_b200/csrc/probe.cuh b/kmer_hasher_b200/csrc/probe.cuh
--- a/kmer_hasher_b200/csrc/probe.cuh
+++ b/kmer_hasher_b200/csrc/probe.cuh
@@ -24,11 +24,17 @@
   uint4 *slots;
   uint64_t nb;
   int hbits;
-  __device__ __forceinline__ uint64_t bucket(uint64_t key) const {
-    const uint64_t h = hash64(key);
-    return hbits ? __umul64hi(h << (64 - hbits), nb) : (h & (nb - 1));
-  }
+  __device__ __forceinline__ uint64_t bucket_of_hash(uint64_t h) const { return hbits ? __umul64hi(h << (64 - hbits), nb) : (h & (nb - 1)); }
+  __device__ __forceinline__ uint64_t bucket(uint64_t key) const { return bucket_of_hash(hash64(key)); }
   __device__ __forceinline__ uint64_t next(uint64_t b) const { return b + 1 == nb ? 0 : b + 1; }
+};
+
+struct KeySource {
+  const uint64_t *words;
+  bool via_start, mixed;
+  __device__ __forceinline__ uint64_t word(uint64_t u, uint32_t s) const { return words[via_start ? (uint64_t)s : u]; }
+  __device__ __forceinline__ uint64_t key(uint64_t w) const { return mixed ? unmix64(w) : w; }
+  __device__ __forceinline__ uint64_t hash(uint64_t w) const { return mixed ? w : hash64(w); }
 };
 
 __device__ __forceinline__ bool claim_slot(uint4 *slot, uint4 desired) {
@@ -56,42 +62,25 @@
   }
 }
 
-__global__ void hash_insert_kernel(const uint64_t *__restrict__ ukeys, const uint32_t *__restrict__ ustart, uint64_t U, KeyHash kh,
+__global__ void hash_insert_kernel(const KeySource ukeys, const uint32_t *__restrict__ ustart, uint64_t U, KeyHash kh,
                                    const bool overflow_only) {
   for (uint64_t u = (uint64_t)blockIdx.x * blockDim.x + threadIdx.x; u < U; u += (uint64_t)gridDim.x * blockDim.x) {
-    const uint64_t key = ukeys[u];
-    const uint64_t b = kh.bucket(key);
+    const uint32_t start = ustart[u];
+    const uint64_t w = ukeys.word(u, start);
+    const uint64_t b = kh.bucket_of_hash(ukeys.hash(w));
     if (overflow_only) {
       if (u < 2) continue;
-      if (kh.bucket(ukeys[u - 1]) != b || kh.bucket(ukeys[u - 2]) != b) continue;
-    }
-    const uint32_t start = ustart[u];
-    cas_insert(kh, key, start, ustart[u + 1] - start, b, overflow_only);
+      if (kh.bucket_of_hash(ukeys.hash(ukeys.word(u - 1, ustart[u - 1]))) != b ||
+          kh.bucket_of_hash(ukeys.hash(ukeys.word(u - 2, ustart[u - 2]))) != b) continue;
+    }
+    cas_insert(kh, ukeys.key(w), start, ustart[u + 1] - start, b, overflow_only);
   }
 }
 
 template <int ITEMS>
-__global__ void __launch_bounds__(256)
-hash_overflow_kernel(const uint64_t *__restrict__ ukeys, const uint32_t *__restrict__ ustart, uint64_t U, KeyHash kh) {
-  const uint64_t u0 = ((uint64_t)blockIdx.x * blockDim.x + threadIdx.x) * ITEMS;
-  if (u0 >= U) return;
-  uint64_t key[ITEMS], cur[ITEMS];
-  uint32_t st[ITEMS], cn[ITEMS], slot = 0;
-  uint32_t pend = 0;
-  uint64_t bm2 = u0 >= 2 ? kh.bucket(ukeys[u0 - 2]) : ~uint64_t(0), bm1 = u0 >= 1 ? kh.bucket(ukeys[u0 - 1]) : ~uint64_t(0);
-#pragma unroll
-  for (int i = 0; i < ITEMS; ++i) {
-    const uint64_t u = u0 + i;
-    key[i] = u < U ? ukeys[u] : 0;
-    const uint64_t b = kh.bucket(key[i]);
-    if (u < U && u >= 2 && bm1 == b && bm2 == b) {
-      pend |= 1u << i;
-      cur[i] = kh.next(b);
-      st[i] = ustart[u];
-      cn[i] = ustart[u + 1] - st[i];
-    }
-    bm2 = bm1; bm1 = b;
-  }
+__device__ __forceinline__ void cas_pending(const KeyHash &kh, const uint64_t (&key)[ITEMS], uint64_t (&cur)[ITEMS],
+                                            const uint32_t (&st)[ITEMS], const uint32_t (&cn)[ITEMS], uint32_t pend) {
+  uint32_t slot = 0;
   while (pend) {
     uint64_t olo[ITEMS], ohi[ITEMS];
 #pragma unroll
@@ -119,19 +108,95 @@
   }
 }
 
-__global__ void hash_stream_kernel(const uint64_t *__restrict__ ukeys, const uint32_t *__restrict__ ustart, uint64_t U, KeyHash kh,
-                                   uint64_t *last_bucket) {
+template <int ITEMS>
+__global__ void __launch_bounds__(256)
+hash_overflow_list_kernel(const uint4 *__restrict__ list, uint64_t n, KeyHash kh) {
+  const uint64_t t0 = ((uint64_t)blockIdx.x * blockDim.x + threadIdx.x) * ITEMS;
+  if (t0 >= n) return;
+  uint64_t key[ITEMS], cur[ITEMS];
+  uint32_t st[ITEMS], cn[ITEMS], pend = 0;
+#pragma unroll
+  for (int i = 0; i < ITEMS; ++i) {
+    const uint4 r = t0 + i < n ? list[t0 + i] : make_uint4(0, 0, 0, 0);
+    key[i] = (uint64_t)r.x | ((uint64_t)r.y << 32);
+    cur[i] = kh.next(kh.bucket(key[i]));
+    st[i] = r.z; cn[i] = r.w;
+    if (t0 + i < n) pend |= 1u << i;
+  }
+  cas_pending<ITEMS>(kh, key, cur, st, cn, pend);
+}
+
+template <int ITEMS>
+__global__ void __launch_bounds__(256)
+hash_overflow_kernel(const KeySource ukeys, const uint32_t *__restrict__ ustart, uint64_t U, KeyHash kh) {
+  const uint64_t u0 = ((uint64_t)blockIdx.x * blockDim.x + threadIdx.x) * ITEMS;
+  if (u0 >= U) return;
+  uint64_t key[ITEMS], cur[ITEMS];
+  uint32_t st[ITEMS], cn[ITEMS], pend = 0;
+  uint64_t bm2 = ~uint64_t(0), bm1 = ~uint64_t(0);
+  if (u0 >= 2) bm2 = kh.bucket_of_hash(ukeys.hash(ukeys.word(u0 - 2, ustart[u0 - 2])));
+  if (u0 >= 1) bm1 = kh.bucket_of_hash(ukeys.hash(ukeys.word(u0 - 1, ustart[u0 - 1])));
+#pragma unroll
+  for (int i = 0; i < ITEMS; ++i) {
+    const uint64_t u = u0 + i;
+    const uint32_t s0 = u < U ? ustart[u] : 0;
+    const uint64_t w = u < U ? ukeys.word(u, s0) : 0;
+    const uint64_t b = kh.bucket_of_hash(ukeys.hash(w));
+    key[i] = ukeys.key(w);
+    if (u < U && u >= 2 && bm1 == b && bm2 == b) {
+      pend |= 1u << i;
+      cur[i] = kh.next(b);
+      st[i] = s0;
+      cn[i] = ustart[u + 1] - s0;
+    }
+    bm2 = bm1; bm1 = b;
+  }
+  cas_pending<ITEMS>(kh, key, cur, st, cn, pend);
+}
+
+__global__ void hash_stream_kernel(const KeySource ks, const uint32_t *__restrict__ ustart, uint64_t U, KeyHash kh,
+                                   uint64_t *last_bucket, uint4 *__restrict__ list, uint32_t cap, uint32_t *n_list) {
   const uint4 zero = make_uint4(0, 0, 0, 0);
-  for (uint64_t u = (uint64_t)blockIdx.x * blockDim.x + threadIdx.x; u < U; u += (uint64_t)gridDim.x * blockDim.x) {
-    const uint64_t key = ukeys[u];
-    const uint64_t b = kh.bucket(key);
-    const int64_t bp1 = u > 0 ? (int64_t)kh.bucket(ukeys[u - 1]) : -1;
+  const unsigned lane = lane_id();
+  for (uint64_t u = (uint64_t)blockIdx.x * blockDim.x + threadIdx.x; u - lane < U; u += (uint64_t)gridDim.x * blockDim.x) {
+    const bool ok = u < U;
+    const uint32_t s0 = ok ? ustart[u] : 0;
+    const uint32_t sm1 = lane == 0 && ok && u >= 1 ? ustart[u - 1] : 0, sm2 = lane == 0 && ok && u >= 2 ? ustart[u - 2] : 0;
+    const uint32_t sp1 = lane == 31 && ok ? ustart[u + 1] : 0, sp2 = lane == 31 && u + 2 <= U ? ustart[u + 2] : 0;
+    const uint64_t w = ok ? ks.word(u, s0) : 0;
+    const uint64_t wm1 = lane == 0 && ok && u >= 1 ? ks.word(u - 1, sm1) : 0, wm2 = lane == 0 && ok && u >= 2 ? ks.word(u - 2, sm2) : 0;
+    const uint64_t wp1 = lane == 31 && u + 1 < U ? ks.word(u + 1, sp1) : 0;
+    const uint64_t b = kh.bucket_of_hash(ks.hash(w));
+    uint64_t bm1 = __shfl_up_sync(FULL, b, 1);
+    if (lane == 0) bm1 = kh.bucket_of_hash(ks.hash(wm1));
+    uint64_t bm2 = __shfl_up_sync(FULL, bm1, 1);
+    if (lane == 0) bm2 = kh.bucket_of_hash(ks.hash(wm2));
+    uint32_t s1 = __shfl_down_sync(FULL, s0, 1);
+    uint64_t wn = __shfl_down_sync(FULL, w, 1);
+    if (lane == 31) { s1 = sp1; wn = wp1; }
+    uint32_t s2 = __shfl_down_sync(FULL, s1, 1);
+    if (lane == 31) s2 = sp2;
+    if (u + 1 == U) s1 = ustart[U];
+    if (u + 2 == U) s2 = ustart[U];
+    const bool over = ok && u >= 2 && bm1 == b && bm2 == b;
+    const unsigned m = __ballot_sync(FULL, over);
+    if (m) {
+      uint32_t base = 0;
+      const int first = __ffs(m) - 1;
+      if ((int)lane == first) base = atomicAdd(n_list, (uint32_t)__popc(m));
+      base = __shfl_sync(FULL, base, first);
+      const uint32_t at = base + __popc(m & lanemask_lt());
+      const uint64_t key = ks.key(w);
+      if (over && at < cap) list[at] = make_uint4((uint32_t)key, (uint32_t)(key >> 32), s0, s1 - s0);
+    }
+    if (!ok) continue;
+    const int64_t bp1 = u > 0 ? (int64_t)bm1 : -1;
     if (bp1 != (int64_t)b) {
-      const uint32_t s0 = ustart[u], s1 = ustart[u + 1];
+      const uint64_t key = ks.key(w);
       uint4 second = zero;
-      if (u + 1 < U) {
-        const uint64_t kn = ukeys[u + 1];
-        if (kh.bucket(kn) == b) second = make_uint4((uint32_t)kn, (uint32_t)(kn >> 32), s1, ustart[u + 2] - s1);
+      if (u + 1 < U && kh.bucket_of_hash(ks.hash(wn)) == b) {
+        const uint64_t kn = ks.key(wn);
+        second = make_uint4((uint32_t)kn, (uint32_t)(kn >> 32), s1, s2 - s1);
       }
       kh.slots[b * BUCKET_SLOTS] = make_uint4((uint32_t)key, (uint32_t)(key >> 32), s0, s1 - s0);
       kh.slots[b * BUCKET_SLOTS + 1] = second;
diff --git a/kmer_hasher_b200/rglue/kmer_hash.c b/kmer_hasher_b200/rglue/kmer_hash.c
--- a/kmer_hasher_b200/rglue/kmer_hash.c
+++ b/kmer_hasher_b200/rglue/kmer_hash.c
@@ -212,14 +212,18 @@
   if (!failed && (flag & F_POS)) {
     SEXP m = allocMatrix(INTSXP, 2, (int)N);
     SET_VECTOR_ELT(ret, 1, m);
-    if (kmg_positions(h->index, INTEGER(m)) != KMG_OK) failed = "pos";
+    if (flag & F_COUNT) {
+      SEXP v = allocVector(INTSXP, (R_xlen_t)U);
+      SET_VECTOR_ELT(ret, 3, v);
+      if (kmg_positions_counts(h->index, 0, INTEGER(m), INTEGER(v)) != KMG_OK) failed = "pos/count";
+    } else if (kmg_positions(h->index, INTEGER(m)) != KMG_OK) failed = "pos";
   }
   if (!failed && (flag & F_PAIRS)) {
     SEXP m = allocMatrix(INTSXP, 3, (int)P);
     SET_VECTOR_ELT(ret, 2, m);
     if (kmg_pairs(h->index, INTEGER(m)) != KMG_OK) failed = "pair.pos";
   }
-  if (!failed && (flag & F_COUNT)) {
+  if (!failed && (flag & F_COUNT) && !(flag & F_POS)) {
     SEXP v = allocVector(INTSXP, (R_xlen_t)U);
     SET_VECTOR_ELT(ret, 3, v);
     if (kmg_counts(h->index, INTEGER(v)) != KMG_OK) failed = "count";
```

Result: faster. 26.91 billion (median of 6 runs) (+5.0%).
